# peabody124/PosePipeline

Hardware: AMD Instinct MI355X
Metric: frames/sec (whole node), detect->2D->3D cascade on 1080p; MPJPE vs reference (higher is better)
Workload: dtype f32; eligible float32 convolutions are evaluated as 2-term float16 splits (22 significand bits under per-channel / per-sample power-of-two scales, 3 products per term) on the 16-bit matrix cores with float32 accumulation (float32-accurate at any input magnitude, not bit-identical: tests/test_gpu_spl

## Files before the change

### include/posepipe_hip.h

```cpp
#ifndef POSEPIPE_HIP_H
#define POSEPIPE_HIP_H

#include <stddef.h>
#include <stdint.h>

#ifdef __cplusplus
extern "C" {
#endif

#define PP_ABI_VERSION 10

typedef enum {
    PP_OK = 0,
    PP_ERR_ARG = -1,
    PP_ERR_HIP = -2,
    PP_ERR_STATE = -3,
    PP_ERR_UNSUPPORTED = -4
} pp_status;

typedef enum { PP_MEM_HOST = 0, PP_MEM_DEVICE = 1 } pp_mem_kind;

typedef struct pp_ctx pp_ctx;
typedef struct pp_net pp_net;
typedef struct pp_tracker pp_tracker;
typedef struct pp_topdown pp_topdown;

int pp_abi_version(void);
const char* pp_last_error(void);
int pp_device_count(void);
int pp_ctx_create(int device, pp_ctx** out);
void pp_ctx_destroy(pp_ctx* ctx);
int pp_ctx_set_stream(pp_ctx* ctx, void* hip_stream);
int pp_ctx_synchronize(pp_ctx* ctx);
int pp_timer_start(pp_ctx* ctx);
int pp_timer_stop(pp_ctx* ctx, float* elapsed_ms);
int pp_debug_knob(const char* name, int value);
int pp_malloc(pp_ctx* ctx, size_t bytes, void** dptr);
int pp_free(pp_ctx* ctx, void* dptr);
int pp_memcpy_h2d(pp_ctx* ctx, void* dst, const void* src, size_t bytes);
int pp_memcpy_d2h(pp_ctx* ctx, void* dst, const void* src, size_t bytes);
int pp_memcpy_d2d(pp_ctx* ctx, void* dst, const void* src, size_t bytes);
int pp_host_alloc(pp_ctx* ctx, size_t bytes, void** host_ptr);
int pp_host_free(pp_ctx* ctx, void* host_ptr);
int pp_upload_begin(pp_ctx* ctx, void* dst_device, const void* src_host, size_t bytes);
int pp_upload_begin_nv12(pp_ctx* ctx, void* dst_bgr_device, void* tmp_nv12_device, const void* src_nv12_host, int frames,
                         int height, int width);
int pp_nv12_to_bgr(pp_ctx* ctx, const uint8_t* nv12_device, int frames, int height, int width, uint8_t* bgr_device);
int pp_upload_wait(pp_ctx* ctx, int host_sync);
int pp_upload_release(pp_ctx* ctx);

typedef enum {
    PP_OP_CONV = 1,
    PP_OP_MAXPOOL = 2,
    PP_OP_ROIALIGN = 3,
    PP_OP_COPY = 4,
    PP_OP_VIT_ENCODER = 5,
    PP_OP_DEPTH_TO_SPACE = 6,
    PP_OP_DECONV_BF16 = 8,
    PP_OP_AVGPOOL = 9,
    PP_OP_UPSAMPLE_ADD = 7,
    PP_OP_BILINEAR_ADD = 10,
    PP_OP_DWCONV3X3 = 11,
    PP_OP_LAYERNORM = 12,
    PP_OP_WINDOW_ATTN = 13,
    PP_OP_GELU_ADD = 14,
    PP_OP_ATTENTION = 15
} pp_op_type;

#define PP_RELU_NONE 0
#define PP_RELU_LAST 1
#define PP_RELU_FIRST 2
#define PP_ACT_LEAKY 3
#define PP_ACT_MISH 4
#define PP_ACT_ELU 5
#define PP_ACT_SWISH 6
#define PP_ACT_GELU 7
#define PP_DW_GELU_IN 1

typedef struct pp_op {
    int32_t type;
    int32_t in, out;
    int32_t res1, res2;
    int32_t cin, cout;
    int32_t kh, kw, stride, pad_h, pad_w, dil_h, dil_w;
    int32_t relu;
    int32_t up_log2;
    int32_t out_nchw;
    int32_t res1_shift;
    int32_t res1_off_w;
    int32_t out_c_off;
    int32_t in_c_off;
    int32_t pad_end;
    int64_t w_off, b_off;
    int32_t in2, in3;
    int32_t up2_log2, up3_log2;
} pp_op;

typedef struct pp_buf {
    int32_t h, w, c;
    int32_t pad;
} pp_buf;

int pp_net_create(pp_ctx* ctx, const pp_op* ops, int n_ops, const pp_buf* bufs, int n_bufs,
                  const float* weights, size_t n_weights, int max_batch, pp_net** out);
int pp_net_create_mem(pp_ctx* ctx, const pp_op* ops, int n_ops, const pp_buf* bufs, int n_bufs,
                      const float* weights, size_t n_weights, int weights_mem, int max_batch, pp_net** out);
#define PP_NET_NUMERICS_DEFAULT 0
#define PP_NET_NUMERICS_EXACT 1
#define PP_NET_NUMERICS_SPLIT 2
#define PP_NET_NUMERICS_SPLIT_BF16 3
#define PP_NET_NUMERICS_SPLIT_F16 4
int pp_net_create_ex(pp_ctx* ctx, const pp_op* ops, int n_ops, const pp_buf* bufs, int n_bufs,
                     const float* weights, size_t n_weights, int weights_mem, int max_batch, int numerics, pp_net** out);
int pp_net_numerics(pp_net* net);
int pp_net_split_kind(pp_net* net);
void pp_net_destroy(pp_net* net);
int pp_net_buffer(pp_net* net, int buf, void** dptr, size_t* bytes_per_sample);
int pp_net_input_amax(pp_net* net, int buf, void** dptr);
int pp_net_run(pp_net* net, int batch, int first_op, int last_op);
int pp_net_forward(pp_net* net, int batch, int in_buf, const float* in, int out_buf, float* out,
                   int mem);
int pp_net_set_lanes(pp_net* net, int enable);
int pp_net_set_lane_count(pp_net* net, int n_lanes);
int pp_net_capture(pp_net* net, int batch);
int pp_net_profile(pp_net* net, int batch, float* ms_per_op);
int pp_net_conv_kinds(pp_net* net, int* kinds);
int pp_net_folded_into(pp_net* net, int* into);

int pp_conv_force(int ct, int pt);
int pp_conv_variant(int variant);
int pp_conv_exact(int exact);
int pp_conv_split_kind(int f16);

int pp_conv2d(pp_ctx* ctx, const pp_op* op, int n, int hin, int win, const float* x,
              const float* w, const float* bias, const float* res1, const float* res2, float* y,
              int res1_h, int res1_w, int mem);

int pp_crop_resize_bilinear(pp_ctx* ctx, const float* src_nhwc4, int n_src, int src_h, int src_w, const int32_t* rects5, int n,
                            int out_h, int out_w, float* out_nhwc4);

int pp_net_vit_timing(pp_net* net, int enable, float* ms3, int* n_gemm);
int pp_f32_to_bf16(pp_ctx* ctx, const float* x, uint16_t* y, size_t n);
int pp_gemm_bf16(pp_ctx* ctx, const uint16_t* a, const uint16_t* w, const float* bias, const float* res, int res_mod,
                 void* c, int m, int n, int k, int act, int out_bf16);
int pp_layernorm(pp_ctx* ctx, const float* x, const float* gamma, const float* beta, int rows, int dim, float eps,
                 void* y, int out_bf16);
int pp_attention_bf16(pp_ctx* ctx, const uint16_t* qkv, int batch, int tokens, int heads, int head_dim, uint16_t* out);

int pp_crop_affine_normalize(pp_ctx* ctx, const uint8_t* frames, int n_frames, int h, int w,
                             const int32_t* frame_idx, const double* bbox_tlwh, int n_person,
                             int out_w, int out_h, const float* lut, const int32_t* chan_map,
                             int flip, float* out, float* center_scale, uint8_t* crop_u8,
                             int32_t* valid, int mem);

int pp_flip_merge_decode(pp_ctx* ctx, const float* hm, const float* hm_flip, int n, int k, int h,
                         int w, const int32_t* flip_perm, int shift_heatmap, int post,
                         int blur_kernel, const float* center_scale, float* kpts, float* merged,
                         int mem);

int pp_topdown_create(pp_net* net, int in_buf, int out_buf, int num_joints, const int32_t* flip_perm,
                      int shift_heatmap, int post, int blur_kernel, const float* lut,
                      const int32_t* chan_map, pp_topdown** out);
void pp_topdown_destroy(pp_topdown* t);
int pp_topdown_run(pp_topdown* t, const uint8_t* frames, int n_frames, int h, int w, int frames_mem,
                   const int32_t* frame_idx, const double* bbox_tlwh, int n_person, float* kpts,
                   int kpts_mem, int32_t* valid);
int pp_topdown_run_precropped(pp_topdown* t, const float* x_nhwc4, int x_mem, const float* center_scale,
                              int n_person, float* kpts, int kpts_mem);

int pp_topdown_timing(pp_topdown* t, float* ms3);

int pp_nms(pp_ctx* ctx, const void* boxes, const void* scores, int n, double iou_thr, int convention,
           int32_t* keep, int32_t* n_keep, int mem);

int pp_tracker_create(int mode, int feat_dim, double max_iou_distance, double max_cosine_distance,
                      int max_age, int n_init, pp_tracker** out);
void pp_tracker_destroy(pp_tracker* t);
int pp_tracker_step(pp_tracker* t, const double* dets_tlwh, const double* conf, const double* feats,
                    int n_det, int cap, int64_t* track_id, double* tlwh, int32_t* info, int32_t* n_out);
int pp_tracker_dump(pp_tracker* t, int cap, int64_t* ids, int32_t* state4, double* mean8,
                    double* cov64, int32_t* n_out);
int pp_kalman_initiate(const double* z4, double* mean8, double* cov64);
int pp_kalman_predict(double* mean8, double* cov64);
int pp_kalman_update(double* mean8, double* cov64, const double* z4);
int pp_kalman_gating_distance(const double* mean8, const double* cov64, const double* z4, int n,
                              double* out);
int pp_linear_sum_assignment(const double* cost, int n_rows, int n_cols, int32_t* rows,
                             int32_t* cols, int32_t* n_pairs);

typedef struct pp_detector pp_detector;
int pp_detector_input_size(int src_h, int src_w, int32_t* nh, int32_t* nw, int32_t* hp, int32_t* wp);
int pp_rescale_size(int src_h, int src_w, int max_long, int max_short, int divisor, int32_t* nh, int32_t* nw,
                    int32_t* hp, int32_t* wp);
int pp_resize_pad_normalize(pp_ctx* ctx, const uint8_t* frames, int n, int src_h, int src_w, int frames_mem, int nh,
                            int nw, int hp, int wp, const float* lut, float pad_val, float* out_device);
int pp_detector_constants(double* out, int cap);
int pp_detector_create(pp_net* net_a, pp_net* net_b, const int32_t* bufs_a, const int32_t* bufs_b, int src_h,
                       int src_w, const float* lut, const float* base_anchors, pp_detector** out);
void pp_detector_destroy(pp_detector* d);
int pp_detector_run(pp_detector* d, const uint8_t* frames, int n_frames, int frames_mem, float* dets,
                    int32_t* n_dets, float* proposals, int32_t* n_proposals);
int pp_detector_timing(pp_detector* d, float* ms6);
int pp_detector_enqueue(pp_detector* d, const uint8_t* frames, int n_frames, int frames_mem, int want_proposals);
int pp_detector_collect(pp_detector* d, float* dets, int32_t* n_dets, float* proposals, int32_t* n_proposals);
#define PP_DET_N_MARGINS 8
#define PP_DET_MARGIN_RPN_CUT 0
#define PP_DET_MARGIN_RPN_NMS 1
#define PP_DET_MARGIN_RPN_TOP 2
#define PP_DET_MARGIN_ROI_LEVEL 3
#define PP_DET_MARGIN_SCORE_THR 4
#define PP_DET_MARGIN_DET_NMS 5
#define PP_DET_MARGIN_DET_TOP 6
#define PP_DET_MARGIN_DET_ORDER 7
int pp_detector_enable_margins(pp_detector* d, int enable, float score_weight);
int pp_detector_margins(pp_detector* d, int n_frames, float* margins);

int pp_detector_regress(pp_detector* d, int frame, const float* boxes_src_px, int n, float* out_boxes, float* out_scores);

enum { PP_ECC_OK = 0, PP_ECC_NAN = 1 , PP_ECC_DIVERGED = 2  };
int pp_gray_from_nhwc4(pp_ctx* ctx, const float* x_nhwc4, int n, int h, int w, int r, int g, int b, float* gray);
int pp_ecc_euclidean(pp_ctx* ctx, const float* gray, int n_images, int h, int w, const int32_t* pairs, int n_pairs, int num_iters,
                     double stop_eps, double* warp, double* rho, int32_t* iters, int32_t* status);

int pp_letterbox_bicubic(pp_ctx* ctx, const uint8_t* frames, int n, int src_h, int src_w, int frames_mem,
                         const int32_t* xtab, int nw, int kx, const int32_t* ytab, int nh, int ky, int size_h,
                         int size_w, float* out_device);
int pp_yolo_decode(pp_ctx* ctx, const float* feats, int n, int gh, int gw, int num_classes, int cls,
                   const float* anchors3x2, int input_h, int input_w, int image_h, int image_w, float* boxes,
                   float* scores, int out_mem);
int pp_reid_patches(pp_ctx* ctx, const uint8_t* frames, int n_frames, int src_h, int src_w, int frames_mem,
                    const int32_t* rects, int n, int ph, int pw, float* out_device);

int pp_videopose3d_lift_many(pp_net* net, int in_buf, int out_buf, const float* kpts2d_norm,
                             const int32_t* seg_frames, int n_segs, int in_features, int out_features,
                             int pad, float* out, int mem);
int pp_videopose3d_lift(pp_net* net, int in_buf, int out_buf, const float* kpts2d_norm, int n_frames,
                        int in_features, int out_features, int pad, float* out);

int pp_warp_affine_normalize(pp_ctx* ctx, const uint8_t* frames, int n_frames, int h, int w, const double* center,
                             const double* scale, int out_w, int out_h, const float* lut, const int32_t* chan_map,
                             int flip, float* out, uint8_t* warp_u8, int mem);
int pp_bottomup_aggregate(pp_ctx* ctx, const float* s0, const float* s1, int n_frames, int k, int h0, int w0, int h1,
                          int w1, const int32_t* flip_perm, int hr, int wr, int align_corners, float* hm);
int pp_bottomup_candidates(pp_ctx* ctx, const float* hm, const float* s0, int n_frames, int k, int h0, int w0,
                           const int32_t* flip_perm, int hr, int wr, int align_corners, int max_people, float* cand);
int pp_bottomup_refine(pp_ctx* ctx, const float* hm, const float* s0, int n_frames, int k, int h0, int w0,
                       const int32_t* flip_perm, int hr, int wr, int align_corners, int n_person,
                       const int32_t* person_frame, const float* mean_tag, const int32_t* need, float* out);

int pp_attention_f32(pp_ctx* ctx, const float* qkv, int batch, int tokens, int heads, int c_real, int c_buf, float* out);
int pp_poseformer_spatial_param_floats(void);
int pp_poseformer_head_param_floats(void);
int pp_poseformer_spatial(pp_ctx* ctx, const float* params, const float* kpts2d_norm, int n_frames, int kpts_mem, float* features);
int pp_poseformer_lift(pp_net* net, int in_buf, int out_buf, long long spatial_off, long long pos_off, long long head_off,
                       const float* kpts2d_norm, int n_frames, float* out, int mem, float* stage_ms);

#define PP_OP_DCN3X3 16
#define PP_OP_DWDECONV 17
int pp_fairmot_input_size(int src_h, int src_w, int32_t* hp, int32_t* wp, int32_t* nh, int32_t* nw, int32_t* top, int32_t* left);
int pp_fairmot_preprocess(pp_ctx* ctx, const uint8_t* frames, int n, int src_h, int src_w, int frames_mem, int hp, int wp, int nh,
                          int nw, int top, int left, float* out_device);
int pp_fairmot_decode(pp_ctx* ctx, const float* hm, const float* wh, const float* reg, const float* id, int n, int h, int w, int K,
                      int id_dim, float* dets, float* feats, int32_t* inds, int mem);

typedef struct pp_smpl_model pp_smpl_model;
int pp_warp_affine_normalize_each(pp_ctx* ctx, const uint8_t* frames, int n_frames, int h, int w, const int32_t* frame_idx,
                                  const double* matrices, int n, int out_w, int out_h, const float* lut, const int32_t* chan_map,
                                  float* out, uint8_t* crop_u8, int mem);
long long pp_gru_param_floats(int in, int hidden, int layers);
int pp_gru_forward(pp_ctx* ctx, const float* x, int B, int T, int in, int hidden, int layers, const float* params, float* y, int mem);
int pp_smpl_model_create(pp_ctx* ctx, const float* v_template, const float* shapedirs, const float* posedirs, const float* j_regressor,
                         const float* weights, const float* j_regressor_extra, int n_verts, const int32_t* vertex_ids,
                         const int32_t* joint_map, pp_smpl_model** out);
void pp_smpl_model_destroy(pp_smpl_model* model);
int pp_smpl_forward(pp_ctx* ctx, pp_smpl_model* model, const float* betas, const float* rotmat, const float* cam, int F, float* verts,
                    float* joints3d, float* kp2d, float* pose_aa, int mem);
int pp_vibe_head_unpack(pp_ctx* ctx, const float* pose6d, const float* shape, int shape_stride, const float* cam_in, int cam_stride,
                        int F, float* rotmat, float* betas, float* cam);

#define PP_OP_SUB_CAT 18
// ... 16 lines not shown
```

### posepipeline_amd/_lib.py

```python
from __future__ import annotations

import ctypes as C
import os

import numpy as np

_HERE = os.path.dirname(os.path.abspath(__file__))
LIB_PATH = os.environ.get("POSEPIPE_LIB", os.path.join(_HERE, "libposepipe_hip.so"))

PP_MEM_HOST, PP_MEM_DEVICE = 0, 1
PP_OP_CONV, PP_OP_MAXPOOL, PP_OP_ROIALIGN, PP_OP_COPY, PP_OP_VIT_ENCODER, PP_OP_DEPTH_TO_SPACE, PP_OP_UPSAMPLE_ADD = 1, 2, 3, 4, 5, 6, 7
PP_OP_DECONV_BF16 = 8
PP_OP_AVGPOOL = 9
PP_OP_BILINEAR_ADD = 10
PP_OP_DWCONV3X3, PP_OP_LAYERNORM, PP_OP_WINDOW_ATTN, PP_OP_GELU_ADD = 11, 12, 13, 14
PP_OP_ATTENTION = 15
PP_OP_DCN3X3, PP_OP_DWDECONV = 16, 17
PP_OP_SUB_CAT, PP_OP_BCAST_MUL, PP_OP_BLEND2 = 18, 19, 20
PP_OP_GRAPH_MIX, PP_OP_JOINT_ATTN = 21, 22
PP_RELU_NONE, PP_RELU_LAST, PP_RELU_FIRST = 0, 1, 2
PP_ACT_LEAKY, PP_ACT_MISH, PP_ACT_ELU, PP_ACT_SWISH = 3, 4, 5, 6
PP_ACT_GELU = 7
PP_DW_GELU_IN = 1
PP_NET_NUMERICS_DEFAULT, PP_NET_NUMERICS_EXACT, PP_NET_NUMERICS_SPLIT = 0, 1, 2
PP_NET_NUMERICS_SPLIT_BF16, PP_NET_NUMERICS_SPLIT_F16 = 3, 4
PP_ECC_OK, PP_ECC_NAN, PP_ECC_DIVERGED = 0, 1, 2
NUMERICS = {None: 0, "default": 0, "exact": 1, "split": 2, "split_bf16": 3, "split_f16": 4}


class PosePipeHipError(RuntimeError):
    pass


class pp_op(C.Structure):
    _fields_ = [
        ("type", C.c_int32),
        ("in_", C.c_int32),
        ("out", C.c_int32),
        ("res1", C.c_int32),
        ("res2", C.c_int32),
        ("cin", C.c_int32),
        ("cout", C.c_int32),
        ("kh", C.c_int32),
        ("kw", C.c_int32),
        ("stride", C.c_int32),
        ("pad_h", C.c_int32),
        ("pad_w", C.c_int32),
        ("dil_h", C.c_int32),
        ("dil_w", C.c_int32),
        ("relu", C.c_int32),
        ("up_log2", C.c_int32),
        ("out_nchw", C.c_int32),
        ("res1_shift", C.c_int32),
        ("res1_off_w", C.c_int32),
        ("out_c_off", C.c_int32),
        ("in_c_off", C.c_int32),
        ("pad_end", C.c_int32),
        ("w_off", C.c_int64),
        ("b_off", C.c_int64),
        ("in2", C.c_int32),
        ("in3", C.c_int32),
        ("up2_log2", C.c_int32),
        ("up3_log2", C.c_int32),
    ]

    def __init__(self, *args, **kw):
        kw.setdefault("in2", -1)
        kw.setdefault("in3", -1)
        super().__init__(*args, **kw)


class pp_buf(C.Structure):
    _fields_ = [("h", C.c_int32), ("w", C.c_int32), ("c", C.c_int32), ("pad", C.c_int32)]


_vp = C.c_void_p
_i = C.c_int
_sz = C.c_size_t

SIGNATURES = {
    "pp_abi_version": (_i, []),
    "pp_last_error": (C.c_char_p, []),
    "pp_device_count": (_i, []),
    "pp_ctx_create": (_i, [_i, C.POINTER(_vp)]),
    "pp_ctx_destroy": (None, [_vp]),
    "pp_ctx_set_stream": (_i, [_vp, _vp]),
    "pp_ctx_synchronize": (_i, [_vp]),
    "pp_timer_start": (_i, [_vp]),
    "pp_timer_stop": (_i, [_vp, C.POINTER(C.c_float)]),
    "pp_malloc": (_i, [_vp, _sz, C.POINTER(_vp)]),
    "pp_free": (_i, [_vp, _vp]),
    "pp_memcpy_h2d": (_i, [_vp, _vp, _vp, _sz]),
    "pp_memcpy_d2h": (_i, [_vp, _vp, _vp, _sz]),
    "pp_memcpy_d2d": (_i, [_vp, _vp, _vp, _sz]),
    "pp_host_alloc": (_i, [_vp, _sz, C.POINTER(_vp)]),
    "pp_host_free": (_i, [_vp, _vp]),
    "pp_upload_begin": (_i, [_vp, _vp, _vp, _sz]),
    "pp_upload_begin_nv12": (_i, [_vp, _vp, _vp, _vp, _i, _i, _i]),
    "pp_nv12_to_bgr": (_i, [_vp, _vp, _i, _i, _i, _vp]),
    "pp_upload_wait": (_i, [_vp, _i]),
    "pp_upload_release": (_i, [_vp]),
    "pp_net_create": (_i, [_vp, C.POINTER(pp_op), _i, C.POINTER(pp_buf), _i, _vp, _sz, _i, C.POINTER(_vp)]),
    "pp_net_create_mem": (_i, [_vp, C.POINTER(pp_op), _i, C.POINTER(pp_buf), _i, _vp, _sz, _i, _i, C.POINTER(_vp)]),
    "pp_net_create_ex": (_i, [_vp, C.POINTER(pp_op), _i, C.POINTER(pp_buf), _i, _vp, _sz, _i, _i, _i, C.POINTER(_vp)]),
    "pp_net_numerics": (_i, [_vp]),
    "pp_net_split_kind": (_i, [_vp]),
    "pp_conv_split_kind": (_i, [_i]),
    "pp_net_destroy": (None, [_vp]),
    "pp_net_buffer": (_i, [_vp, _i, C.POINTER(_vp), C.POINTER(_sz)]),
    "pp_net_run": (_i, [_vp, _i, _i, _i]),
    "pp_net_forward": (_i, [_vp, _i, _i, _vp, _i, _vp, _i]),
    "pp_net_capture": (_i, [_vp, _i]),
    "pp_net_set_lanes": (_i, [_vp, _i]),
    "pp_net_set_lane_count": (_i, [_vp, _i]),
    "pp_net_conv_kinds": (_i, [_vp, _vp]),
    "pp_net_folded_into": (_i, [_vp, _vp]),
    "pp_net_profile": (_i, [_vp, _i, _vp]),
    "pp_crop_resize_bilinear": (_i, [_vp, _vp, _i, _i, _i, _vp, _i, _i, _i, _vp]),
    "pp_conv_force": (_i, [_i, _i]),
    "pp_conv_variant": (_i, [_i]),
    "pp_conv_exact": (_i, [_i]),
    "pp_conv2d": (_i, [_vp, C.POINTER(pp_op), _i, _i, _i, _vp, _vp, _vp, _vp, _vp, _vp, _i, _i, _i]),
    "pp_crop_affine_normalize": (_i, [_vp, _vp, _i, _i, _i, _vp, _vp, _i, _i, _i, _vp, _vp, _i, _vp, _vp, _vp, _vp, _i]),
    "pp_topdown_create": (_i, [_vp, _i, _i, _i, _vp, _i, _i, _i, _vp, _vp, C.POINTER(_vp)]),
    "pp_topdown_destroy": (None, [_vp]),
    "pp_topdown_run": (_i, [_vp, _vp, _i, _i, _i, _i, _vp, _vp, _i, _vp, _i, _vp]),
    "pp_topdown_run_precropped": (_i, [_vp, _vp, _i, _vp, _i, _vp, _i]),
    "pp_topdown_timing": (_i, [_vp, _vp]),
    "pp_detector_input_size": (_i, [_i, _i] + [C.POINTER(C.c_int32)] * 4),
    "pp_detector_constants": (_i, [C.POINTER(C.c_double), _i]),
    "pp_debug_knob": (_i, [C.c_char_p, _i]),
    "pp_net_input_amax": (_i, [_vp, _i, C.POINTER(_vp)]),
    "pp_rescale_size": (_i, [_i, _i, _i, _i, _i] + [C.POINTER(C.c_int32)] * 4),
    "pp_resize_pad_normalize": (_i, [_vp, _vp, _i, _i, _i, _i, _i, _i, _i, _i, _vp, C.c_float, _vp]),
    "pp_detector_create": (_i, [_vp, _vp, _vp, _vp, _i, _i, _vp, _vp, C.POINTER(_vp)]),
    "pp_detector_destroy": (None, [_vp]),
    "pp_detector_run": (_i, [_vp, _vp, _i, _i, _vp, _vp, _vp, _vp]),
    "pp_detector_timing": (_i, [_vp, _vp]),
    "pp_detector_enqueue": (_i, [_vp, _vp, _i, _i, _i]),
    "pp_detector_collect": (_i, [_vp, _vp, _vp, _vp, _vp]),
    "pp_detector_enable_margins": (_i, [_vp, _i, C.c_float]),
    "pp_detector_margins": (_i, [_vp, _i, _vp]),
    "pp_detector_regress": (_i, [_vp, _i, _vp, _i, _vp, _vp]),
    "pp_gray_from_nhwc4": (_i, [_vp, _vp, _i, _i, _i, _i, _i, _i, _vp]),
    "pp_ecc_euclidean": (_i, [_vp, _vp, _i, _i, _i, _vp, _i, _i, C.c_double, _vp, _vp, _vp, _vp]),
    "pp_nms": (_i, [_vp, _vp, _vp, _i, C.c_double, _i, _vp, C.POINTER(C.c_int32), _i]),
    "pp_videopose3d_lift": (_i, [_vp, _i, _i, _vp, _i, _i, _i, _i, _vp]),
    "pp_videopose3d_lift_many": (_i, [_vp, _i, _i, _vp, _vp, _i, _i, _i, _i, _vp, _i]),
    "pp_letterbox_bicubic": (_i, [_vp, _vp, _i, _i, _i, _i, _vp, _i, _i, _vp, _i, _i, _i, _i, _vp]),
    "pp_yolo_decode": (_i, [_vp, _vp, _i, _i, _i, _i, _i, _vp, _i, _i, _i, _i, _vp, _vp, _i]),
    "pp_reid_patches": (_i, [_vp, _vp, _i, _i, _i, _i, _vp, _i, _i, _i, _vp]),
    "pp_tracker_create": (_i, [_i, _i, C.c_double, C.c_double, _i, _i, C.POINTER(_vp)]),
    "pp_tracker_destroy": (None, [_vp]),
    "pp_tracker_step": (_i, [_vp, _vp, _vp, _vp, _i, _i, _vp, _vp, _vp, C.POINTER(C.c_int32)]),
    "pp_tracker_dump": (_i, [_vp, _i, _vp, _vp, _vp, _vp, C.POINTER(C.c_int32)]),
    "pp_kalman_initiate": (_i, [_vp, _vp, _vp]),
    "pp_kalman_predict": (_i, [_vp, _vp]),
    "pp_kalman_update": (_i, [_vp, _vp, _vp]),
    "pp_kalman_gating_distance": (_i, [_vp, _vp, _vp, _i, _vp]),
    "pp_linear_sum_assignment": (_i, [_vp, _i, _i, _vp, _vp, C.POINTER(C.c_int32)]),
    "pp_flip_merge_decode": (_i, [_vp, _vp, _vp, _i, _i, _i, _i, _vp, _i, _i, _i, _vp, _vp, _vp, _i]),
    "pp_net_vit_timing": (_i, [_vp, _i, _vp, _vp]),
    "pp_f32_to_bf16": (_i, [_vp, _vp, _vp, _sz]),
    "pp_gemm_bf16": (_i, [_vp, _vp, _vp, _vp, _vp, _i, _vp, _i, _i, _i, _i, _i]),
    "pp_layernorm": (_i, [_vp, _vp, _vp, _vp, _i, _i, C.c_float, _vp, _i]),
    "pp_attention_bf16": (_i, [_vp, _vp, _i, _i, _i, _i, _vp]),
    "pp_warp_affine_normalize": (_i, [_vp, _vp, _i, _i, _i, _vp, _vp, _i, _i, _vp, _vp, _i, _vp, _vp, _i]),
    "pp_bottomup_aggregate": (_i, [_vp, _vp, _vp, _i, _i, _i, _i, _i, _i, _vp, _i, _i, _i, _vp]),
    "pp_bottomup_candidates": (_i, [_vp, _vp, _vp, _i, _i, _i, _i, _vp, _i, _i, _i, _i, _vp]),
    "pp_bottomup_refine": (_i, [_vp, _vp, _vp, _i, _i, _i, _i, _vp, _i, _i, _i, _i, _vp, _vp, _vp, _vp]),
    "pp_attention_f32": (_i, [_vp, _vp, _i, _i, _i, _i, _i, _vp]),
    "pp_poseformer_spatial_param_floats": (_i, []),
    "pp_poseformer_head_param_floats": (_i, []),
    "pp_poseformer_spatial": (_i, [_vp, _vp, _vp, _i, _i, _vp]),
    "pp_poseformer_lift": (_i, [_vp, _i, _i, C.c_longlong, C.c_longlong, C.c_longlong, _vp, _i, _vp, _i, _vp]),
    "pp_fairmot_input_size": (_i, [_i, _i] + [C.POINTER(C.c_int32)] * 6),
    "pp_fairmot_preprocess": (_i, [_vp, _vp, _i, _i, _i, _i, _i, _i, _i, _i, _i, _i, _vp]),
    "pp_fairmot_decode": (_i, [_vp, _vp, _vp, _vp, _vp, _i, _i, _i, _i, _i, _vp, _vp, _vp, _i]),
    "pp_trades_cva": (_i, [_vp, _vp, _vp, _i, _i, _i, _i, _vp, _vp, _vp, _i]),
    "pp_trades_render_prehm": (_i, [_vp, _vp, _i, _i, _i, _vp, _i]),
    "pp_trades_decode": (_i, [_vp, _vp, _vp, _vp, _vp, _i, _i, _i, _i, _vp, _vp, _i]),
    "pp_warp_affine_normalize_each": (_i, [_vp, _vp, _i, _i, _i, _vp, _vp, _i, _i, _i, _vp, _vp, _vp, _vp, _i]),
    "pp_gru_param_floats": (C.c_longlong, [_i, _i, _i]),
    "pp_gru_forward": (_i, [_vp, _vp, _i, _i, _i, _i, _i, _vp, _vp, _i]),
    "pp_smpl_model_create": (_i, [_vp, _vp, _vp, _vp, _vp, _vp, _vp, _i, _vp, _vp, C.POINTER(_vp)]),
    "pp_smpl_model_destroy": (None, [_vp]),
    "pp_smpl_forward": (_i, [_vp, _vp, _vp, _vp, _vp, _i, _vp, _vp, _vp, _vp, _i]),
    "pp_vibe_head_unpack": (_i, [_vp, _vp, _vp, _i, _vp, _i, _i, _vp, _vp, _vp]),
}

_lib = None


def load_library() -> C.CDLL:
    global _lib
    if _lib is not None:
        return _lib
    if not os.path.exists(LIB_PATH):
        raise PosePipeHipError(
            f"{LIB_PATH} not found: build it with `python -c 'import __graft_entry__ as g; g.build()'` "
            "or `make -C posepipeline_amd/csrc` (there is no CPU fallback)"
        )
    lib = C.CDLL(LIB_PATH)
    for name, (res, args) in SIGNATURES.items():
        fn = getattr(lib, name)
        fn.restype = res
        fn.argtypes = args
    _lib = lib
    return lib


import contextlib


@contextlib.contextmanager
def default_numerics(mode):
    lib = load_library()
    prev = _DEFAULT_NUMERICS[0]

    def apply(m):
        check(lib.pp_conv_exact({None: -1, "default": -1, "exact": 1, "split": 0, "split_bf16": 0, "split_f16": 0}[m]), "pp_conv_exact")
        check(lib.pp_conv_split_kind({"split_bf16": 0, "split_f16": 1}.get(m, -1)), "pp_conv_split_kind")
    apply(mode)
    _DEFAULT_NUMERICS[0] = mode
    try:
        yield
    finally:
        apply(prev)
        _DEFAULT_NUMERICS[0] = prev


_DEFAULT_NUMERICS = [None]


def last_error() -> str:
    return load_library().pp_last_error().decode("utf-8", "replace")


def check(rc: int, what: str = "") -> None:
    if rc != 0:
        raise PosePipeHipError(f"{what or 'libposepipe_hip'} failed (status {rc}): {last_error()}")


def ptr(a):
    if a is None:
        return None
    if isinstance(a, int):
        return C.c_void_p(a)
    if isinstance(a, np.ndarray):
        assert a.flags["C_CONTIGUOUS"], "array must be C-contiguous"
        return C.c_void_p(a.ctypes.data)
    if hasattr(a, "data_ptr"):
        assert a.is_contiguous(), "tensor must be contiguous"
        return C.c_void_p(a.data_ptr())
    raise TypeError(type(a))


def mem_kind(a) -> int:
    if isinstance(a, np.ndarray):
        return PP_MEM_HOST
    if hasattr(a, "is_cuda"):
        return PP_MEM_DEVICE if a.is_cuda else PP_MEM_HOST
    raise TypeError(type(a))


class Context:

    def __init__(self, device: int = 0):
# ... 47 lines not shown
```

### posepipeline_amd/csrc/api_core.hip

```cpp
#include <dlfcn.h>

#include <algorithm>
#include <memory>

#include "pp_internal.h"

#include <atomic>
extern std::atomic<int> g_decode_generic, g_split_gemm_epi;

static thread_local std::string g_last_error;

void pp_set_error(const char* fmt, ...) {
    char buf[1024];
    va_list ap;
    va_start(ap, fmt);
    vsnprintf(buf, sizeof(buf), fmt, ap);
    va_end(ap);
    g_last_error = buf;
}

namespace {
struct Roctx {
    int (*push)(const char*) = nullptr;
    int (*pop)() = nullptr;
    Roctx() {
        for (const char* lib : {"librocprofiler-sdk-roctx.so", "librocprofiler-sdk-roctx.so.1", "libroctx64.so", "libroctx64.so.4"}) {
            void* h = dlopen(lib, RTLD_LAZY | RTLD_LOCAL);
            if (!h) continue;
            push = reinterpret_cast<int (*)(const char*)>(dlsym(h, "roctxRangePushA"));
            pop = reinterpret_cast<int (*)()>(dlsym(h, "roctxRangePop"));
            if (push && pop) return;
            push = nullptr; pop = nullptr;
        }
    }
};
const Roctx& roctx() {
    static const Roctx r;
    return r;
}
}

void pp_range_push(const char* name) {
    if (roctx().push) (void)roctx().push(name);
}
void pp_range_pop() {
    if (roctx().pop) (void)roctx().pop();
}

int pp_ctx::ensure_scratch(size_t bytes) {
    if (bytes <= scratch_bytes) return PP_OK;
    if (scratch) {
        PP_HIP_CHECK(hipStreamSynchronize(stream));
        PP_HIP_CHECK(hipFree(scratch));
        scratch = nullptr;
        scratch_bytes = 0;
    }
    size_t want = std::max(bytes, size_t(1) << 20);
    PP_HIP_CHECK(hipMalloc(&scratch, want));
    scratch_bytes = want;
    return PP_OK;
}

extern "C" {

int pp_abi_version(void) { return PP_ABI_VERSION; }

int pp_debug_knob(const char* name, int value) {
    PP_REQUIRE(name && value >= -1 && value <= 1, "pp_debug_knob: name and a value in {-1, 0, 1}");
    if (!strcmp(name, "decode_generic")) g_decode_generic.store(value, std::memory_order_relaxed);
    else if (!strcmp(name, "split_gemm_epilogue")) g_split_gemm_epi.store(value, std::memory_order_relaxed);
    else {
        pp_set_error("pp_debug_knob: unknown knob '%s' (decode_generic, split_gemm_epilogue)", name);
        return PP_ERR_ARG;
    }
    return PP_OK;
}

const char* pp_last_error(void) { return g_last_error.c_str(); }

int pp_device_count(void) {
    int n = 0;
    if (hipGetDeviceCount(&n) != hipSuccess) {
        (void)hipGetLastError();
        return 0;
    }
    return n;
}

int pp_ctx_create(int device, pp_ctx** out) {
    PP_REQUIRE(out != nullptr, "pp_ctx_create: out is NULL");
    *out = nullptr;
    int n = 0;
    hipError_t e = hipGetDeviceCount(&n);
    if (e != hipSuccess || n <= 0) {
        (void)hipGetLastError();
        pp_set_error("pp_ctx_create: no HIP device visible (%s) -- this library has no CPU fallback",
                     e == hipSuccess ? "device count 0" : hipGetErrorString(e));
        return PP_ERR_HIP;
    }
    PP_REQUIRE(device >= 0 && device < n, "pp_ctx_create: device %d out of range [0,%d)", device, n);
    PP_HIP_CHECK(hipSetDevice(device));
    std::unique_ptr<pp_ctx> c(new pp_ctx());
    c->device = device;
    PP_HIP_CHECK(hipStreamCreateWithFlags(&c->stream, hipStreamNonBlocking));
    PP_HIP_CHECK(hipEventCreate(&c->ev_start));
    PP_HIP_CHECK(hipEventCreate(&c->ev_stop));
    PP_HIP_CHECK(hipStreamCreateWithFlags(&c->copy_stream, hipStreamNonBlocking));
    PP_HIP_CHECK(hipEventCreateWithFlags(&c->ev_upload, hipEventDisableTiming));
    PP_HIP_CHECK(hipEventCreateWithFlags(&c->ev_consumed, hipEventDisableTiming));
    *out = c.release();
    return PP_OK;
}

void pp_ctx_destroy(pp_ctx* ctx) {
    if (!ctx) return;
    (void)hipSetDevice(ctx->device);
    if (ctx->stream) (void)hipStreamSynchronize(ctx->stream);
    if (ctx->scratch) (void)hipFree(ctx->scratch);
    if (ctx->ev_start) (void)hipEventDestroy(ctx->ev_start);
    if (ctx->ev_stop) (void)hipEventDestroy(ctx->ev_stop);
    if (ctx->copy_stream) {
        (void)hipStreamSynchronize(ctx->copy_stream);
        (void)hipStreamDestroy(ctx->copy_stream);
    }
    if (ctx->ev_upload) (void)hipEventDestroy(ctx->ev_upload);
    if (ctx->ev_consumed) (void)hipEventDestroy(ctx->ev_consumed);
    if (ctx->own_stream && ctx->stream) (void)hipStreamDestroy(ctx->stream);
    delete ctx;
}

int pp_ctx_set_stream(pp_ctx* ctx, void* hip_stream) {
    PP_REQUIRE(ctx, "pp_ctx_set_stream: ctx is NULL");
    PP_HIP_CHECK(hipStreamSynchronize(ctx->stream));
    if (ctx->own_stream && ctx->stream) PP_HIP_CHECK(hipStreamDestroy(ctx->stream));
    ctx->stream = static_cast<hipStream_t>(hip_stream);
    ctx->own_stream = false;
    return PP_OK;
}

int pp_ctx_synchronize(pp_ctx* ctx) {
    PP_REQUIRE(ctx, "pp_ctx_synchronize: ctx is NULL");
    PP_HIP_CHECK(hipStreamSynchronize(ctx->stream));
    return PP_OK;
}

int pp_timer_start(pp_ctx* ctx) {
    PP_REQUIRE(ctx, "pp_timer_start: ctx is NULL");
    PP_HIP_CHECK(hipEventRecord(ctx->ev_start, ctx->stream));
    return PP_OK;
}

int pp_timer_stop(pp_ctx* ctx, float* elapsed_ms) {
    PP_REQUIRE(ctx && elapsed_ms, "pp_timer_stop: NULL argument");
    PP_HIP_CHECK(hipEventRecord(ctx->ev_stop, ctx->stream));
    PP_HIP_CHECK(hipEventSynchronize(ctx->ev_stop));
    PP_HIP_CHECK(hipEventElapsedTime(elapsed_ms, ctx->ev_start, ctx->ev_stop));
    return PP_OK;
}

int pp_malloc(pp_ctx* ctx, size_t bytes, void** dptr) {
    PP_REQUIRE(ctx && dptr, "pp_malloc: NULL argument");
    PP_HIP_CHECK(hipSetDevice(ctx->device));
    PP_HIP_CHECK(hipMalloc(dptr, bytes ? bytes : 1));
    return PP_OK;
}

int pp_free(pp_ctx* ctx, void* dptr) {
    PP_REQUIRE(ctx, "pp_free: ctx is NULL");
    if (!dptr) return PP_OK;
    PP_HIP_CHECK(hipStreamSynchronize(ctx->stream));
    PP_HIP_CHECK(hipFree(dptr));
    return PP_OK;
}

int pp_memcpy_h2d(pp_ctx* ctx, void* dst, const void* src, size_t bytes) {
    PP_REQUIRE(ctx && (bytes == 0 || (dst && src)), "pp_memcpy_h2d: NULL argument");
    PP_HIP_CHECK(hipMemcpyAsync(dst, src, bytes, hipMemcpyHostToDevice, ctx->stream));
    PP_HIP_CHECK(hipStreamSynchronize(ctx->stream));
    return PP_OK;
}

int pp_host_alloc(pp_ctx* ctx, size_t bytes, void** out) {
    PP_REQUIRE(ctx && out, "pp_host_alloc: NULL argument");
    *out = nullptr;
    PP_HIP_CHECK(hipSetDevice(ctx->device));
    PP_HIP_CHECK(hipHostMalloc(out, bytes ? bytes : 1, hipHostMallocDefault));
    return PP_OK;
}

int pp_host_free(pp_ctx* ctx, void* p) {
    PP_REQUIRE(ctx != nullptr, "pp_host_free: ctx is NULL");
    if (p) PP_HIP_CHECK(hipHostFree(p));
    return PP_OK;
}

int pp_upload_begin(pp_ctx* ctx, void* dst, const void* src, size_t bytes) {
    PP_REQUIRE(ctx && (bytes == 0 || (dst && src)), "pp_upload_begin: NULL argument");
    PP_HIP_CHECK(hipStreamWaitEvent(ctx->copy_stream, ctx->ev_consumed, 0));
    PP_HIP_CHECK(hipMemcpyAsync(dst, src, bytes, hipMemcpyHostToDevice, ctx->copy_stream));
    PP_HIP_CHECK(hipEventRecord(ctx->ev_upload, ctx->copy_stream));
    return PP_OK;
}

int pp_upload_begin_nv12(pp_ctx* ctx, void* dst_bgr, void* tmp_nv12, const void* src_host, int frames, int height, int width) {
    PP_REQUIRE(ctx && (frames == 0 || (dst_bgr && tmp_nv12 && src_host)), "pp_upload_begin_nv12: NULL argument");
    PP_REQUIRE(frames >= 0 && height > 0 && width > 0, "pp_upload_begin_nv12: bad shape");
    PP_HIP_CHECK(hipStreamWaitEvent(ctx->copy_stream, ctx->ev_consumed, 0));
    const size_t bytes = (size_t)frames * height * width * 3 / 2;
    if (bytes) PP_HIP_CHECK(hipMemcpyAsync(tmp_nv12, src_host, bytes, hipMemcpyHostToDevice, ctx->copy_stream));
    const int r = pp_launch_nv12_to_bgr((const unsigned char*)tmp_nv12, (unsigned char*)dst_bgr, frames, height, width, ctx->copy_stream);
    if (r != PP_OK) return r;
    PP_HIP_CHECK(hipEventRecord(ctx->ev_upload, ctx->copy_stream));
    return PP_OK;
}

int pp_nv12_to_bgr(pp_ctx* ctx, const uint8_t* nv12, int frames, int height, int width, uint8_t* bgr) {
    PP_REQUIRE(ctx && (frames == 0 || (nv12 && bgr)), "pp_nv12_to_bgr: NULL argument");
    return pp_launch_nv12_to_bgr(nv12, bgr, frames, height, width, ctx->stream);
}

int pp_upload_wait(pp_ctx* ctx, int host_sync) {
    PP_REQUIRE(ctx != nullptr, "pp_upload_wait: ctx is NULL");
    PP_HIP_CHECK(hipStreamWaitEvent(ctx->stream, ctx->ev_upload, 0));
    if (host_sync) PP_HIP_CHECK(hipEventSynchronize(ctx->ev_upload));
    return PP_OK;
// ... 81 lines not shown
```

### posepipeline_amd/csrc/conv_split.hip

```cpp
#include <algorithm>
#include <atomic>
#include <map>
#include <mutex>
#include <type_traits>
#include <vector>
#include <cstring>
#include <cstdio>

#include "pp_internal.h"
#include "pp_amax.h"

#ifndef PP_SPLIT_ABLATE
#define PP_SPLIT_ABLATE 0
#endif

typedef __attribute__((ext_vector_type(8))) __bf16 bf16x8;
typedef __attribute__((ext_vector_type(8))) _Float16 f16x8;
typedef __attribute__((ext_vector_type(16))) float f32x16;

std::atomic<int> g_split_gemm_epi{-1};

namespace {


struct SplitArgs {
    const float* x;
    const uint4* w;
    const float* bias;
    const float* res1;
    const float* res2;
    float* y;
    int N, H, W, Cin, Cout, ncb;
    int xp_h, xp_w;
    int y_pad, r1_pad, r2_pad, relu;
    int nchunks;
    int tiles_x, tiles_y, TH, TW, bw_log2, gx_log2;
    int PWp;
    int NP, NPp;
    int mode, stride;
    int r1_shift, r1_H, r1_W;
    int ktaps, KW, pad, Hin, Win;
    long long S;
    unsigned x_bytes;
    int xcd_remap;
    int SP;
    int gx, gy;
    int col_major;
    int epi_lds;
    unsigned dv_per[2], dv_row[2];
    unsigned dv_tx[2], dv_ty[2], dv_pw[2];
    unsigned dv_ncol[2], dv_run0[2], dv_run1[2];
    unsigned dv_ktaps[2], dv_kw[2];
    const float* wscale;
    const unsigned* x_amax;
    unsigned* y_amax;
    const float* x2;
    const unsigned* x2_amax;
    int Cin2, stride2, xp2_h, xp2_w, seg1;
#ifdef PP_SPLIT_TIMELINE
    unsigned long long* dbg;
#endif
};

#ifdef PP_SPLIT_TIMELINE
#define PP_TL_DECL unsigned long long tl_t[10] = {0, 0, 0, 0, 0, 0, 0, 0, 0, 0}
#define PP_TL_MARK(i) do { if (a.dbg) tl_t[i] = __builtin_amdgcn_s_memtime(); } while (0)
#define PP_TL_FLUSH()                                                                                                    \
    do {                                                                                                                 \
        if (a.dbg && threadIdx.x == 0) {                                                                                 \
            unsigned hw, xcc;                                                                                            \
            asm volatile("s_getreg_b32 %0, hwreg(HW_REG_HW_ID)" : "=s"(hw));                                            \
            asm volatile("s_getreg_b32 %0, hwreg(HW_REG_XCC_ID)" : "=s"(xcc));                                          \
            unsigned long long* r = a.dbg + (size_t)blockIdx.x * 16;                                                     \
            r[0] = blockIdx.x; r[1] = ((unsigned long long)xcc << 32) | hw;                                              \
            r[2] = tl_t[0]; r[3] = tl_t[1]; r[4] = tl_t[2]; r[5] = tl_t[3]; r[6] = L; r[7] = col;                       \
            for (int i_ = 4; i_ < 10; ++i_) r[4 + i_] = tl_t[i_];                                                        \
        }                                                                                                                \
    } while (0)
#else
#define PP_TL_DECL
#define PP_TL_MARK(i)
#define PP_TL_FLUSH()
#endif

__device__ __forceinline__ unsigned pp_udiv(unsigned n, const unsigned (&dv)[2]) {
    const unsigned t = __umulhi(n, dv[0]);
    const unsigned q = (t + ((n - t) >> 1)) >> (dv[1] & 31u);
    return dv[1] >= 32u ? n : q;
}

__device__ __forceinline__ bool xcd_tile_column(unsigned L, const SplitArgs& a, unsigned& tile, unsigned& col) {
    const unsigned ntiles = (unsigned)a.gx, ncol = (unsigned)a.gy;
    const unsigned xcd = L & 7u, j = L >> 3;
    const unsigned q = ntiles >> 3, r = ntiles & 7u;
    const unsigned run = xcd < r ? q + 1 : q;
    unsigned tj;
    if (a.col_major) {
        if (run == 0) return false;
        col = xcd < r ? pp_udiv(j, a.dv_run1) : pp_udiv(j, a.dv_run0);
        tj = j - col * run;
        if (col >= ncol) return false;
    } else {
        tj = pp_udiv(j, a.dv_ncol);
        col = j - tj * ncol;
        if (tj >= run) return false;
    }
    tile = (xcd < r ? xcd * (q + 1) : r * (q + 1) + (xcd - r) * q) + tj;
    return true;
}

typedef __attribute__((ext_vector_type(2))) __bf16 bf16x2_t;
typedef __attribute__((ext_vector_type(2))) float f32x2_t;
__device__ __forceinline__ void split4(const float4 v, uint2& p0, uint2& p1, uint2& p2) {
    const f32x2_t a = {v.x, v.y}, b = {v.z, v.w};
    const bf16x2_t a0 = __builtin_convertvector(a, bf16x2_t), b0 = __builtin_convertvector(b, bf16x2_t);
    const f32x2_t ra = a - __builtin_convertvector(a0, f32x2_t), rb = b - __builtin_convertvector(b0, f32x2_t);
    const bf16x2_t a1 = __builtin_convertvector(ra, bf16x2_t), b1 = __builtin_convertvector(rb, bf16x2_t);
    const f32x2_t sa = ra - __builtin_convertvector(a1, f32x2_t), sb = rb - __builtin_convertvector(b1, f32x2_t);
    const bf16x2_t a2 = __builtin_convertvector(sa, bf16x2_t), b2 = __builtin_convertvector(sb, bf16x2_t);
    p0 = make_uint2(__builtin_bit_cast(unsigned, a0), __builtin_bit_cast(unsigned, b0));
    p1 = make_uint2(__builtin_bit_cast(unsigned, a1), __builtin_bit_cast(unsigned, b1));
    p2 = make_uint2(__builtin_bit_cast(unsigned, a2), __builtin_bit_cast(unsigned, b2));
}

typedef __attribute__((ext_vector_type(2))) _Float16 f16x2_t;
__device__ __forceinline__ void split2h(const float x0, const float x1, const float s, unsigned& h0, unsigned& h1) {
    unsigned d, e;
    asm("v_fma_mixlo_f16 %0, %1, %2, 0" : "=v"(d) : "v"(x0), "v"(s));
    asm("v_fma_mixhi_f16 %0, %1, %2, 0" : "+v"(d) : "v"(x1), "v"(s));
    asm("v_fma_mixlo_f16 %0, %1, %2, -%3 op_sel_hi:[0,0,1]" : "=v"(e) : "v"(x0), "v"(s), "v"(d));
    asm("v_fma_mixhi_f16 %0, %1, %2, -%3 op_sel:[0,0,1] op_sel_hi:[0,0,1]" : "+v"(e) : "v"(x1), "v"(s), "v"(d));
    h0 = d;
    h1 = e;
}
__device__ __forceinline__ void split4h(const float4 v, const float s, uint2& p0, uint2& p1) {
    split2h(v.x, v.y, s, p0.x, p1.x);
    split2h(v.z, v.w, s, p0.y, p1.y);
}

__device__ __forceinline__ float split_activate(float x, int act) {
    if (act == PP_ACT_LEAKY) return x >= 0.f ? x : 0.1f * x;
    if (act == PP_ACT_MISH) {
        if (x > 20.f) return x;
        const double n = exp((double)x);
        const double t = n * (n + 2.0);
        return x * (float)(t / (t + 2.0));
    }
    if (act == PP_ACT_ELU) return x > 0.f ? x : (float)expm1((double)x);
    if (act == PP_ACT_SWISH) return x * (float)(1.0 / (1.0 + exp(-(double)x)));
    return x;
}

__device__ __forceinline__ int lane_q(int r) {
    const int g1 = ((r >= 4 && r < 12) || (r >= 16 && r < 20) || r >= 28) ? 1 : 0;
    int idx;
    if (!g1) idx = r < 4 ? r : r < 16 ? r - 8 : r - 12;
    else idx = r < 12 ? r - 4 : r < 20 ? r - 8 : r - 16;
    return g1 * 16 + idx;
}
__device__ __forceinline__ void block_pixel(int r, int bw_log2, int& iy, int& ix) {
    if (bw_log2 == 0) {
        iy = 0;
        ix = r;
        return;
    }
    const int q = lane_q(r);
    if (bw_log2 == 1) {
        iy = q >> 4;
        ix = q & 15;
    } else {
        iy = ((q >> 3) & 1) * 2 + (q >> 4);
        ix = q & 7;
    }
}

enum { MODE_TILE = 0, MODE_STREAM = 1, MODE_GEMM = 2 };

template <int T, int NSLOT, int COB, int PXB = 2, int NW = 4, bool RING4 = false, bool H = false, bool S2 = false>
__global__ __launch_bounds__(64 * NW, NW == 4 ? 2 : 1) void conv_split_kernel(SplitArgs a) {
    static_assert(!S2 || (T == 9 && RING4 && H && PXB == 1), "S2 is the 4-wave fp16 ring form with one pixel block per wave");
    constexpr int NT = 64 * NW;
    constexpr int XP = H ? 2 : 3;
    constexpr int WPL = H ? 2 : 3;
    constexpr bool WLDS = NW == 8 || RING4;
    static_assert(!RING4 || (NW == 4 && T == 9), "RING4 is the 4-wave 3x3 form");
    extern __shared__ __attribute__((aligned(16))) unsigned char smem[];
    const int tid = threadIdx.x;
    const int lane = tid & 63;
    const int wave = tid >> 6;
    unsigned L = blockIdx.x, col = blockIdx.y;
    PP_TL_DECL;
    PP_TL_MARK(0);
    if (a.xcd_remap) {
        if (!xcd_tile_column(blockIdx.x, a, L, col)) return;
    }
    const int cb0 = (int)col * COB;
    const int plane_bytes = 2 * a.NPp * 16;
    const int buf_bytes = XP * plane_bytes;

    int n = 0, x0 = 0, y0 = 0;
    unsigned s0 = 0;
    if (a.mode == MODE_TILE) {
        const unsigned L2 = pp_udiv(L, a.dv_tx);
        const int tx = (int)(L - L2 * (unsigned)a.tiles_x);
        n = (int)pp_udiv(L2, a.dv_ty);
        const int ty = (int)(L2 - (unsigned)n * (unsigned)a.tiles_y);
        x0 = tx * a.TW;
        y0 = ty * a.TH;
    } else {
        s0 = L * (unsigned)(32 * PXB * NW);
    }

    unsigned goff[NSLOT];
    unsigned vmask[T == 1 ? NSLOT : 1];
    int simg[H ? NSLOT : 1];
    const int woff0 = ((((tid & 3) >> 1) * a.NPp + (tid >> 2)) * 16 + (tid & 1) * 8);
    if (a.mode == MODE_STREAM) {
        const int pos0 = (int)s0 - a.PWp - 1 + (tid >> 2);
        const unsigned cin4 = (unsigned)a.Cin * 4u;
        const unsigned base = (unsigned)pos0 * cin4 + (unsigned)(tid & 3) * 16u;
#pragma unroll
        for (int j = 0; j < NSLOT; ++j) goff[j] = pos0 + (NT / 4) * j < 0 ? 0xffffffffu : base + (unsigned)((NT / 4) * j) * cin4;
        if constexpr (T == 1) {
#pragma unroll
            for (int j = 0; j < NSLOT; ++j) vmask[j] = 0;
        }
        if constexpr (H) {
#pragma unroll
            for (int j = 0; j < NSLOT; ++j) {
                const int pj = pos0 + (NT / 4) * j;
                simg[j] = (int)pp_udiv((unsigned)min(max(pj, 0), (int)a.S - 1), a.dv_per);
            }
        }
    } else {
#pragma unroll
    for (int j = 0; j < NSLOT; ++j) {
        const int u = tid + NT * j;
        const int p = u >> 2, quad = u & 3;
        const bool in_patch = p < a.NP;
        unsigned off = 0xffffffffu;
        if constexpr (H) simg[j] = n;
        if constexpr (S2) {
            const int ph = (int)pp_udiv((unsigned)p, a.dv_row), r = p - ph * a.SP;
            const int qr = (int)pp_udiv((unsigned)r, a.dv_pw), qc = r - qr * a.PWp;
            const int pr = 2 * qr + (ph >> 1), pc = 2 * qc + (ph & 1);
            const int iy = 2 * y0 - 1 + pr, ix = 2 * x0 - 1 + pc;
            if (in_patch && pc <= 2 * a.TW && (unsigned)iy < (unsigned)a.Hin && (unsigned)ix < (unsigned)a.Win)
                off = (unsigned)(((n * a.xp_h + iy) * a.xp_w + ix) * a.Cin) * 4u;
        } else if (a.mode == MODE_TILE) {
            const int pr = (int)pp_udiv((unsigned)p, a.dv_pw), pc = p - pr * a.PWp;
            const int iy = y0 - 1 + pr, ix = x0 - 1 + pc;
            if (in_patch && pc < a.TW + 2 && (unsigned)iy < (unsigned)a.H && (unsigned)ix < (unsigned)a.W)
                off = (unsigned)(((n * a.xp_h + iy) * a.xp_w + ix) * a.Cin) * 4u;
        } else {
            const unsigned m = s0 + (unsigned)p;
            if constexpr (T == 1) vmask[j] = 0;
            if (in_patch && m < (unsigned)a.S) {
                const int img = (int)pp_udiv(m, a.dv_per), rem = (int)(m - (unsigned)img * (unsigned)(a.H * a.W));
                const int ho = (int)pp_udiv((unsigned)rem, a.dv_row), wo = rem - ho * a.W;
                if constexpr (H) simg[j] = img;
                if (T == 1 && a.ktaps > 1) {
                    const int iy0 = ho * a.stride - a.pad, ix0 = wo * a.stride - a.pad;
                    off = (unsigned)(((img * a.xp_h + iy0) * a.xp_w + ix0) * a.Cin) * 4u;
                    unsigned vm = 0;
                    for (int t = 0, dy = 0, dx = 0; t < a.ktaps; ++t) {
                        if ((unsigned)(iy0 + dy) < (unsigned)a.Hin && (unsigned)(ix0 + dx) < (unsigned)a.Win) vm |= 1u << t;
                        if (++dx == a.KW) { dx = 0; ++dy; }
                    }
                    if constexpr (T == 1) vmask[j] = vm;
                    if (off == 0xffffffffu) off = 0xfffffffeu;
                } else {
                    off = (unsigned)(((img * a.xp_h + ho * a.stride) * a.xp_w + wo * a.stride) * a.Cin) * 4u;
                }
            }
        }
        goff[j] = off == 0xffffffffu ? off : off + (unsigned)quad * 16u;
    }
    }
    const __amdgpu_buffer_rsrc_t xrsrc = __builtin_amdgcn_make_buffer_rsrc((void*)a.x, 0, (int)a.x_bytes, 0x00020000);
    float4 xr[NSLOT];
    auto load_patch = [&](int c) {
        unsigned add = (unsigned)c * 64u;
        int tbit = -1;
        if (T == 1 && a.ktaps > 1) {
            const int cc = (int)pp_udiv((unsigned)c, a.dv_ktaps), t = c - cc * a.ktaps;
            const int dy = (int)pp_udiv((unsigned)t, a.dv_kw), dx = t - dy * a.KW;
            add = (unsigned)(((dy * a.xp_w + dx) * a.Cin + 16 * cc) * 4);
            tbit = t;
        }
#pragma unroll
        for (int j = 0; j < NSLOT; ++j) {
            bool ok = goff[j] != 0xffffffffu;
            if constexpr (T == 1) {
                if (tbit >= 0) ok = ((vmask[j] >> tbit) & 1u) != 0;
            }
            const unsigned off = ok ? goff[j] + add : 0xffffffffu;
            xr[j] = __builtin_bit_cast(float4, __builtin_amdgcn_raw_buffer_load_b128(xrsrc, (int)off, 0, 0));
        }
    };
    const bool last_ok = (tid >> 2) + (NT / 4) * (NSLOT - 1) < a.NP;
    unsigned sxe[H ? (NSLOT + 3) / 4 : 1];
    auto store_patch = [&](int buf, int j0, int j1) {
#pragma unroll
        for (int j = 0; j < NSLOT; ++j) {
            if (j < j0 || j >= j1) continue;
            uint2 p0, p1, p2;
            if constexpr (H) split4h(xr[j], __uint_as_float((268u - ((sxe[j >> 2] >> (8 * (j & 3))) & 0xffu)) << 23), p0, p1);
            else split4(xr[j], p0, p1, p2);
            if (j == NSLOT - 1 && !last_ok) continue;
            unsigned char* d = smem + buf * buf_bytes + woff0 + (NT / 4) * 16 * j;
            *reinterpret_cast<uint2*>(d) = p0;
            *reinterpret_cast<uint2*>(d + plane_bytes) = p1;
            if constexpr (!H) *reinterpret_cast<uint2*>(d + 2 * plane_bytes) = p2;
        }
    };
    PP_TL_MARK(4);
    constexpr int WSLOT = COB * WPL * 1024;
    constexpr int NDMA = (COB * WPL + NW - 1) / NW;
    const unsigned wring = (unsigned)((RING4 ? 1 : 2) * buf_bytes);
    const unsigned lds_base = (unsigned)(size_t)(__attribute__((address_space(3))) unsigned char*)smem;
    const int nsteps = a.nchunks * T;
    const size_t wstep = (size_t)a.ncb * WPL * 64;
    auto issue_w = [&](int step) {
        if (step >= nsteps) return;
#pragma unroll
        for (int i = 0; i < NDMA; ++i) {
            const int myslab = (wave + NW * i) % (COB * WPL);
            const unsigned dst = __builtin_amdgcn_readfirstlane(lds_base + wring + (unsigned)((step & 3) * WSLOT + myslab * 1024));
            const uint4* g = a.w + (size_t)cb0 * (WPL * 64) + myslab * 64 + lane + (size_t)step * wstep;
            asm volatile("s_mov_b32 m0, %1\n\ts_nop 0\n\tglobal_load_lds_dwordx4 %0, off" ::"v"(g), "s"(dst) : "memory", "m0");
        }
    };
    const uint4* wlane = a.w + (size_t)cb0 * WPL * 64 + lane;
    constexpr int WSETS = COB >= 4 ? 1 : 2;
    uint4 wf[WSETS][COB][WPL];
    uint4 xf[PXB][XP];
    const uint4* wp = wlane;
    auto load_w = [&](uint4 (&dst)[COB][WPL]) {
#pragma unroll
        for (int cb = 0; cb < COB; ++cb)
#pragma unroll
            for (int pl = 0; pl < WPL; ++pl) dst[cb][pl] = wp[(cb * WPL + pl) * 64];
        wp += wstep;
    };
    if constexpr (WLDS) {
        issue_w(0);
        issue_w(1);
        issue_w(2);
        load_patch(0);
    } else {
        load_patch(0);
        load_w(wf[0]);
    }
    unsigned xam[H ? NSLOT : 1];
    if constexpr (H) {
#pragma unroll
        for (int j = 0; j < NSLOT; ++j) xam[j] = a.x_amax[simg[j]];
    }
    __builtin_amdgcn_sched_barrier(0);

    auto pixel_coords = [&](int lane_, int wave_, int pb, int& aofs_, int& on_, int& oy_, int& ox_, bool& ok_) {
        if (a.mode == MODE_TILE) {
            const int BW = 32 >> a.bw_log2, BH = 1 << a.bw_log2;
            int by, bx;
            block_pixel(lane_ & 31, a.bw_log2, by, bx);
            const int b = wave_ * PXB + pb;
            const int gy = b >> a.gx_log2, gx = b & ((1 << a.gx_log2) - 1);
            const int ry = gy * BH + by, rx = gx * BW + bx;
            aofs_ = (((lane_ >> 5) * a.NPp) + ry * a.PWp + rx) * 16;
            on_ = n;
            oy_ = y0 + ry;
            ox_ = x0 + rx;
            ok_ = oy_ < a.H && ox_ < a.W;
        } else {
            const unsigned per = a.mode == MODE_STREAM ? (unsigned)(a.xp_h * a.PWp) : (unsigned)(a.H * a.W);
            const unsigned row = a.mode == MODE_STREAM ? (unsigned)a.PWp : (unsigned)a.W;
            const int pl = (wave_ * PXB + pb) * 32 + (lane_ & 31);
            aofs_ = (((lane_ >> 5) * a.NPp) + pl) * 16;
            const unsigned sp = s0 + (unsigned)pl;
            const bool in = sp < (unsigned)a.S;
            const unsigned sc = in ? sp : 0u;
            const unsigned img = pp_udiv(sc, a.dv_per);
            const unsigned rem = sc - img * per;
            const unsigned yy = pp_udiv(rem, a.dv_row);
            on_ = (int)img;
            oy_ = (int)yy;
            ox_ = (int)(rem - yy * row);
            ok_ = in && oy_ < a.H && ox_ < a.W;
        }
    };
    int aofs[PXB];
#pragma unroll
    for (int pb = 0; pb < PXB; ++pb) {
        int on_, oy_, ox_;
        bool ok_;
        pixel_coords(lane, wave, pb, aofs[pb], on_, oy_, ox_, ok_);
    }

    f32x16 acc[COB][PXB];
#pragma unroll
    for (int cb = 0; cb < COB; ++cb)
#pragma unroll
        for (int pb = 0; pb < PXB; ++pb)
#pragma unroll
            for (int i = 0; i < 16; ++i) acc[cb][pb][i] = 0.f;
    if constexpr (H) {
#pragma unroll
        for (int q = 0; q < (NSLOT + 3) / 4; ++q) sxe[q] = 0;
#pragma unroll
        for (int j = 0; j < NSLOT; ++j) sxe[j >> 2] |= pp_amax_exp(xam[j]) << (8 * (j & 3));
    }

    auto load_x = [&](const unsigned char* pbuf, int t, int pb) {
        const int dy = t / 3, dx = t % 3;
        const int toff = S2 ? ((((dy & 1) * 2 + (dx & 1)) * a.SP) + (dy >> 1) * a.PWp + (dx >> 1)) * 16 : T == 9 ? (dy * a.PWp + dx) * 16 : 0;
#pragma unroll
        for (int pl = 0; pl < XP; ++pl) xf[pb][pl] = *reinterpret_cast<const uint4*>(pbuf + pl * plane_bytes + aofs[pb] + toff);
    };

    if constexpr (!WLDS) {
        store_patch(0, 0, NSLOT);
        PP_TL_MARK(5);
        if (a.nchunks > 1) load_patch(1);
        __syncthreads();
#pragma unroll
        for (int pb = 0; pb < PXB; ++pb) load_x(smem, 0, pb);
    }

    auto mma = [&](const uint4 (&wc)[COB][WPL], int pb) {
        if constexpr (H) {
            constexpr int WI[3] = {1, 0, 0}, XI[3] = {0, 1, 0};
#pragma unroll
            for (int p = 0; p < 3; ++p)
#pragma unroll
                for (int cb = 0; cb < COB; ++cb)
                    acc[cb][pb] = __builtin_amdgcn_mfma_f32_32x32x16_f16(__builtin_bit_cast(f16x8, wc[cb][WI[p]]),
                                                                         __builtin_bit_cast(f16x8, xf[pb][XI[p]]), acc[cb][pb], 0, 0, 0);
        } else {
        constexpr int WI[6] = {2, 1, 0, 1, 0, 0}, XI[6] = {0, 1, 2, 0, 1, 0};
#pragma unroll
        for (int p = 0; p < 6; ++p)
#pragma unroll
            for (int cb = 0; cb < COB; ++cb)
                acc[cb][pb] = __builtin_amdgcn_mfma_f32_32x32x16_bf16(__builtin_bit_cast(bf16x8, wc[cb][WI[p]]),
                                                                      __builtin_bit_cast(bf16x8, xf[pb][XI[p]]), acc[cb][pb], 0, 0, 0);
        }
    };

    if constexpr (WLDS) {
        auto read_w = [&](int step, uint4 (&dst)[COB][WPL]) {
            const unsigned char* base = smem + wring + (step & 3) * WSLOT + lane * 16;
#pragma unroll
            for (int cb = 0; cb < COB; ++cb)
#pragma unroll
                for (int pl = 0; pl < WPL; ++pl) dst[cb][pl] = *reinterpret_cast<const uint4*>(base + (cb * WPL + pl) * 1024);
        };
        auto wait_all_but = [&](int n) {
            if (n == NSLOT + NDMA) asm volatile("s_waitcnt vmcnt(%0)" ::"n"(NSLOT + NDMA) : "memory");
            else if (n == NSLOT) asm volatile("s_waitcnt vmcnt(%0)" ::"n"(NSLOT) : "memory");
            else if (n == NDMA) asm volatile("s_waitcnt vmcnt(%0)" ::"n"(NDMA) : "memory");
            else asm volatile("s_waitcnt vmcnt(0)" ::: "memory");
        };
        store_patch(0, 0, NSLOT);
        PP_TL_MARK(5);
        if (a.nchunks > 1) load_patch(1);
        asm volatile("s_waitcnt lgkmcnt(0)" ::: "memory");
        __builtin_amdgcn_s_barrier();
        read_w(0, wf[0]);
#pragma unroll
        for (int pb = 0; pb < PXB; ++pb) load_x(smem, 0, pb);

        auto chunk8 = [&](auto par, int c) {
            constexpr int PAR = decltype(par)::value;
            const unsigned char* pbuf = smem + (c & 1) * buf_bytes;
            const int st0 = c * T;
            const bool more_patch = c + 1 < a.nchunks;
#pragma unroll
            for (int t = 0; t < T; ++t) {
                const int cur = (PAR + t) & 1;
                const int st = st0 + t;
#pragma unroll
                for (int pb = 0; pb < PXB; ++pb) {
                    if (pb == PXB - 1 && t == T / 2) {
                        if (more_patch) store_patch((c + 1) & 1, 0, NSLOT);
                        issue_w(st + 3);
                    }
                    mma(wf[cur % WSETS], pb);
                    __builtin_amdgcn_sched_barrier(0);
                    if (pb == 0) {
                        if (st + 1 < nsteps) read_w(st + 1, wf[(cur ^ 1) % WSETS]);
                        if (t != T / 2) issue_w(st + 3);
                    }
                    if (t + 1 < T) load_x(pbuf, t + 1, pb);
                    __builtin_amdgcn_sched_barrier(0);
                }
                {
                    const int younger = (st + 3 < nsteps ? NDMA : 0) + ((t == 0 && c + 1 < a.nchunks) ? NSLOT : 0);
                    wait_all_but(younger);
                    __builtin_amdgcn_s_barrier();
                }
            }
            if (c + 1 < a.nchunks) {
#pragma unroll
                for (int pb = 0; pb < PXB; ++pb) load_x(smem + ((c + 1) & 1) * buf_bytes, 0, pb);
            }
            if (c + 2 < a.nchunks) load_patch(c + 2);
        };
        auto chunk4 = [&](auto par, int c) {
            constexpr int PAR = decltype(par)::value;
            const int st0 = c * T;
            const bool more_patch = c + 1 < a.nchunks;
#pragma unroll
            for (int t = 0; t < T; ++t) {
                const int cur = (PAR + t) & 1;
                const int st = st0 + t;
#pragma unroll
                for (int pb = 0; pb < PXB; ++pb) {
                    if (pb == 0 && t == T - 1) {
                        if (more_patch) store_patch(0, 0, NSLOT);
                        issue_w(st + 3);
                        if (c + 2 < a.nchunks) load_patch(c + 2);
                    }
                    mma(wf[cur % WSETS], pb);
                    __builtin_amdgcn_sched_barrier(0);
                    if (pb == 0) {
                        if (WSETS == 2 && st + 1 < nsteps) read_w(st + 1, wf[(cur ^ 1) % WSETS]);
// ... 45 lines not shown
            __builtin_amdgcn_sched_barrier(0);
#pragma unroll
            for (int pb = 0; pb < PXB; ++pb) {
#if !(PP_SPLIT_ABLATE & 2)
                if (pb == PXB - 1 && t == T / 2 && c + 1 < a.nchunks) store_patch((c + 1) & 1, 0, NSLOT);
#endif
#if !(PP_SPLIT_ABLATE & 16)
                mma(wf[(PP_SPLIT_ABLATE & 1) ? 0 : cur % WSETS], pb);
#endif
                __builtin_amdgcn_sched_barrier(0);
#if !(PP_SPLIT_ABLATE & 8)
                if (t + 1 < T) load_x(pbuf, t + 1, pb);
#endif
                __builtin_amdgcn_sched_barrier(0);
            }
        }
#if !(PP_SPLIT_ABLATE & 4)
        __syncthreads();
#endif
#if !(PP_SPLIT_ABLATE & 8)
        if (c + 1 < a.nchunks) {
#pragma unroll
            for (int pb = 0; pb < PXB; ++pb) load_x(smem + ((c + 1) & 1) * buf_bytes, 0, pb);
        }
#endif
#if !(PP_SPLIT_ABLATE & 2)
        if (c + 2 < a.nchunks) load_patch(c + 2);
#endif
    };
    PP_TL_MARK(1);
    int c = 0;
    for (; c + 1 < a.nchunks; c += 2) {
        chunk(std::integral_constant<int, 0>{}, c);
        chunk(std::integral_constant<int, 1>{}, c + 1);
    }
    if (c < a.nchunks) chunk(std::integral_constant<int, 0>{}, c);
    }
    PP_TL_MARK(2);

    int on[PXB], oy[PXB], ox[PXB];
    bool ook[PXB];
    unsigned oam[H ? PXB : 1];
    {
        int tid_e = tid;
        asm volatile("" : "+v"(tid_e));
#pragma unroll
        for (int pb = 0; pb < PXB; ++pb) {
            int aofs_;
            pixel_coords(tid_e & 63, tid_e >> 6, pb, aofs_, on[pb], oy[pb], ox[pb], ook[pb]);
        }
        if constexpr (H) {
#pragma unroll
            for (int pb = 0; pb < PXB; ++pb) oam[pb] = a.x_amax[on[pb]];
        }
    }
#if (PP_SPLIT_ABLATE & 32)
    if (a.relu != 77) {
        if (ook[0]) a.y[(((size_t)on[0] * (a.H + a.y_pad) + oy[0]) * (a.W + a.y_pad) + ox[0]) * a.Cout + (lane >> 5)] = acc[0][0][0] + acc[COB - 1][PXB - 1][15];
        return;
    }
#endif
    constexpr int CBB = COB >= 3 ? 1 : COB;
    size_t ypix[PXB], r1pix[PXB], r2pix[PXB];
    float xinv[H ? PXB : 1];
#pragma unroll
    for (int pb = 0; pb < PXB; ++pb) {
        if constexpr (H) xinv[pb] = pp_act_unscale(oam[pb]);
        const int n_ = ook[pb] ? on[pb] : 0, y_ = ook[pb] ? oy[pb] : 0, x_ = ook[pb] ? ox[pb] : 0;
        ypix[pb] = ((size_t)n_ * (a.H + a.y_pad) + y_) * (a.W + a.y_pad) + x_;
        r1pix[pb] = ((size_t)n_ * (a.r1_H + a.r1_pad) + (y_ >> a.r1_shift)) * (a.r1_W + a.r1_pad) + (x_ >> a.r1_shift);
        r2pix[pb] = ((size_t)n_ * (a.H + a.r2_pad) + y_) * (a.W + a.r2_pad) + x_;
    }
    float ymax[PXB];
#pragma unroll
    for (int pb = 0; pb < PXB; ++pb) ymax[pb] = 0.f;
#pragma unroll
    for (int cq = 0; cq < COB; cq += CBB) {
    bool cok[CBB][4];
    int cos[CBB][4];
    float4 b4[CBB][4];
    float4 sc4[H ? CBB : 1][H ? 4 : 1];
#pragma unroll
    for (int cb = 0; cb < CBB; ++cb)
#pragma unroll
        for (int g = 0; g < 4; ++g) {
            const int co = (cb0 + cq + cb) * 32 + 8 * g + 4 * (lane >> 5);
            cok[cb][g] = co < a.Cout;
            cos[cb][g] = cok[cb][g] ? co : 0;
            b4[cb][g] = *reinterpret_cast<const float4*>(a.bias + cos[cb][g]);
            if constexpr (H) sc4[cb][g] = *reinterpret_cast<const float4*>(a.wscale + cos[cb][g]);
        }
    float4 rv[PXB][CBB][4];
    if (a.res1) {
#pragma unroll
        for (int pb = 0; pb < PXB; ++pb)
#pragma unroll
            for (int cb = 0; cb < CBB; ++cb)
#pragma unroll
                for (int g = 0; g < 4; ++g) rv[pb][cb][g] = *reinterpret_cast<const float4*>(a.res1 + r1pix[pb] * a.Cout + cos[cb][g]);
    }
#pragma unroll
    for (int pb = 0; pb < PXB; ++pb)
#pragma unroll
        for (int cb = 0; cb < CBB; ++cb)
#pragma unroll
            for (int g = 0; g < 4; ++g) {
                const f32x16 cc = acc[cq + cb][pb];
                const float4 b = b4[cb][g];
                float4 v;
                if constexpr (H) {
                    const float xi = xinv[pb];
                    const float4 sc = make_float4(sc4[cb][g].x * xi, sc4[cb][g].y * xi, sc4[cb][g].z * xi, sc4[cb][g].w * xi);
                    v = make_float4(__builtin_fmaf(cc[4 * g + 0], sc.x, b.x), __builtin_fmaf(cc[4 * g + 1], sc.y, b.y),
                                    __builtin_fmaf(cc[4 * g + 2], sc.z, b.z), __builtin_fmaf(cc[4 * g + 3], sc.w, b.w));
                } else {
                    v = make_float4(cc[4 * g + 0] + b.x, cc[4 * g + 1] + b.y, cc[4 * g + 2] + b.z, cc[4 * g + 3] + b.w);
                }
                if (a.relu == PP_RELU_FIRST) { v.x = fmaxf(v.x, 0.f); v.y = fmaxf(v.y, 0.f); v.z = fmaxf(v.z, 0.f); v.w = fmaxf(v.w, 0.f); }
                else if (a.relu >= PP_ACT_LEAKY) { v.x = split_activate(v.x, a.relu); v.y = split_activate(v.y, a.relu); v.z = split_activate(v.z, a.relu); v.w = split_activate(v.w, a.relu); }
                if (a.res1) { v.x += rv[pb][cb][g].x; v.y += rv[pb][cb][g].y; v.z += rv[pb][cb][g].z; v.w += rv[pb][cb][g].w; }
                rv[pb][cb][g] = v;
            }
    PP_TL_MARK(6);
    if (a.res2) {
#pragma unroll
        for (int pb = 0; pb < PXB; ++pb)
#pragma unroll
            for (int cb = 0; cb < CBB; ++cb)
#pragma unroll
                for (int g = 0; g < 4; ++g) {
                    const float4 r = *reinterpret_cast<const float4*>(a.res2 + r2pix[pb] * a.Cout + cos[cb][g]);
                    rv[pb][cb][g].x += r.x; rv[pb][cb][g].y += r.y; rv[pb][cb][g].z += r.z; rv[pb][cb][g].w += r.w;
                }
    }
#pragma unroll
    for (int pb = 0; pb < PXB; ++pb) {
#pragma unroll
        for (int cb = 0; cb < CBB; ++cb)
#pragma unroll
            for (int g = 0; g < 4; ++g) {
                float4 v = rv[pb][cb][g];
                if (a.relu == PP_RELU_LAST) { v.x = fmaxf(v.x, 0.f); v.y = fmaxf(v.y, 0.f); v.z = fmaxf(v.z, 0.f); v.w = fmaxf(v.w, 0.f); }
                if (ook[pb] && cok[cb][g]) {
                    *reinterpret_cast<float4*>(a.y + ypix[pb] * a.Cout + cos[cb][g]) = v;
                    ymax[pb] = fmaxf(ymax[pb], pp_abs4max(v));
                }
            }
    }
    }
    if (a.y_amax) {
        int wg_first = n, wg_last = n;
        if (a.mode != MODE_TILE) {
            const unsigned last = (unsigned)min((long long)s0 + 32 * PXB * NW - 1, a.S - 1);
            wg_first = (int)pp_udiv(min(s0, last), a.dv_per);
            wg_last = (int)pp_udiv(last, a.dv_per);
        }
        pp_amax_commit_wg<NW, PXB>(a.y_amax, on, ymax, wg_first, wg_last, reinterpret_cast<float*>(smem));
    }
    PP_TL_MARK(3);
#ifdef PP_SPLIT_TIMELINE
    asm volatile("s_waitcnt vmcnt(0)" ::: "memory");
    PP_TL_MARK(7);
#endif
    PP_TL_FLUSH();
}

typedef __attribute__((ext_vector_type(4))) float f32x4;

template <int NSLOT, bool H = false, bool WRING = false>
__global__ __launch_bounds__(256, 2) void conv_split48_kernel(SplitArgs a) {
    constexpr int NT = 256, NPAIR = 5, CB = 3, SB = 4;
    constexpr int XP = H ? 2 : 3;
    constexpr int WPL = H ? 2 : 3;
    extern __shared__ __attribute__((aligned(16))) unsigned char smem[];
    const int tid = threadIdx.x;
    const int lane = tid & 63;
    const int wave = tid >> 6;
    unsigned L = blockIdx.x, col = blockIdx.y;
    PP_TL_DECL;
    PP_TL_MARK(0);
    if (a.xcd_remap) {
        if (!xcd_tile_column(blockIdx.x, a, L, col)) return;
    }
    const int cbase = (int)col * CB;
    const int plane_bytes = 2 * a.NPp * 16;
    const int buf_bytes = XP * plane_bytes;
    int n = 0, x0 = 0, y0 = 0;
    unsigned s0 = 0;
    if (a.mode == MODE_TILE) {
        const unsigned L2 = pp_udiv(L, a.dv_tx);
        const int tx = (int)(L - L2 * (unsigned)a.tiles_x);
        n = (int)pp_udiv(L2, a.dv_ty);
        const int ty = (int)(L2 - (unsigned)n * (unsigned)a.tiles_y);
        x0 = tx * a.TW;
        y0 = ty * a.TH;
    } else {
        s0 = L * 256u;
    }
    unsigned goff[NSLOT];
    int simg[H ? NSLOT : 1];
    const int woff0 = ((((tid & 3) >> 1) * a.NPp + (tid >> 2)) * 16 + (tid & 1) * 8);
    if (a.mode == MODE_STREAM) {
        const int pos0 = (int)s0 - a.PWp - 1 + (tid >> 2);
        const unsigned cin4 = (unsigned)a.Cin * 4u;
        const unsigned base = (unsigned)pos0 * cin4 + (unsigned)(tid & 3) * 16u;
#pragma unroll
        for (int j = 0; j < NSLOT; ++j) goff[j] = pos0 + (NT / 4) * j < 0 ? 0xffffffffu : base + (unsigned)((NT / 4) * j) * cin4;
        if constexpr (H) {
#pragma unroll
            for (int j = 0; j < NSLOT; ++j) {
                const int pj = pos0 + (NT / 4) * j;
                simg[j] = (int)pp_udiv((unsigned)min(max(pj, 0), (int)a.S - 1), a.dv_per);
            }
        }
    } else {
#pragma unroll
        for (int j = 0; j < NSLOT; ++j) {
            const int u = tid + NT * j;
            const int p = u >> 2, quad = u & 3;
            const bool in_patch = p < a.NP;
            unsigned off = 0xffffffffu;
            if constexpr (H) simg[j] = n;
            const int pr = (int)pp_udiv((unsigned)p, a.dv_pw), pc = p - pr * a.PWp;
            const int iy = y0 - 1 + pr, ix = x0 - 1 + pc;
            if (in_patch && pc < a.TW + 2 && (unsigned)iy < (unsigned)a.H && (unsigned)ix < (unsigned)a.W)
                off = (unsigned)(((n * a.xp_h + iy) * a.xp_w + ix) * a.Cin) * 4u;
            goff[j] = off == 0xffffffffu ? off : off + (unsigned)quad * 16u;
        }
    }
    const __amdgpu_buffer_rsrc_t xrsrc = __builtin_amdgcn_make_buffer_rsrc((void*)a.x, 0, (int)a.x_bytes, 0x00020000);
    float4 xr[NSLOT];
    auto load_patch = [&](int c) {
#pragma unroll
        for (int j = 0; j < NSLOT; ++j) {
            const unsigned off = goff[j] == 0xffffffffu ? 0xffffffffu : goff[j] + (unsigned)c * 64u;
            xr[j] = __builtin_bit_cast(float4, __builtin_amdgcn_raw_buffer_load_b128(xrsrc, (int)off, 0, 0));
        }
    };
    const bool last_ok = (tid >> 2) + (NT / 4) * (NSLOT - 1) < a.NP;
    float sx[H ? NSLOT : 1];
    auto store_patch = [&](int buf) {
#pragma unroll
        for (int j = 0; j < NSLOT; ++j) {
            uint2 p0, p1, p2;
            if constexpr (H) split4h(xr[j], sx[j], p0, p1);
            else split4(xr[j], p0, p1, p2);
            if (j == NSLOT - 1 && !last_ok) continue;
            unsigned char* d = smem + buf * buf_bytes + woff0 + (NT / 4) * 16 * j;
            *reinterpret_cast<uint2*>(d) = p0;
            *reinterpret_cast<uint2*>(d + plane_bytes) = p1;
            if constexpr (!H) *reinterpret_cast<uint2*>(d + 2 * plane_bytes) = p2;
        }
    };
    const uint4* wp = a.w + (size_t)cbase * WPL * 64 + lane;
    const size_t wstep = (size_t)a.ncb * WPL * 64;
    uint4 wf[2][CB][WPL];
    auto load_w = [&](uint4 (&dst)[CB][WPL]) {
#pragma unroll
        for (int cb = 0; cb < CB; ++cb)
#pragma unroll
            for (int pl = 0; pl < WPL; ++pl) dst[cb][pl] = wp[(cb * WPL + pl) * 64];
        wp += wstep;
    };
    constexpr int WSLOT = CB * WPL * 1024, NDMA = (CB * WPL + 3) / 4;
    const int nsteps = a.nchunks * NPAIR;
    const unsigned lds_base = (unsigned)(size_t)(__attribute__((address_space(3))) unsigned char*)smem;
    const unsigned wring = (unsigned)(2 * buf_bytes);
    auto issue_w = [&](int step) {
        if (step >= nsteps) return;
#pragma unroll
        for (int i = 0; i < NDMA; ++i) {
            const int myslab = (wave + 4 * i) % (CB * WPL);
            const unsigned dst = __builtin_amdgcn_readfirstlane(lds_base + wring + (unsigned)((step & 3) * WSLOT + myslab * 1024));
            const uint4* g = a.w + (size_t)cbase * WPL * 64 + myslab * 64 + lane + (size_t)step * wstep;
            asm volatile("s_mov_b32 m0, %1\n\ts_nop 0\n\tglobal_load_lds_dwordx4 %0, off" ::"v"(g), "s"(dst) : "memory", "m0");
        }
    };
    auto read_w = [&](int step, uint4 (&dst)[CB][WPL]) {
        const unsigned char* base = smem + wring + (step & 3) * WSLOT + lane * 16;
#pragma unroll
        for (int cb = 0; cb < CB; ++cb)
#pragma unroll
            for (int pl = 0; pl < WPL; ++pl) dst[cb][pl] = *reinterpret_cast<const uint4*>(base + (cb * WPL + pl) * 1024);
    };
    auto wait_all_but = [&](int n) {
        if (n == NSLOT + NDMA) asm volatile("s_waitcnt vmcnt(%0) lgkmcnt(0)" ::"n"(NSLOT + NDMA) : "memory");
        else if (n == NSLOT) asm volatile("s_waitcnt vmcnt(%0) lgkmcnt(0)" ::"n"(NSLOT) : "memory");
        else if (n == NDMA) asm volatile("s_waitcnt vmcnt(%0) lgkmcnt(0)" ::"n"(NDMA) : "memory");
        else asm volatile("s_waitcnt vmcnt(0) lgkmcnt(0)" ::: "memory");
    };
    PP_TL_MARK(4);
    if constexpr (WRING) {
        issue_w(0);
        issue_w(1);
        issue_w(2);
        load_patch(0);
    } else {
        load_patch(0);
        load_w(wf[0]);
    }
    unsigned xam[H ? NSLOT : 1];
    if constexpr (H) {
#pragma unroll
        for (int j = 0; j < NSLOT; ++j) xam[j] = a.x_amax[simg[j]];
    }
    __builtin_amdgcn_sched_barrier(0);
    const int khalf = (lane >> 4) & 1;
    auto sub_block = [&](int sb, int& aof, int& on_, int& oy_, int& ox_, bool& ok) {
        const int b = wave * 2 + (sb >> 1), r = (sb & 1) * 16 + (lane & 15);
        if (a.mode == MODE_TILE) {
            const int BW = 32 >> a.bw_log2, BH = 1 << a.bw_log2;
            int by, bx;
            block_pixel(r, a.bw_log2, by, bx);
            const int gy = b >> a.gx_log2, gx = b & ((1 << a.gx_log2) - 1);
            const int ry = gy * BH + by, rx = gx * BW + bx;
            aof = ((khalf * a.NPp) + ry * a.PWp + rx) * 16;
            on_ = n;
            oy_ = y0 + ry;
            ox_ = x0 + rx;
            ok = oy_ < a.H && ox_ < a.W;
        } else {
            const int pl = b * 32 + r;
            aof = ((khalf * a.NPp) + pl) * 16;
            const unsigned sp = s0 + (unsigned)pl;
            const bool in = sp < (unsigned)a.S;
            const unsigned sc = in ? sp : 0u;
            const unsigned img = pp_udiv(sc, a.dv_per);
            const unsigned rem = sc - img * (unsigned)(a.xp_h * a.PWp);
            const unsigned yy = pp_udiv(rem, a.dv_row);
            on_ = (int)img;
            oy_ = (int)yy;
            ox_ = (int)(rem - yy * (unsigned)a.PWp);
            ok = in && oy_ < a.H && ox_ < a.W;
        }
    };
    int aofs[SB];
    unsigned oam[H ? SB : 1];
#pragma unroll
    for (int sb = 0; sb < SB; ++sb) {
        int t0, t1, t2;
        bool t3;
        sub_block(sb, aofs[sb], t0, t1, t2, t3);
        if constexpr (H) oam[sb] = a.x_amax[t0];
    }
    int tofs[NPAIR];
#pragma unroll
    for (int q = 0; q < NPAIR; ++q) {
        const int t = min(2 * q + (lane >> 5), 8);
        tofs[q] = ((t / 3) * a.PWp + (t % 3)) * 16;
    }
    f32x4 acc[CB][SB];
#pragma unroll
    for (int cb = 0; cb < CB; ++cb)
#pragma unroll
        for (int sb = 0; sb < SB; ++sb) acc[cb][sb] = f32x4{0.f, 0.f, 0.f, 0.f};
    uint4 xf[2][XP];
    auto load_x = [&](const unsigned char* pbuf, int q, int sb) {
#pragma unroll
        for (int pl = 0; pl < XP; ++pl) xf[sb & 1][pl] = *reinterpret_cast<const uint4*>(pbuf + pl * plane_bytes + aofs[sb] + tofs[q]);
    };
    auto mma = [&](const uint4 (&wc)[CB][WPL], int sb) {
        if constexpr (H) {
            constexpr int WI[3] = {1, 0, 0}, XI[3] = {0, 1, 0};
#pragma unroll
            for (int p = 0; p < 3; ++p)
#pragma unroll
                for (int cb = 0; cb < CB; ++cb)
                    acc[cb][sb] = __builtin_amdgcn_mfma_f32_16x16x32_f16(__builtin_bit_cast(f16x8, wc[cb][WI[p]]),
                                                                         __builtin_bit_cast(f16x8, xf[sb & 1][XI[p]]), acc[cb][sb], 0, 0, 0);
        } else {
        constexpr int WI[6] = {2, 1, 0, 1, 0, 0}, XI[6] = {0, 1, 2, 0, 1, 0};
#pragma unroll
        for (int p = 0; p < 6; ++p)
#pragma unroll
            for (int cb = 0; cb < CB; ++cb)
                acc[cb][sb] = __builtin_amdgcn_mfma_f32_16x16x32_bf16(__builtin_bit_cast(bf16x8, wc[cb][WI[p]]),
                                                                      __builtin_bit_cast(bf16x8, xf[sb & 1][XI[p]]), acc[cb][sb], 0, 0, 0);
        }
    };
    if constexpr (H) {
#pragma unroll
        for (int j = 0; j < NSLOT; ++j) sx[j] = pp_act_scale(xam[j]);
    }
    store_patch(0);
    PP_TL_MARK(5);
    if (a.nchunks > 1) load_patch(1);
    if constexpr (WRING) {
        asm volatile("s_waitcnt lgkmcnt(0)" ::: "memory");
        __builtin_amdgcn_s_barrier();
        read_w(0, wf[0]);
    } else {
        __syncthreads();
    }
    load_x(smem, 0, 0);
    auto chunk = [&](auto par, int c) {
        constexpr int PAR = decltype(par)::value;
        const unsigned char* pbuf = smem + (c & 1) * buf_bytes;
#pragma unroll
        for (int q = 0; q < NPAIR; ++q) {
            const int cur = (PAR + q) & 1;
            load_w(wf[cur ^ 1]);
            __builtin_amdgcn_sched_barrier(0);
#pragma unroll
            for (int sb = 0; sb < SB; ++sb) {
                if (sb == SB - 1 && q == NPAIR / 2 && c + 1 < a.nchunks) store_patch((c + 1) & 1);
                if (sb + 1 < SB) load_x(pbuf, q, sb + 1);
                else if (q + 1 < NPAIR) load_x(pbuf, q + 1, 0);
                __builtin_amdgcn_sched_barrier(0);
                mma(wf[cur], sb);
                __builtin_amdgcn_sched_barrier(0);
            }
        }
        __syncthreads();
        if (c + 1 < a.nchunks) load_x(smem + ((c + 1) & 1) * buf_bytes, 0, 0);
        if (c + 2 < a.nchunks) load_patch(c + 2);
    };
    auto chunk_ring = [&](auto par, int c) {
        constexpr int PAR = decltype(par)::value;
        const unsigned char* pbuf = smem + (c & 1) * buf_bytes;
#pragma unroll
        for (int q = 0; q < NPAIR; ++q) {
            const int cur = (PAR + q) & 1;
            const int st = c * NPAIR + q;
#pragma unroll
            for (int sb = 0; sb < SB; ++sb) {
                if (sb == SB - 1 && q == NPAIR / 2) {
                    if (c + 1 < a.nchunks) store_patch((c + 1) & 1);
                    issue_w(st + 3);
                    if (c + 2 < a.nchunks) load_patch(c + 2);
                }
                if (sb + 1 < SB) load_x(pbuf, q, sb + 1);
                else if (q + 1 < NPAIR) load_x(pbuf, q + 1, 0);
                __builtin_amdgcn_sched_barrier(0);
                mma(wf[cur], sb);
                __builtin_amdgcn_sched_barrier(0);
                if (sb == 0) {
                    if (st + 1 < nsteps) read_w(st + 1, wf[cur ^ 1]);
                    if (q != NPAIR / 2) issue_w(st + 3);
                }
            }
            const int younger = (st + 3 < nsteps ? NDMA : 0) + (((q == NPAIR / 2 || q == NPAIR / 2 + 1) && c + 2 < a.nchunks) ? NSLOT : 0);
            wait_all_but(younger);
            __builtin_amdgcn_s_barrier();
        }
        if (c + 1 < a.nchunks) load_x(smem + ((c + 1) & 1) * buf_bytes, 0, 0);
    };
    PP_TL_MARK(1);
    int c = 0;
    for (; c + 1 < a.nchunks; c += 2) {
        if constexpr (WRING) {
            chunk_ring(std::integral_constant<int, 0>{}, c);
            chunk_ring(std::integral_constant<int, 1>{}, c + 1);
        } else {
            chunk(std::integral_constant<int, 0>{}, c);
            chunk(std::integral_constant<int, 1>{}, c + 1);
        }
    }
    if (c < a.nchunks) {
        if constexpr (WRING) chunk_ring(std::integral_constant<int, 0>{}, c);
        else chunk(std::integral_constant<int, 0>{}, c);
    }
    PP_TL_MARK(2);
    bool cok[CB];
    int cos[CB];
    float4 b4[CB];
    float4 sc4[H ? CB : 1];
#pragma unroll
    for (int cb = 0; cb < CB; ++cb) {
        const int co = (cbase + cb) * 16 + 4 * (lane >> 4);
        cok[cb] = co < a.Cout;
        cos[cb] = cok[cb] ? co : 0;
        b4[cb] = *reinterpret_cast<const float4*>(a.bias + cos[cb]);
        if constexpr (H) sc4[cb] = *reinterpret_cast<const float4*>(a.wscale + cos[cb]);
    }
    size_t ypix[SB], r1pix[SB], r2pix[SB];
    bool ook[SB];
    int onn[SB];
    float xinv[H ? SB : 1];
#pragma unroll
    for (int sb = 0; sb < SB; ++sb) {
        int aof_, on_, oy_, ox_;
        sub_block(sb, aof_, on_, oy_, ox_, ook[sb]);
        onn[sb] = on_;
        if constexpr (H) xinv[sb] = pp_act_unscale(oam[sb]);
        const int n_ = ook[sb] ? on_ : 0, y_ = ook[sb] ? oy_ : 0, x_ = ook[sb] ? ox_ : 0;
        ypix[sb] = ((size_t)n_ * (a.H + a.y_pad) + y_) * (a.W + a.y_pad) + x_;
        r1pix[sb] = ((size_t)n_ * (a.r1_H + a.r1_pad) + (y_ >> a.r1_shift)) * (a.r1_W + a.r1_pad) + (x_ >> a.r1_shift);
        r2pix[sb] = ((size_t)n_ * (a.H + a.r2_pad) + y_) * (a.W + a.r2_pad) + x_;
    }
    float4 rv[SB][CB];
    if (a.res1) {
#pragma unroll
        for (int sb = 0; sb < SB; ++sb)
#pragma unroll
            for (int cb = 0; cb < CB; ++cb) rv[sb][cb] = *reinterpret_cast<const float4*>(a.res1 + r1pix[sb] * a.Cout + cos[cb]);
    }
#pragma unroll
    for (int sb = 0; sb < SB; ++sb)
#pragma unroll
        for (int cb = 0; cb < CB; ++cb) {
            const f32x4 cc = acc[cb][sb];
            const float4 b = b4[cb];
            float4 v;
            if constexpr (H) v = make_float4(__builtin_fmaf(cc[0], sc4[cb].x * xinv[sb], b.x), __builtin_fmaf(cc[1], sc4[cb].y * xinv[sb], b.y),
                                             __builtin_fmaf(cc[2], sc4[cb].z * xinv[sb], b.z), __builtin_fmaf(cc[3], sc4[cb].w * xinv[sb], b.w));
            else v = make_float4(cc[0] + b.x, cc[1] + b.y, cc[2] + b.z, cc[3] + b.w);
            if (a.relu == PP_RELU_FIRST) { v.x = fmaxf(v.x, 0.f); v.y = fmaxf(v.y, 0.f); v.z = fmaxf(v.z, 0.f); v.w = fmaxf(v.w, 0.f); }
            else if (a.relu >= PP_ACT_LEAKY) { v.x = split_activate(v.x, a.relu); v.y = split_activate(v.y, a.relu); v.z = split_activate(v.z, a.relu); v.w = split_activate(v.w, a.relu); }
            if (a.res1) { v.x += rv[sb][cb].x; v.y += rv[sb][cb].y; v.z += rv[sb][cb].z; v.w += rv[sb][cb].w; }
            rv[sb][cb] = v;
        }
    PP_TL_MARK(6);
    if (a.res2) {
#pragma unroll
        for (int sb = 0; sb < SB; ++sb)
#pragma unroll
            for (int cb = 0; cb < CB; ++cb) {
                const float4 r = *reinterpret_cast<const float4*>(a.res2 + r2pix[sb] * a.Cout + cos[cb]);
                rv[sb][cb].x += r.x; rv[sb][cb].y += r.y; rv[sb][cb].z += r.z; rv[sb][cb].w += r.w;
            }
    }
    float ymax[SB];
#pragma unroll
    for (int sb = 0; sb < SB; ++sb) {
        ymax[sb] = 0.f;
#pragma unroll
        for (int cb = 0; cb < CB; ++cb) {
            float4 v = rv[sb][cb];
            if (a.relu == PP_RELU_LAST) { v.x = fmaxf(v.x, 0.f); v.y = fmaxf(v.y, 0.f); v.z = fmaxf(v.z, 0.f); v.w = fmaxf(v.w, 0.f); }
            if (ook[sb] && cok[cb]) {
                *reinterpret_cast<float4*>(a.y + ypix[sb] * a.Cout + cos[cb]) = v;
                ymax[sb] = fmaxf(ymax[sb], pp_abs4max(v));
            }
        }
    }
    if (a.y_amax) {
        int wg_first = n, wg_last = n;
        if (a.mode != MODE_TILE) {
            const unsigned last = (unsigned)min((long long)s0 + 255, a.S - 1);
            wg_first = (int)pp_udiv(min(s0, last), a.dv_per);
            wg_last = (int)pp_udiv(last, a.dv_per);
        }
        pp_amax_commit_wg<4, SB>(a.y_amax, onn, ymax, wg_first, wg_last, reinterpret_cast<float*>(smem));
    }
    PP_TL_MARK(3);
#ifdef PP_SPLIT_TIMELINE
    asm volatile("s_waitcnt vmcnt(0)" ::: "memory");
    PP_TL_MARK(7);
#endif
    PP_TL_FLUSH();
}

__device__ __forceinline__ float channel_scale(float cmax) {
    if (!(cmax > 0.f) || !(cmax < 3.0e38f)) return 1.f;
    int e;
    (void)frexpf(cmax, &e);
    return ldexpf(1.f, 15 - e);
}
__device__ __forceinline__ void split_weight_h(float v, float c, unsigned short& q0, unsigned short& q1, unsigned short& q2) {
    const float vs = v * c;
    const _Float16 g0 = (_Float16)vs;
    const float r = vs - (float)g0;
    const _Float16 g1 = (_Float16)r;
    q0 = __builtin_bit_cast(unsigned short, g0);
    q1 = __builtin_bit_cast(unsigned short, g1);
    q2 = 0;
}
__global__ __launch_bounds__(64) void weight_channel_max_kernel(const float* w, int kchunks, int CoutPad, int nout, float* cmax, float* inv_scale) {
    const int cout = blockIdx.x, lane = threadIdx.x;
    float m = 0.f;
    if (cout < CoutPad)
        for (int c = lane >> 5; c < kchunks; c += 2) m = fmaxf(m, fabsf(w[((size_t)c * CoutPad + cout) * 32 + (lane & 31)]));
#pragma unroll
    for (int o = 32; o > 0; o >>= 1) m = fmaxf(m, __shfl_xor(m, o));
    if (lane == 0 && cout < nout) {
        cmax[cout] = m;
        inv_scale[cout] = 1.f / channel_scale(m);
    }
}

template <bool H>
__global__ __launch_bounds__(256) void split_weights48_kernel(const float* w, uint4* out, int Cin, int CoutPad, int ncb16, size_t total, const float* cmax) {
    const size_t i = blockIdx.x * (size_t)256 + threadIdx.x;
    if (i >= total) return;
    const int lane = (int)(i & 63);
    size_t r = i >> 6;
    const int cb = (int)(r % ncb16);
    r /= ncb16;
    const int pair = (int)(r % 5);
    const int c = (int)(r / 5);
    const int g = lane >> 4;
    const int t = 2 * pair + (g >> 1);
    const int cout = cb * 16 + (lane & 15);
    unsigned short h[3][8];
#pragma unroll
    for (int j = 0; j < 8; ++j) {
        const int cin = c * 16 + (g & 1) * 8 + j;
        const int k = t * Cin + cin;
        float v = 0.f;
        if (t < 9 && cout < CoutPad) v = w[((size_t)(k >> 5) * CoutPad + cout) * 32 + 8 * (k & 3) + ((k & 31) >> 2)];
        if constexpr (H) {
            split_weight_h(v, channel_scale(cmax[cout]), h[0][j], h[1][j], h[2][j]);
            continue;
        }
        const __bf16 q0 = (__bf16)v;
        const float r1 = v - (float)q0;
        const __bf16 q1 = (__bf16)r1;
        const float r2 = r1 - (float)q1;
        const __bf16 q2 = (__bf16)r2;
        h[0][j] = __builtin_bit_cast(unsigned short, q0);
        h[1][j] = __builtin_bit_cast(unsigned short, q1);
        h[2][j] = __builtin_bit_cast(unsigned short, q2);
    }
    constexpr int WPL = H ? 2 : 3;
    const size_t frag = (i >> 6) * WPL;
#pragma unroll
    for (int pl = 0; pl < WPL; ++pl) {
        uint4 o;
        o.x = h[pl][0] | ((unsigned)h[pl][1] << 16);
        o.y = h[pl][2] | ((unsigned)h[pl][3] << 16);
        o.z = h[pl][4] | ((unsigned)h[pl][5] << 16);
        o.w = h[pl][6] | ((unsigned)h[pl][7] << 16);
        out[(frag + pl) * 64 + lane] = o;
    }
}

template <int WM, int WN, bool H = false, bool SEG2 = false>
__global__ __launch_bounds__(64 * WM * WN, 512 / (64 * WM * WN)) void conv_split_gemm_kernel(SplitArgs a) {
    static_assert(H || !SEG2, "the second K segment exists in the fp16 form only");
    constexpr int XP = H ? 2 : 3;
    constexpr int WPL = H ? 2 : 3;
    constexpr int NT = 64 * WM * WN, NWAVE = WM * WN;
    constexpr int BM = 128 * WM, BN = 64 * WN;
    constexpr int XS = BM * 4 / NT;
    constexpr int WU = BN * 2 * WPL;
    constexpr int NPp = BM + 4;
    constexpr int XPLANE = 2 * NPp * 16;
    constexpr int XBYTES = XP * XPLANE, STAGE = XBYTES + WU * 16;
    extern __shared__ __attribute__((aligned(16))) unsigned char smem[];
    const int tid = threadIdx.x;
    const int lane = tid & 63;
    const int wave = tid >> 6;
    const int wm = wave / WN, wn = wave % WN;
    unsigned bx = blockIdx.x, by = blockIdx.y;
    PP_TL_DECL;
    PP_TL_MARK(0);
    if (a.xcd_remap) {
        if (!xcd_tile_column(blockIdx.x, a, bx, by)) return;
    }
    const unsigned L = bx, col = by;
    (void)L; (void)col;
    const long long m0 = (long long)bx * BM;
    const int cbB = by * (BN / 32);
    const int cb0 = cbB + wn * 2;

    const unsigned mfirst = (unsigned)min(m0 + wm * 128, a.S - 1), mlast = (unsigned)min(m0 + wm * 128 + 127, a.S - 1);
    const int img_first = __builtin_amdgcn_readfirstlane((int)pp_udiv(mfirst, a.dv_per)), img_last = __builtin_amdgcn_readfirstlane((int)pp_udiv(mlast, a.dv_per));
    unsigned oam_first = 0;
    if constexpr (H) oam_first = a.x_amax[img_first];
    if constexpr (SEG2) oam_first = max(oam_first, a.x2_amax[img_first]);
    const unsigned lds_base0 = (unsigned)(size_t)(__attribute__((address_space(3))) unsigned char*)smem;
    const size_t wstep0 = (size_t)a.ncb * (WPL * 64);
    f32x16 acc[2][4];
    if constexpr (H) {
    constexpr int XR = 3, XSTG = BM * 64, WR = 3, WBYTES = WU * 16;
    constexpr int NXD = BM / 16 / NWAVE;
    constexpr int NWD = WU / 64 / NWAVE;
    static_assert(BM / 16 % NWAVE == 0 && WU / 64 % NWAVE == 0, "every wave issues the same number of DMAs (vmcnt arithmetic)");
    unsigned gx[NXD];
#pragma unroll
    for (int i = 0; i < NXD; ++i) {
        const int pl = (wave + NWAVE * i) * 16 + (lane >> 2);
        const unsigned m = (unsigned)min(m0 + pl, a.S - 1);
        const int img = (int)pp_udiv(m, a.dv_per), rem = (int)(m - (unsigned)img * (unsigned)(a.H * a.W));
        const int ho = (int)pp_udiv((unsigned)rem, a.dv_row), wo = rem - ho * a.W;
        gx[i] = (unsigned)(((img * a.xp_h + ho * a.stride) * a.xp_w + wo * a.stride) * a.Cin) * 4u + (unsigned)(((lane & 3) ^ ((pl >> 1) & 3)) * 16);
    }
    unsigned gx2[SEG2 ? NXD : 1];
    if constexpr (SEG2) {
#pragma unroll
        for (int i = 0; i < NXD; ++i) {
            const int pl = (wave + NWAVE * i) * 16 + (lane >> 2);
            const unsigned m = (unsigned)min(m0 + pl, a.S - 1);
            const int img = (int)pp_udiv(m, a.dv_per), rem = (int)(m - (unsigned)img * (unsigned)(a.H * a.W));
            const int ho = (int)pp_udiv((unsigned)rem, a.dv_row), wo = rem - ho * a.W;
            gx2[i] = (unsigned)(((img * a.xp2_h + ho * a.stride2) * a.xp2_w + wo * a.stride2) * a.Cin2) * 4u + (unsigned)(((lane & 3) ^ ((pl >> 1) & 3)) * 16);
        }
    }
    float xsc[4];
#pragma unroll
    for (int pb = 0; pb < 4; ++pb) xsc[pb] = pp_act_scale(oam_first);
    if (img_first != img_last) {
#pragma unroll
        for (int pb = 0; pb < 4; ++pb) {
// ... 561 lines not shown
#pragma unroll
        for (int j = 0; j < STEM_SLOTS; ++j) {
            const int p = tid + 512 * j;
            uint2 p0, p1;
            split4h(xr[j], sx, p0, p1);
            if (p >= STEM_PH * STEM_PW) continue;
            unsigned char* d = pbase + buf * STEM_BUF + p * 8;
            *reinterpret_cast<uint2*>(d) = p0;
            *reinterpret_cast<uint2*>(d + STEM_PLANE) = p1;
        }
    };

    const int xofs = ((4 * wave) * STEM_PW + 2 * px + 2 * hk) * 8;
    const unsigned char* const wlane = wl + lane * 16;
    const int rdrow = lane >> 3, rdc = lane & 7;
    float bias_l[2][4], wsc_l[2][4];
#pragma unroll
    for (int cb = 0; cb < 2; ++cb) {
        const float4 b = *reinterpret_cast<const float4*>(a.bias + cb * 32 + 4 * rdc);
        const float4 c = *reinterpret_cast<const float4*>(a.wscale + cb * 32 + 4 * rdc);
        bias_l[cb][0] = b.x; bias_l[cb][1] = b.y; bias_l[cb][2] = b.z; bias_l[cb][3] = b.w;
        wsc_l[cb][0] = c.x; wsc_l[cb][1] = c.y; wsc_l[cb][2] = c.z; wsc_l[cb][3] = c.w;
    }

    int t = blockIdx.x;
    if (t >= a.ntiles) return;
    load_patch(t);
    {
        const float sx = pp_act_scale(a.x_amax[tn]);
        store_patch(0, sx);
    }
    __syncthreads();
    int it = 0;
    for (; t < a.ntiles; t += gridDim.x, ++it) {
        const int buf = it & 1;
        int n, y0, x0;
        locate(t, n, y0, x0);
        const unsigned am = a.x_amax[n];
        const int tnext = t + (int)gridDim.x;
        const bool more = tnext < a.ntiles;
        unsigned am_next = 0;
        if (more) {
            load_patch(tnext);
            am_next = a.x_amax[tn];
        }
        f32x16 acc[2][2];
#pragma unroll
        for (int cb = 0; cb < 2; ++cb)
#pragma unroll
            for (int pb = 0; pb < 2; ++pb)
#pragma unroll
                for (int i = 0; i < 16; ++i) acc[cb][pb][i] = 0.f;
        const unsigned char* const pl = pbase + buf * STEM_BUF + xofs;
        uint4 wf[2][2][2], xf[2][2][2];
        auto load_frags = [&](int s, int set) {
#pragma unroll
            for (int cb = 0; cb < 2; ++cb)
#pragma unroll
                for (int pn = 0; pn < 2; ++pn) wf[set][cb][pn] = *reinterpret_cast<const uint4*>(wlane + ((s * 2 + cb) * 2 + pn) * 1024);
#pragma unroll
            for (int pb = 0; pb < 2; ++pb)
#pragma unroll
                for (int pn = 0; pn < 2; ++pn)
                    xf[set][pb][pn] = *reinterpret_cast<const uint4*>(pl + pn * STEM_PLANE + ((2 * pb + (s >> 1)) * STEM_PW + (s & 1) * 4) * 8);
        };
        load_frags(0, 0);
#pragma unroll
        for (int s = 0; s < STEM_STEPS; ++s) {
            if (s == STEM_STEPS / 2 && more) store_patch(buf ^ 1, pp_act_scale(am_next));
            if (s + 1 < STEM_STEPS) load_frags(s + 1, (s + 1) & 1);
            __builtin_amdgcn_sched_barrier(0);
            constexpr int WI[3] = {1, 0, 0}, XI[3] = {0, 1, 0};
#pragma unroll
            for (int p = 0; p < 3; ++p)
#pragma unroll
                for (int pb = 0; pb < 2; ++pb)
#pragma unroll
                    for (int cb = 0; cb < 2; ++cb)
                        acc[cb][pb] = __builtin_amdgcn_mfma_f32_32x32x16_f16(__builtin_bit_cast(f16x8, wf[s & 1][cb][WI[p]]),
                                                                             __builtin_bit_cast(f16x8, xf[s & 1][pb][XI[p]]), acc[cb][pb], 0, 0, 0);
            __builtin_amdgcn_sched_barrier(0);
        }
        __syncthreads();

        const float xinv = pp_act_unscale(am);
        unsigned char* const stg = pbase + buf * STEM_BUF + wave * 4096;
        float ymax = 0.f;
#pragma unroll
        for (int pb = 0; pb < 2; ++pb) {
            const int oy = y0 + 2 * wave + pb;
#pragma unroll
            for (int cb = 0; cb < 2; ++cb) {
#pragma unroll
                for (int g = 0; g < 4; ++g) {
                    const float4 v = make_float4(acc[cb][pb][4 * g], acc[cb][pb][4 * g + 1], acc[cb][pb][4 * g + 2], acc[cb][pb][4 * g + 3]);
                    *reinterpret_cast<float4*>(stg + px * 128 + (((2 * g + hk) ^ (px & 7)) << 4)) = v;
                }
                asm volatile("s_waitcnt lgkmcnt(0)" ::: "memory");
#pragma unroll
                for (int r4 = 0; r4 < 4; ++r4) {
                    const int r = r4 * 8 + rdrow, ox = x0 + r;
                    const float4 c = *reinterpret_cast<const float4*>(stg + r * 128 + ((rdc ^ (r & 7)) << 4));
                    float4 v = make_float4(__builtin_fmaf(c.x, wsc_l[cb][0] * xinv, bias_l[cb][0]), __builtin_fmaf(c.y, wsc_l[cb][1] * xinv, bias_l[cb][1]),
                                           __builtin_fmaf(c.z, wsc_l[cb][2] * xinv, bias_l[cb][2]), __builtin_fmaf(c.w, wsc_l[cb][3] * xinv, bias_l[cb][3]));
                    if (a.relu != PP_RELU_NONE) { v.x = fmaxf(v.x, 0.f); v.y = fmaxf(v.y, 0.f); v.z = fmaxf(v.z, 0.f); v.w = fmaxf(v.w, 0.f); }
                    if (oy < a.Hout && ox < a.Wout) {
                        *reinterpret_cast<float4*>(a.y + (((size_t)n * (a.Hout + a.y_pad) + oy) * (a.Wout + a.y_pad) + ox) * 64 + cb * 32 + 4 * rdc) = v;
                        ymax = fmaxf(ymax, pp_abs4max(v));
                    }
                }
                asm volatile("s_waitcnt lgkmcnt(0)" ::: "memory");
            }
        }
        if (a.y_amax) {
            const int img[1] = {n};
            const float m[1] = {ymax};
            pp_amax_commit_wg<8, 1>(a.y_amax, img, m, n, n, red);
        }
        __syncthreads();
    }
}

__global__ __launch_bounds__(256) void split_weights_stem7_kernel(const float* w, uint4* out, int CoutPad, const float* cmax) {
    const int i = blockIdx.x * 256 + threadIdx.x;
    if (i >= STEM_STEPS * 2 * 64) return;
    const int lane = i & 63, cb = (i >> 6) & 1, s = i >> 7;
    const int cout = cb * 32 + (lane & 31);
    unsigned short h[2][8];
#pragma unroll
    for (int j = 0; j < 8; ++j) {
        const int dy = s >> 1, dx = 4 * (s & 1) + 2 * (lane >> 5) + (j >> 2), c = j & 3;
        float v = 0.f;
        if (dx < 7) {
            const int k = (dy * 7 + dx) * 4 + c;
            v = w[((size_t)(k >> 5) * CoutPad + cout) * 32 + 8 * (k & 3) + ((k & 31) >> 2)];
        }
        unsigned short q2;
        split_weight_h(v, channel_scale(cmax[cout]), h[0][j], h[1][j], q2);
    }
#pragma unroll
    for (int pn = 0; pn < 2; ++pn) {
        uint4 o;
        o.x = h[pn][0] | ((unsigned)h[pn][1] << 16);
        o.y = h[pn][2] | ((unsigned)h[pn][3] << 16);
        o.z = h[pn][4] | ((unsigned)h[pn][5] << 16);
        o.w = h[pn][6] | ((unsigned)h[pn][7] << 16);
        out[(size_t)(((s * 2 + cb) * 2 + pn) * 64 + lane)] = o;
    }
}

}


static TileGeom tap_tiling(const ConvArgs& a, int nw, int stream_env) {
    const int max_np = nw == 8 ? 768 : 512, xp_h = a.Hin + a.x_pad, xp_w = a.Win + a.x_pad;
    TileGeom g = pick_tile(a.Hout, a.Wout, max_np, nw / 2);
    g.mode = MODE_TILE;
    const int snp = 64 * nw + 2 + 2 * xp_w;
    const double stream_eff = (double)a.Hout * a.Wout / ((double)xp_h * xp_w);
    bool use_stream = a.x_pad >= 1 && snp <= max_np && (g.eff < 0 || stream_eff > g.eff + 0.02);
    if (stream_env == 0 && g.eff >= 0) use_stream = false;
    if (stream_env == 1 && a.x_pad >= 1 && snp <= max_np) use_stream = true;
    if (use_stream) {
        g.mode = MODE_STREAM;
        g.PWp = xp_w;
        g.NP = g.NPp = snp;
        while (g.NPp % 8 != 4) ++g.NPp;
    }
    return g;
}

SplitPlan pp_conv_split_plan(const ConvArgs& a) {
    static const int stem7_on = env_int("POSEPIPE_SPLIT_STEM7", 1);
    static const int s2_on = env_int("POSEPIPE_SPLIT_S2", 1), s2p_on = env_int("POSEPIPE_SPLIT_S2P", 1);
    static const int gemm8_on = env_int("POSEPIPE_SPLIT_GEMM8", 1), gemm4_min_c = env_int("POSEPIPE_SPLIT_GEMM4_MIN_C", 64);
    static const int gemm_min_cin = env_int("POSEPIPE_SPLIT_GEMM_MIN_CIN", 1024);
    static const int c48_on = env_int("POSEPIPE_SPLIT_C48", 1), c48_mult = env_int("POSEPIPE_SPLIT_C48_MULT", 0);
    static const int stream_env = env_int("POSEPIPE_SPLIT_STREAM", -1);
    const char* s2_env = getenv("POSEPIPE_SPLIT_S2_MIN_CIN");
    SplitPlan p;
    p.f16 = a.split_f16 != 0;
    const size_t wpl = p.f16 ? 2 : 3;
    p.ncb = (a.Cout + 31) / 32;
    p.nout = p.ncb * 32;
    if (stem7_on && p.f16 && a.KH == 7 && a.KW == 7 && a.stride == 2 && a.pad_h == 3 && a.pad_w == 3 && a.dil_h == 1 && a.dil_w == 1 &&
        a.Cin == 4 && a.Cout == 64 && a.CoutPad >= 64 && a.up_log2 == 0 && !a.out_nchw && !a.res1 && !a.res2 &&
        (a.relu == PP_RELU_NONE || a.relu == PP_RELU_FIRST || a.relu == PP_RELU_LAST) && (a.y_stride == 0 || a.y_stride == a.Cout) &&
        a.y_coff == 0 && a.Hout == (a.Hin - 1) / 2 + 1 && a.Wout == (a.Win - 1) / 2 + 1) {
        p.kernel = SPLIT_STEM7;
        p.cin = a.Cin;
        p.frag_bytes = STEM_WBYTES;
        p.bytes = p.frag_bytes + (size_t)2 * p.nout * sizeof(float);
        return p;
    }
    const bool k3 = a.KH == 3 && a.KW == 3 && a.stride == 1 && a.pad_h == 1 && a.pad_w == 1 && a.dil_h == 1 && a.dil_w == 1 &&
                    a.Hout == a.Hin && a.Wout == a.Win;
    const bool k1 = a.KH == 1 && a.KW == 1 && a.pad_h == 0 && a.pad_w == 0;
    const bool full = a.KH == a.Hin && a.KW == a.Win && a.pad_h == 0 && a.pad_w == 0 && a.dil_h == 1 && a.dil_w == 1 &&
                      a.x_pad == 0 && a.Hout == 1 && a.Wout == 1 && !k1;
    const bool s2_pick = s2_env ? a.Cin >= atoi(s2_env) : p.f16 ? (a.Cin >= 96 || (a.Cin >= 48 && p.ncb >= 6)) : (a.Cin >= 128 && (p.ncb & 1) == 0);
    const bool s2_shape = a.KH == 3 && a.KW == 3 && a.stride == 2 && a.pad_h == 1 && a.pad_w == 1 && a.dil_h == 1 && a.dil_w == 1 && !full;
    const bool s2p_map = a.Hout * a.Wout >= 1500 || (a.Hout * a.Wout >= 400 && a.Cout >= 96);
    const bool s2p = s2p_on && p.f16 && s2_shape && s2p_map;
    const bool k3s2 = s2_on && s2_shape && (s2_pick || s2p);
    if (!(k3 || k1 || full || k3s2)) return p;
    p.taps = (k3 || k3s2) ? 9 : 1;
    p.cin = full ? a.K : a.Cin;
    const bool product = gemm8_on && p.taps == 1 && p.cin >= gemm4_min_c && a.Cout % 128 == 0;
    const bool one_column = p.f16 && p.cin >= 256 && a.Cout > 32 && a.Cout <= 64 && a.HWout >= 4096;
    if (p.taps == 1 && p.cin < gemm_min_cin && !one_column && !product) return p;
    const bool res1_plain = !a.res1 || (a.res1_off_w == 0 && a.res1_shift >= 0 && a.res1_shift <= 4 &&
                                        ((a.Hout - 1) >> a.res1_shift) < a.res1_H && ((a.Wout - 1) >> a.res1_shift) < a.res1_W &&
                                        (a.res1_shift > 0 || (a.res1_H == a.Hout && a.res1_W == a.Wout)));
    if (!(p.cin % 16 == 0 && a.Cout % 4 == 0 && a.up_log2 == 0 && !a.out_nchw && res1_plain && a.relu <= PP_ACT_SWISH &&
          (a.y_stride == 0 || a.y_stride == a.Cout) && a.y_coff == 0))
        return p;
    const bool c48 = c48_on && k3 && ((a.Cout > 32 && a.Cout <= 48) || (c48_mult == 1 && a.Cout % 48 == 0) || (c48_mult == 2 && a.Cout == 192));
    if (a.Cin2 > 0) {
        if (!(product && p.f16 && k1 && a.stride == 1 && !a.res1 && a.Cin2 % 16 == 0 && a.stride2 >= 1 && a.x_pad == 0 && a.x2_pad == 0 &&
              (a.Hout - 1) * a.stride2 < a.Hin2 && (a.Wout - 1) * a.stride2 < a.Win2))
            return SplitPlan();
        p.cin2 = a.Cin2;
    }
    size_t steps = (size_t)((p.cin + p.cin2) / 16) * p.taps;
    if (product) {
        p.kernel = SPLIT_PRODUCT;
    } else if (!k3 && !s2p) {
        p.kernel = p.taps > 1 ? SPLIT_TAP_GATHER : SPLIT_ONE_TAP;
        p.tile[0].mode = MODE_GEMM;
        p.tile[0].NP = 256;
        p.tile[0].NPp = 260;
    } else if (s2p) {
        p.kernel = SPLIT_S2P;
        p.tile[0] = pick_tile_s2(a.Hout, a.Wout, 13 * 64);
        p.tile[0].mode = MODE_TILE;
    } else if (c48) {
        p.kernel = SPLIT_C48;
        p.ncb = (a.Cout + 47) / 48 * 3;
        p.nout = p.ncb * 16;
        steps = (size_t)(p.cin / 16) * 5;
        p.tile[0] = tap_tiling(a, 4, stream_env);
    } else {
        p.kernel = SPLIT_TAP3;
        p.tile[0] = tap_tiling(a, 4, stream_env);
        p.tile[1] = tap_tiling(a, 8, stream_env);
    }
    p.frag_bytes = (steps + 1) * p.ncb * wpl * 64 * sizeof(uint4);
    p.bytes = p.frag_bytes + (p.f16 ? (size_t)2 * p.nout * sizeof(float) : 0);
    if (p.cin2 > 0) {
        p.bias_off = (p.bytes + 15) / 16 * 16;
        p.bytes = p.bias_off + (size_t)a.CoutPad * sizeof(float);
    }
    return p;
}

static int split_weights_folded(const SplitPlan& p, const ConvArgs& a, void* out, hipStream_t stream) {
    const int kcat = p.cin + p.cin2, kpad = (kcat + 31) / 32 * 32;
    const size_t total = (size_t)kpad * a.CoutPad;
    float* cat = nullptr;
    PP_HIP_CHECK(hipMalloc((void**)&cat, total * sizeof(float)));
    hipLaunchKernelGGL(concat_weights_kernel, dim3((unsigned)((total + 255) / 256)), dim3(256), 0, stream, a.w, a.w2, cat, p.cin, p.cin2, a.CoutPad, total);
    SplitPlan q = p;
    q.cin = kcat;
    q.cin2 = 0;
    ConvArgs b = a;
    b.w = cat;
    b.Cin = kcat; b.K = kcat; b.Kpad = kpad;
    int rc = pp_conv_split_weights(q, b, out, stream);
    std::vector<float> b0(a.CoutPad), b1(a.CoutPad);
    hipError_t e = hipStreamSynchronize(stream);
    if (e == hipSuccess) e = hipMemcpy(b0.data(), a.bias, b0.size() * sizeof(float), hipMemcpyDeviceToHost);
    if (e == hipSuccess) e = hipMemcpy(b1.data(), a.bias2, b1.size() * sizeof(float), hipMemcpyDeviceToHost);
    for (size_t i = 0; i < b0.size(); ++i) b0[i] += b1[i];
    if (e == hipSuccess) e = hipMemcpy(static_cast<unsigned char*>(out) + p.bias_off, b0.data(), b0.size() * sizeof(float), hipMemcpyHostToDevice);
    (void)hipFree(cat);
    if (rc == PP_OK && e != hipSuccess) {
        pp_set_error("split_weights (folded shortcut) failed: %s", hipGetErrorString(e));
        rc = PP_ERR_HIP;
    }
    return rc;
}

int pp_conv_split_weights(const SplitPlan& p, const ConvArgs& a, void* out, hipStream_t stream) {
    if (p.cin2 > 0) return split_weights_folded(p, a, out, stream);
    float* cmax = nullptr;
    if (p.f16) {
        float* inv_scale = reinterpret_cast<float*>(static_cast<unsigned char*>(out) + p.frag_bytes);
        cmax = inv_scale + p.nout;
        hipLaunchKernelGGL(weight_channel_max_kernel, dim3((unsigned)p.nout), dim3(64), 0, stream, a.w, a.Kpad / 32, a.CoutPad, p.nout, cmax, inv_scale);
    }
    const char* what = "split_weights";
    if (p.kernel == SPLIT_STEM7) {
        what = "split_weights_stem7";
        hipLaunchKernelGGL(split_weights_stem7_kernel, dim3((STEM_STEPS * 2 * 64 + 255) / 256), dim3(256), 0, stream, a.w, (uint4*)out, a.CoutPad, cmax);
    } else if (p.kernel == SPLIT_C48) {
        what = "split_weights48";
        const size_t total = (size_t)(p.cin / 16) * 5 * p.ncb * 64;
        const dim3 grid((unsigned)((total + 255) / 256));
        if (p.f16) hipLaunchKernelGGL(split_weights48_kernel<true>, grid, dim3(256), 0, stream, a.w, (uint4*)out, p.cin, a.CoutPad, p.ncb, total, cmax);
        else hipLaunchKernelGGL(split_weights48_kernel<false>, grid, dim3(256), 0, stream, a.w, (uint4*)out, p.cin, a.CoutPad, p.ncb, total, cmax);
    } else {
        const size_t total = (size_t)(p.cin / 16) * p.taps * p.ncb * 64;
        const dim3 grid((unsigned)((total + 255) / 256));
        if (p.f16) hipLaunchKernelGGL(split_weights_kernel<true>, grid, dim3(256), 0, stream, a.w, (uint4*)out, p.cin, p.taps, a.CoutPad, p.ncb, total, cmax);
        else hipLaunchKernelGGL(split_weights_kernel<false>, grid, dim3(256), 0, stream, a.w, (uint4*)out, p.cin, p.taps, a.CoutPad, p.ncb, total, cmax);
    }
    hipError_t e = hipGetLastError();
    if (e != hipSuccess) {
        pp_set_error("%s launch failed: %s", what, hipGetErrorString(e));
        return PP_ERR_HIP;
    }
    return PP_OK;
}

__global__ __launch_bounds__(256) void amax_kernel(const float4* x, size_t quads, unsigned per, unsigned* amax) {
    const unsigned n = blockIdx.x / per, part = blockIdx.x - n * per;
    const float4* xs = x + (size_t)n * quads;
    float m = 0.f;
    for (size_t i = (size_t)part * 256 + threadIdx.x; i < quads; i += (size_t)per * 256) m = fmaxf(m, pp_abs4max(xs[i]));
    __shared__ float red[16];
    const int im[1] = {(int)n};
    const float mm[1] = {m};
    pp_amax_commit_wg<4, 1>(amax, im, mm, (int)n, (int)n, red);
}

int pp_launch_amax(const float* x, int n, size_t elems, unsigned* amax, hipStream_t stream) {
    if (n <= 0 || elems == 0) return PP_OK;
    if (elems % 4 != 0) {
        pp_set_error("amax: %zu floats per sample (a multiple of 4 is required)", elems);
        return PP_ERR_ARG;
    }
    const size_t quads = elems / 4;
    const unsigned per = (unsigned)std::min<size_t>(std::max<size_t>((quads + 1023) / 1024, 1), std::max<size_t>(2048 / (size_t)n, 1));
    hipLaunchKernelGGL(amax_kernel, dim3(per * (unsigned)n), dim3(256), 0, stream, (const float4*)x, quads, per, amax);
    hipError_t e = hipGetLastError();
    if (e != hipSuccess) {
        pp_set_error("amax launch failed: %s", hipGetErrorString(e));
        return PP_ERR_HIP;
    }
    return PP_OK;
}

#ifdef PP_SPLIT_TIMELINE
static unsigned long long* tl_buf = nullptr;
static const size_t TL_MAX_WG = 1 << 19;
static unsigned long long* tl_begin(const ConvArgs& a, hipStream_t stream) {
    static const char* path = getenv("POSEPIPE_SPLIT_TIMELINE");
    static const int only_cin = env_int("POSEPIPE_SPLIT_TIMELINE_CIN", 0);
    static const int max_launches = env_int("POSEPIPE_SPLIT_TIMELINE_MAX", 300);
    static int recorded = 0;
    if (!path || (only_cin && a.Cin != only_cin) || recorded >= max_launches) return nullptr;
    ++recorded;
    if (!tl_buf && hipMalloc(&tl_buf, TL_MAX_WG * 128) != hipSuccess) return nullptr;
    (void)hipMemsetAsync(tl_buf, 0, TL_MAX_WG * 128, stream);
    return tl_buf;
}
static void tl_end(const ConvArgs& a, const SplitArgs& s, const char* kernel, unsigned nwg, hipStream_t stream) {
    if (!s.dbg) return;
    (void)hipStreamSynchronize(stream);
    nwg = std::min<unsigned>(nwg, TL_MAX_WG);
    std::vector<unsigned long long> h((size_t)nwg * 16);
    (void)hipMemcpy(h.data(), tl_buf, h.size() * 8, hipMemcpyDeviceToHost);
    static int launch = 0;
    FILE* f = fopen(getenv("POSEPIPE_SPLIT_TIMELINE"), "ab");
    if (!f) return;
    long long hdr[16] = {0x54494d454c494e45ll, launch++, (long long)nwg, a.N, a.Hout, a.Wout, a.Cin, a.Cout, s.mode, s.nchunks, s.gx, s.gy,
                         a.res1 != nullptr, a.res2 != nullptr, 0, 0};
    memcpy(&hdr[14], kernel, std::min<size_t>(strlen(kernel), 15));
    fwrite(hdr, 8, 16, f);
    fwrite(h.data(), 8, h.size(), f);
    fclose(f);
}
#define PP_TL_BEGIN() s.dbg = tl_begin(a, stream)
#define PP_TL_END(name, nwg) tl_end(a, s, name, nwg, stream)
#else
#define PP_TL_BEGIN()
#define PP_TL_END(name, nwg)
#endif

static void fill_divisors(SplitArgs& s) {
    const bool stream_mode = s.mode == MODE_STREAM;
    make_magic(stream_mode ? (unsigned)(s.xp_h * s.PWp) : (unsigned)(s.H * s.W), s.dv_per);
    make_magic(stream_mode ? (unsigned)s.PWp : (unsigned)s.W, s.dv_row);
    make_magic((unsigned)std::max(s.tiles_x, 1), s.dv_tx);
    make_magic((unsigned)std::max(s.tiles_y, 1), s.dv_ty);
    make_magic((unsigned)std::max(s.PWp, 1), s.dv_pw);
    make_magic((unsigned)std::max(s.gy, 1), s.dv_ncol);
    make_magic((unsigned)std::max(s.gx >> 3, 1), s.dv_run0);
    make_magic((unsigned)((s.gx >> 3) + 1), s.dv_run1);
    make_magic((unsigned)std::max(s.ktaps, 1), s.dv_ktaps);
    make_magic((unsigned)std::max(s.KW, 1), s.dv_kw);
}

template <auto K, int MAX_LDS, class Args>
static void launch_split(dim3 grid, unsigned threads, size_t lds, hipStream_t stream, const Args& s) {
    static PpPerDeviceOnce once;
    once.run([] { (void)hipFuncSetAttribute((const void*)K, hipFuncAttributeMaxDynamicSharedMemorySize, MAX_LDS); });
    hipLaunchKernelGGL(K, grid, dim3(threads), lds, stream, s);
}

template <int NS, int... MORE, class F>
static void with_nslot(int nslot, F&& f) {
    if constexpr (sizeof...(MORE) == 0) f(std::integral_constant<int, NS>());
    else if (nslot <= NS) f(std::integral_constant<int, NS>());
    else with_nslot<MORE...>(nslot, f);
}

template <int T, int NW, bool R4, int NS>
static void launch_tap(int cob, bool f16, dim3 grid, size_t lds, hipStream_t stream, const SplitArgs& s) {
    constexpr int L = (NW == 8 ? 160 : 100) * 1024;
    if constexpr (R4) {
        if (cob == 3) return launch_split<conv_split_kernel<9, NS, 3, 2, 4, true, true>, L>(grid, 256, lds, stream, s);
        if (cob == 4) return launch_split<conv_split_kernel<9, NS, 4, 2, 4, true, true>, L>(grid, 256, lds, stream, s);
    }
    if (f16 && cob == 2) launch_split<conv_split_kernel<T, NS, 2, 2, NW, R4, true>, L>(grid, 64 * NW, lds, stream, s);
    else if (f16) launch_split<conv_split_kernel<T, NS, 1, 2, NW, R4, true>, L>(grid, 64 * NW, lds, stream, s);
    else if (cob == 2) launch_split<conv_split_kernel<T, NS, 2, 2, NW, R4, false>, L>(grid, 64 * NW, lds, stream, s);
    else launch_split<conv_split_kernel<T, NS, 1, 2, NW, R4, false>, L>(grid, 64 * NW, lds, stream, s);
}

static unsigned apply_tiling(SplitArgs& s, const TileGeom& g, const ConvArgs& a, int nw) {
    s.mode = g.mode;
    s.NP = g.NP;
    s.NPp = g.NPp;
    if (g.mode == MODE_GEMM) {
        s.S = (long long)a.M;
        return (unsigned)((a.M + 255) / 256);
    }
    s.PWp = g.PWp;
    if (g.mode == MODE_STREAM) {
        s.S = (long long)a.N * s.xp_h * s.xp_w;
        return (unsigned)((s.S + 64 * nw - 1) / (64 * nw));
    }
    s.tiles_x = g.tiles_x; s.tiles_y = g.tiles_y; s.TH = g.TH; s.TW = g.TW; s.bw_log2 = g.bw_log2; s.gx_log2 = g.gx_log2;
    return (unsigned)(g.tiles_x * g.tiles_y * a.N);
}

static int launch_stem7(const ConvArgs& a, hipStream_t stream) {
    if (!a.x_amax) {
        pp_set_error("conv_split: the fp16 form needs the per-sample maximum of its input (ConvArgs::x_amax)");
        return PP_ERR_STATE;
    }
    StemArgs s{};
    s.x = a.x; s.w = (const uint4*)a.wsplit; s.bias = a.bias; s.y = a.y;
    s.wscale = reinterpret_cast<const float*>(static_cast<const unsigned char*>(a.wsplit) + STEM_WBYTES);
    s.x_amax = a.x_amax; s.y_amax = a.y_amax;
    s.N = a.N; s.Hin = a.Hin; s.Win = a.Win; s.xp_h = a.Hin + a.x_pad; s.xp_w = a.Win + a.x_pad;
    s.Hout = a.Hout; s.Wout = a.Wout; s.y_pad = a.y_pad; s.relu = a.relu;
    s.tiles_x = (a.Wout + STEM_TW - 1) / STEM_TW;
    s.tiles_y = (a.Hout + STEM_TH - 1) / STEM_TH;
    s.ntiles = a.N * s.tiles_x * s.tiles_y;
    s.x_bytes = a.x_bytes;
    make_magic((unsigned)s.tiles_x, s.dv_tx);
    make_magic((unsigned)s.tiles_y, s.dv_ty);
    static const int ncu = [] {
        int dev = 0, n = 256;
        if (hipGetDevice(&dev) == hipSuccess) (void)hipDeviceGetAttribute(&n, hipDeviceAttributeMultiprocessorCount, dev);
        return n > 0 ? n : 256;
    }();
    launch_split<conv_split_stem7_kernel, STEM_LDS>(dim3((unsigned)std::min(s.ntiles, ncu)), 512, STEM_LDS, stream, s);
    hipError_t e = hipGetLastError();
    if (e != hipSuccess) {
        pp_set_error("conv_split_stem7 launch failed: %s", hipGetErrorString(e));
        return PP_ERR_HIP;
    }
    return PP_OK;
}

int pp_launch_conv_split(const SplitPlan& p, const ConvArgs& a, hipStream_t stream) {
    if (a.wsplit && p.kernel == SPLIT_STEM7) return launch_stem7(a, stream);
    if (!a.wsplit || p.kernel == SPLIT_NONE) {
        pp_set_error("conv_split: layer not eligible");
        return PP_ERR_ARG;
    }
    static const int colmaj_mb = env_int("POSEPIPE_SPLIT_COLMAJOR_MB", 256), gemm_remap = env_int("POSEPIPE_SPLIT_GEMM_REMAP", 1);
    static const int epi_env = env_int("POSEPIPE_SPLIT_GEMM_EPI", 1);
    static const int cob2_env = env_int("POSEPIPE_SPLIT_S2_COB", 0), cob_env = env_int("POSEPIPE_SPLIT_COB", 0);
    static const int nw8_f16 = env_int("POSEPIPE_SPLIT_NW8_F16", 0);
    static const int nw8_min_blocks = env_int("POSEPIPE_SPLIT_NW8_MIN_BLOCKS", 512), nw8_min_chunks = env_int("POSEPIPE_SPLIT_NW8_MIN_CHUNKS", 16);
    static const int ring4_env = env_int("POSEPIPE_SPLIT_RING4", 1), ring48_env = env_int("POSEPIPE_SPLIT_RING48", 1);
    const bool full = p.cin != a.Cin;
    SplitArgs s{};
    s.x = a.x; s.w = (const uint4*)a.wsplit; s.bias = a.bias; s.res1 = a.res1; s.res2 = a.res2; s.y = a.y;
    s.N = a.N; s.H = a.Hout; s.W = a.Wout; s.Cin = p.cin; s.Cout = a.Cout;
    s.ncb = p.ncb;
    s.xp_h = full ? 1 : a.Hin + a.x_pad;
    s.xp_w = full ? 1 : a.Win + a.x_pad;
    s.stride = a.stride;
    s.y_pad = a.y_pad; s.r1_pad = a.r1_pad; s.r2_pad = a.r2_pad; s.relu = a.relu;
    s.r1_shift = a.res1 ? a.res1_shift : 0;
    s.r1_H = a.res1 ? a.res1_H : a.Hout;
    s.r1_W = a.res1 ? a.res1_W : a.Wout;
    s.nchunks = (p.cin + p.cin2) / 16;
    s.seg1 = p.cin / 16;
    if (p.cin2 > 0) {
        if (p.cin2 != a.Cin2 || !a.x2 || !a.x2_amax || p.kernel != SPLIT_PRODUCT || !p.f16 || a.res1) {
            pp_set_error("conv_split: the plan has a folded shortcut of %d channels, the launch does not match it", p.cin2);
            return PP_ERR_STATE;
        }
        s.x2 = a.x2; s.x2_amax = a.x2_amax; s.Cin2 = a.Cin2; s.stride2 = a.stride2;
        s.xp2_h = a.Hin2 + a.x2_pad; s.xp2_w = a.Win2 + a.x2_pad;
    }
    s.ktaps = 1; s.KW = a.KW; s.pad = a.pad_h; s.Hin = a.Hin; s.Win = a.Win;
    if (p.kernel == SPLIT_TAP_GATHER) {
        s.ktaps = p.taps;
        s.nchunks = (p.cin / 16) * p.taps;
    }
    s.x_bytes = a.x_bytes;
    s.xcd_remap = a.xcd_remap;
    const bool f16 = p.f16 != 0;
    const int xp = f16 ? 2 : 3;
    const int wpl = f16 ? 2 : 3;
    s.wscale = f16 ? reinterpret_cast<const float*>(static_cast<const unsigned char*>(a.wsplit) + p.frag_bytes) : nullptr;
    s.x_amax = a.x_amax;
    s.y_amax = a.y_amax;
    if (f16 && !a.x_amax) {
        pp_set_error("conv_split: the fp16 form needs the per-sample maximum of its input (ConvArgs::x_amax)");
        return PP_ERR_STATE;
    }
    PP_TL_BEGIN();
    s.col_major = (size_t)a.x_bytes <= (size_t)colmaj_mb << 20;
    const char* tag;
    dim3 grid;
    if (p.kernel == SPLIT_PRODUCT) {
        s.mode = MODE_GEMM;
        s.S = (long long)a.M;
        s.col_major = 0;
        const int BM = 256, BN = 128;
        grid = dim3((unsigned)((a.M + BM - 1) / BM), (unsigned)(a.Cout / BN));
        s.gx = (int)grid.x; s.gy = (int)grid.y;
        s.xcd_remap = gemm_remap && s.gy > 1;
        if (s.xcd_remap) grid = dim3((unsigned)((s.gx + 7) / 8 * 8 * s.gy), 1);
        const int epi_knob = g_split_gemm_epi.load(std::memory_order_relaxed);
        s.epi_lds = epi_knob >= 0 ? epi_knob : epi_env;
        const int nwave = 4;
        fill_divisors(s);
        const size_t lds_loop = f16 ? (size_t)3 * BM * 64 + (size_t)3 * BN * 2 * wpl * 16 : (size_t)2 * (xp * 2 * (BM + 4) * 16 + BN * 2 * wpl * 16);
        const size_t lds = std::max<size_t>(lds_loop, s.epi_lds ? (size_t)nwave * (16384 + 2048) : 0);
        if (p.cin2 > 0) launch_split<conv_split_gemm_kernel<2, 2, true, true>, 80 * 1024>(grid, 256, lds, stream, s);
        else if (f16) launch_split<conv_split_gemm_kernel<2, 2, true>, 80 * 1024>(grid, 256, lds, stream, s);
        else launch_split<conv_split_gemm_kernel<2, 2, false>, 80 * 1024>(grid, 256, lds, stream, s);
        tag = "g256x128";
    } else if (p.kernel == SPLIT_S2P) {
        if (p.tile[0].eff < 0) {
            pp_set_error("conv_split: no strided-patch tile for a %dx%d map", a.Hout, a.Wout);
            return PP_ERR_STATE;
        }
        const unsigned gx = apply_tiling(s, p.tile[0], a, 4);
        s.SP = (s.TH + 1) * s.PWp;
        int cob = 1;
        for (int c : {4, 3, 2})
            if (s.ncb % c == 0 && (size_t)2 * 2 * s.NPp * 16 + (size_t)4 * c * 2 * 1024 <= 80 * 1024 && (cob2_env == 0 || cob2_env == c)) {
                cob = c;
                break;
            }
        grid = dim3(gx, (unsigned)(s.ncb / cob));
        s.gx = (int)grid.x; s.gy = (int)grid.y;
        if (s.xcd_remap) grid = dim3((unsigned)((s.gx + 7) / 8 * 8 * s.gy), 1);
        fill_divisors(s);
        make_magic((unsigned)s.SP, s.dv_row);
        const size_t lds = (size_t)2 * 2 * s.NPp * 16 + (size_t)4 * cob * 2 * 1024;
        with_nslot<10, 11, 13>((s.NP + 63) / 64, [&](auto ns) {
            constexpr int NS = decltype(ns)::value, L = 100 * 1024;
            if (cob == 4) launch_split<conv_split_kernel<9, NS, 4, 1, 4, true, true, true>, L>(grid, 256, lds, stream, s);
            else if (cob == 3) launch_split<conv_split_kernel<9, NS, 3, 1, 4, true, true, true>, L>(grid, 256, lds, stream, s);
            else if (cob == 2) launch_split<conv_split_kernel<9, NS, 2, 1, 4, true, true, true>, L>(grid, 256, lds, stream, s);
            else launch_split<conv_split_kernel<9, NS, 1, 1, 4, true, true, true>, L>(grid, 256, lds, stream, s);
        });
        tag = "s2p";
    } else if (p.kernel == SPLIT_C48) {
        const unsigned gx = apply_tiling(s, p.tile[0], a, 4);
        s.gx = (int)gx;
        s.gy = s.ncb / 3;
        grid = s.xcd_remap ? dim3((unsigned)((s.gx + 7) / 8 * 8 * s.gy), 1) : dim3(gx, (unsigned)s.gy);
        fill_divisors(s);
        const size_t patch48 = (size_t)2 * xp * 2 * s.NPp * 16;
        const bool ring48 = f16 && ring48_env && patch48 + (size_t)4 * 3 * wpl * 1024 <= 80 * 1024;
        const size_t lds = patch48 + (ring48 ? (size_t)4 * 3 * wpl * 1024 : 0);
        with_nslot<5, 6, 7, 8>((s.NP + 63) / 64, [&](auto ns) {
            constexpr int NS = decltype(ns)::value, L = 100 * 1024;
            if (ring48) launch_split<conv_split48_kernel<NS, true, true>, L>(grid, 256, lds, stream, s);
            else if (f16) launch_split<conv_split48_kernel<NS, true, false>, L>(grid, 256, lds, stream, s);
            else launch_split<conv_split48_kernel<NS, false, false>, L>(grid, 256, lds, stream, s);
        });
        tag = "c48";
    } else {
        const bool tap3 = p.kernel == SPLIT_TAP3;
        int cob = (s.ncb & 1) ? 1 : 2;
        if (tap3 && f16 && s.ncb % 3 == 0 && (cob_env == 0 || cob_env == 3)) cob = 3;
        else if (tap3 && f16 && s.ncb % 4 == 0 && (cob_env == 0 || cob_env == 4)) cob = 4;
        int nw = tap3 && (!f16 || nw8_f16) ? 8 : 4;
        unsigned gx = apply_tiling(s, p.tile[nw == 8], a, nw);
        if (nw == 8 && !((long)gx * (s.ncb / cob) >= nw8_min_blocks && s.nchunks >= nw8_min_chunks)) {
            nw = 4;
            gx = apply_tiling(s, p.tile[0], a, nw);
        }
        const int nslot = (s.NP + 16 * nw - 1) / (16 * nw);
        const auto ring_fits = [&](int c) {
            return ring4_env && nw == 4 && s.mode != MODE_GEMM && (size_t)xp * 2 * s.NPp * 16 + (size_t)4 * c * wpl * 1024 <= 80 * 1024;
        };
        if (cob >= 3 && !(ring_fits(cob) && (cob_env >= 3 || (long)gx * (s.ncb / cob) >= 400))) cob = (s.ncb & 1) ? 1 : 2;
        const bool ring = ring_fits(cob);
        grid = dim3(gx, (unsigned)(s.ncb / cob));
        s.gx = (int)grid.x; s.gy = (int)grid.y;
        if (s.xcd_remap) grid = dim3((unsigned)((s.gx + 7) / 8 * 8 * s.gy), 1);
        const size_t lds = (size_t)(ring ? 1 : 2) * xp * 2 * s.NPp * 16 + ((nw == 8 || ring) ? (size_t)4 * cob * wpl * 1024 : 0);
        fill_divisors(s);
        if (s.mode == MODE_GEMM) launch_tap<1, 4, false, 4>(cob, f16, grid, lds, stream, s);
        else if (nw == 8) with_nslot<5, 6>(nslot, [&](auto ns) { launch_tap<9, 8, false, decltype(ns)::value>(cob, f16, grid, lds, stream, s); });
        else if (ring) with_nslot<5, 6, 7, 8>(nslot, [&](auto ns) { launch_tap<9, 4, true, decltype(ns)::value>(cob, f16, grid, lds, stream, s); });
        else with_nslot<5, 6, 7, 8>(nslot, [&](auto ns) { launch_tap<9, 4, false, decltype(ns)::value>(cob, f16, grid, lds, stream, s); });
        tag = s.mode == MODE_GEMM ? "gemm4" : nw == 8 ? "nw8" : ring ? "ring4" : "nw4";
    }
    PP_TL_END(tag, grid.x * grid.y);
    hipError_t e = hipGetLastError();
    if (e != hipSuccess) {
        pp_set_error("conv_split (%s) launch failed: %s", tag, hipGetErrorString(e));
        return PP_ERR_HIP;
    }
    return PP_OK;
}
```

### posepipeline_amd/csrc/net.hip

```cpp
#include <algorithm>
#include <memory>

#include "pp_internal.h"
#include "pp_amax.h"

struct pp_net {
    pp_ctx* ctx = nullptr;
    std::vector<pp_op> ops;
    std::vector<pp_buf> bufs;
    std::vector<size_t> buf_off;
    std::vector<size_t> buf_elems;
    float* weights = nullptr;
    size_t n_weights = 0;
    unsigned char* wsplit = nullptr;
    std::vector<SplitPlan> split_plan;
    int numerics = PP_NET_NUMERICS_EXACT;
    int split_f16 = 0;
    unsigned* amax = nullptr;
    std::vector<int> op_x_slot, op_y_slot, op_post_slot, slot_owner;
    std::vector<int> op_x2_slot;
    std::vector<int> fold_into, fold_src;
    bool folded(int i) const { return !fold_into.empty() && fold_into[i] >= 0; }
    int carries(int i) const { return fold_src.empty() ? -1 : fold_src[i]; }
    void reads(int i, int (&r)[5]) const {
// ... 741 lines not shown
    for (auto& e : net->ext)
        if (e.buf == buf) e.provided = false;
}

unsigned* pp_net_input_amax_slot(pp_net* net, int buf) {
    if (!net || !net->amax) return nullptr;
    for (auto& e : net->ext)
        if (e.buf == buf) return net->amax_slot(e.slot);
    return nullptr;
}

extern "C" {

int pp_net_create(pp_ctx* ctx, const pp_op* ops, int n_ops, const pp_buf* bufs, int n_bufs,
                  const float* weights, size_t n_weights, int max_batch, pp_net** out) {
    return pp_net_create_mem(ctx, ops, n_ops, bufs, n_bufs, weights, n_weights, PP_MEM_HOST, max_batch, out);
}

int pp_net_create_mem(pp_ctx* ctx, const pp_op* ops, int n_ops, const pp_buf* bufs, int n_bufs,
                      const float* weights, size_t n_weights, int weights_mem, int max_batch, pp_net** out) {
    return pp_net_create_ex(ctx, ops, n_ops, bufs, n_bufs, weights, n_weights, weights_mem, max_batch, PP_NET_NUMERICS_DEFAULT, out);
}

int pp_net_numerics(pp_net* net) { return net ? net->numerics : PP_ERR_ARG; }
int pp_net_split_kind(pp_net* net) {
    if (!net) return PP_ERR_ARG;
    return net->numerics != PP_NET_NUMERICS_SPLIT ? PP_NET_NUMERICS_EXACT : net->split_f16 ? PP_NET_NUMERICS_SPLIT_F16 : PP_NET_NUMERICS_SPLIT_BF16;
}

int pp_net_create_ex(pp_ctx* ctx, const pp_op* ops, int n_ops, const pp_buf* bufs, int n_bufs,
                     const float* weights, size_t n_weights, int weights_mem, int max_batch, int numerics, pp_net** out) {
    PP_REQUIRE(ctx && ops && bufs && weights && out, "pp_net_create: NULL argument");
    PP_REQUIRE(numerics >= PP_NET_NUMERICS_DEFAULT && numerics <= PP_NET_NUMERICS_SPLIT_F16, "pp_net_create_ex: bad numerics %d", numerics);
    PP_REQUIRE(weights_mem == PP_MEM_HOST || weights_mem == PP_MEM_DEVICE, "pp_net_create: bad weights_mem %d", weights_mem);
    PP_REQUIRE(n_ops > 0 && n_bufs > 0 && max_batch > 0, "pp_net_create: empty program");
    *out = nullptr;
    std::unique_ptr<pp_net> net(new pp_net());
    net->ctx = ctx;
    net->ops.assign(ops, ops + n_ops);
    net->bufs.assign(bufs, bufs + n_bufs);
    net->max_batch = max_batch;
    net->n_weights = n_weights;
    net->numerics = numerics != PP_NET_NUMERICS_DEFAULT ? numerics : (pp_conv_split_enabled() ? PP_NET_NUMERICS_SPLIT : PP_NET_NUMERICS_EXACT);
    if (net->numerics >= PP_NET_NUMERICS_SPLIT) {
        net->split_f16 = net->numerics == PP_NET_NUMERICS_SPLIT ? pp_conv_split_f16_default() : net->numerics == PP_NET_NUMERICS_SPLIT_F16;
        net->numerics = PP_NET_NUMERICS_SPLIT;
    }
    size_t off = 0;
    for (int b = 0; b < n_bufs; ++b) {
        PP_REQUIRE(bufs[b].h > 0 && bufs[b].w > 0 && bufs[b].c > 0 && bufs[b].pad >= 0 && bufs[b].pad <= 8, "buffer %d has an empty dim / bad halo", b);
        const size_t e = (size_t)(bufs[b].h + bufs[b].pad) * (bufs[b].w + bufs[b].pad) * bufs[b].c;
        net->buf_elems.push_back(e);
        net->buf_off.push_back(off);
        off += (e * max_batch + 63) / 64 * 64;
    }
    net->arena_floats = off;
    for (int i = 0; i < n_ops; ++i) PP_TRY(net_check_op(*net, net->ops[i], i));
    PP_HIP_CHECK(hipSetDevice(ctx->device));
    PP_HIP_CHECK(hipMalloc((void**)&net->weights, n_weights * sizeof(float)));
    PP_HIP_CHECK(hipMemcpyAsync(net->weights, weights, n_weights * sizeof(float),
                                weights_mem == PP_MEM_HOST ? hipMemcpyHostToDevice : hipMemcpyDeviceToDevice, ctx->stream));
    PP_HIP_CHECK(hipMalloc((void**)&net->arena, net->arena_floats * sizeof(float)));
    PP_HIP_CHECK(hipMemsetAsync(net->arena, 0, net->arena_floats * sizeof(float), ctx->stream));
    net->vits.assign(n_ops, nullptr);
    net->deconvs.assign(n_ops, nullptr);
    for (int i = 0; i < n_ops; ++i) {
        const pp_op& op = net->ops[i];
        const pp_buf& bi = net->bufs[op.in];
        if (op.type == PP_OP_DECONV_BF16)
            PP_TRY(pp_deconv_bf16_create(net->weights + op.w_off, net->weights + op.b_off, bi.h, bi.w, op.cin, op.cout, max_batch,
                                         ctx->stream, &net->deconvs[i]));
        if (op.type == PP_OP_VIT_ENCODER)
            PP_TRY(pp_vit_encoder_create(net->weights + op.w_off, bi.h * bi.w, op.cin, op.kh, op.kw, op.cin * op.stride, max_batch,
                                         ctx->stream, &net->vits[i]));
    }
    net->split_plan.assign(n_ops, SplitPlan());
    if (net->numerics == PP_NET_NUMERICS_SPLIT) {
        size_t bytes = 0;
        for (int i = 0; i < n_ops; ++i) {
            if (net->ops[i].type != PP_OP_CONV) continue;
            SplitPlan p = pp_conv_split_plan(net_conv_args(net.get(), i, 1));
            if (p.kernel == SPLIT_NONE) continue;
            net->split_plan[i] = p;
        }
        net_fold_shortcuts(net.get());
        for (int i = 0; i < n_ops; ++i) {
            SplitPlan& p = net->split_plan[i];
            if (p.kernel == SPLIT_NONE) continue;
            p.off = (long long)bytes;
            bytes += (p.bytes + 255) / 256 * 256;
        }
        net_plan_amax(net.get());
        if (!net->slot_owner.empty()) {
            const size_t ab = net->slot_owner.size() * (size_t)max_batch * sizeof(unsigned);
            PP_HIP_CHECK(hipMalloc((void**)&net->amax, ab));
            PP_HIP_CHECK(hipMemsetAsync(net->amax, 0, ab, ctx->stream));
        }
        if (bytes) {
            PP_HIP_CHECK(hipMalloc((void**)&net->wsplit, bytes));
            for (int i = 0; i < n_ops; ++i) {
                const SplitPlan& p = net->split_plan[i];
                if (p.kernel == SPLIT_NONE) continue;
                ConvArgs ca = net_conv_args(net.get(), i, 1);
                ca.bias = net->weights + net->ops[i].b_off;
                PP_TRY(pp_conv_split_weights(p, ca, net->wsplit + p.off, ctx->stream));
            }
        }
    }
    PP_HIP_CHECK(hipStreamSynchronize(ctx->stream));
    for (int i = 0; i < n_ops; ++i)
        if (net->ops[i].type == PP_OP_CONV) PP_TRY(pp_conv_prepare(net_conv_args(net.get(), i, 1)));
    const char* env_lanes = getenv("POSEPIPE_NET_LANES");
    PP_TRY(net_make_lanes(net.get(), env_lanes ? atoi(env_lanes) : 4));
    *out = net.release();
    return PP_OK;
}

static int net_make_lanes(pp_net* net, int n_lanes) {
    net->drop_lanes();
    const int n_ops = (int)net->ops.size();
    if (n_lanes > 1 && n_ops >= 8) {
        net_plan_lanes(net, n_lanes);
        net->lanes.resize(n_lanes);
        for (auto& l : net->lanes) PP_HIP_CHECK(hipStreamCreateWithFlags(&l, hipStreamNonBlocking));
        net->op_done.assign(n_ops, nullptr);
        for (int i = 0; i < n_ops; ++i)
            if (net->op_needs_event[i]) PP_HIP_CHECK(hipEventCreateWithFlags(&net->op_done[i], hipEventDisableTiming));
        PP_HIP_CHECK(hipEventCreateWithFlags(&net->fork_ev, hipEventDisableTiming));
        net->join_ev.resize(n_lanes);
        for (auto& e : net->join_ev) PP_HIP_CHECK(hipEventCreateWithFlags(&e, hipEventDisableTiming));
    }
    return PP_OK;
}

int pp_net_input_amax(pp_net* net, int buf, void** dptr) {
    PP_REQUIRE(net && dptr && buf >= 0 && buf < (int)net->bufs.size(), "pp_net_input_amax: bad argument");
    *dptr = nullptr;
    for (auto& e : net->ext)
        if (e.buf == buf && net->amax) {
            e.provided = true;
            *dptr = net->amax_slot(e.slot);
        }
    return PP_OK;
}

int pp_net_conv_kinds(pp_net* net, int* kinds) {
    PP_REQUIRE(net && kinds, "pp_net_conv_kinds: NULL argument");
    for (size_t i = 0; i < net->ops.size(); ++i) {
        kinds[i] = net->ops[i].type != PP_OP_CONV ? 0 : net->split_plan[i].kernel != SPLIT_NONE || net->folded((int)i) ? 2 : 1;
    }
    return PP_OK;
}

int pp_net_folded_into(pp_net* net, int* into) {
    PP_REQUIRE(net && into, "pp_net_folded_into: NULL argument");
    for (size_t i = 0; i < net->ops.size(); ++i) into[i] = net->folded((int)i) ? net->fold_into[i] : -1;
    return PP_OK;
}

void pp_net_destroy(pp_net* net) { delete net; }

int pp_net_buffer(pp_net* net, int buf, void** dptr, size_t* bytes_per_sample) {
    PP_REQUIRE(net && buf >= 0 && buf < (int)net->bufs.size(), "pp_net_buffer: bad buffer id");
    PP_REQUIRE(net->bufs[buf].pad == 0, "pp_net_buffer: buffer %d has a zero halo (conv-internal layout); expose dense buffers only", buf);
    if (dptr) *dptr = net->buf_ptr(buf);
    if (bytes_per_sample) *bytes_per_sample = net->buf_elems[buf] * sizeof(float);
    return PP_OK;
}

int pp_net_run(pp_net* net, int batch, int first_op, int last_op) {
    PP_REQUIRE(net, "pp_net_run: net is NULL");
    PP_REQUIRE(batch > 0 && batch <= net->max_batch, "pp_net_run: batch %d not in (0,%d]", batch, net->max_batch);
    if (last_op < 0) last_op = (int)net->ops.size();
    PP_REQUIRE(first_op >= 0 && last_op <= (int)net->ops.size() && first_op <= last_op, "pp_net_run: bad op range");
    if (net->graph_exec && batch == net->graph_batch && first_op == 0 && last_op == (int)net->ops.size()) {
        PP_HIP_CHECK(hipGraphLaunch(net->graph_exec, net->ctx->stream));
        return PP_OK;
    }
    hipStream_t main = net->ctx->stream;
    PpRange range("pp_net_run");
    PP_TRY(net_reset_amax(net, first_op, last_op, batch, main));
    if (net->lanes.empty() || !net->use_lanes || last_op - first_op < 8) {
        for (int i = first_op; i < last_op; ++i) PP_TRY(net_launch_op(net, i, batch, main));
        return PP_OK;
    }
    PP_HIP_CHECK(hipEventRecord(net->fork_ev, main));
    for (hipStream_t l : net->lanes) PP_HIP_CHECK(hipStreamWaitEvent(l, net->fork_ev, 0));
    for (int i = first_op; i < last_op; ++i) {
        hipStream_t s = net->lanes[net->op_lane[i]];
        for (int d : net->op_waits[i])
            if (d >= first_op) PP_HIP_CHECK(hipStreamWaitEvent(s, net->op_done[d], 0));
        PP_TRY(net_launch_op(net, i, batch, s));
        if (net->op_needs_event[i]) PP_HIP_CHECK(hipEventRecord(net->op_done[i], s));
    }
    for (size_t l = 0; l < net->lanes.size(); ++l) {
        PP_HIP_CHECK(hipEventRecord(net->join_ev[l], net->lanes[l]));
        PP_HIP_CHECK(hipStreamWaitEvent(main, net->join_ev[l], 0));
    }
    return PP_OK;
}

int pp_net_vit_timing(pp_net* net, int enable, float* ms3, int* n_gemm) {
    PP_REQUIRE(net, "pp_net_vit_timing: net is NULL");
    for (auto* v : net->vits) {
        if (!v) continue;
        if (ms3) {
            PP_HIP_CHECK(hipStreamSynchronize(net->ctx->stream));
            PP_TRY(pp_vit_encoder_get_timing(v, ms3, n_gemm));
        }
        pp_vit_encoder_set_timing(v, enable);
        return PP_OK;
    }
    pp_set_error("pp_net_vit_timing: the program has no PP_OP_VIT_ENCODER");
    return PP_ERR_STATE;
}

int pp_net_set_lane_count(pp_net* net, int n_lanes) {
    PP_REQUIRE(net && n_lanes >= 1 && n_lanes <= 16, "pp_net_set_lane_count: net is NULL or n_lanes not in [1, 16]");
    PP_HIP_CHECK(hipStreamSynchronize(net->ctx->stream));
    for (auto l : net->lanes) PP_HIP_CHECK(hipStreamSynchronize(l));
    if (net->graph_exec) {
        PP_HIP_CHECK(hipGraphExecDestroy(net->graph_exec));
        net->graph_exec = nullptr;
    }
    return net_make_lanes(net, n_lanes);
}

int pp_net_set_lanes(pp_net* net, int enable) {
    PP_REQUIRE(net, "pp_net_set_lanes: net is NULL");
    PP_HIP_CHECK(hipStreamSynchronize(net->ctx->stream));
    net->use_lanes = enable != 0;
    return PP_OK;
}

int pp_net_capture(pp_net* net, int batch) {
    PP_REQUIRE(net, "pp_net_capture: net is NULL");
    PP_REQUIRE(batch > 0 && batch <= net->max_batch, "pp_net_capture: bad batch");
    if (net->graph_exec) {
        PP_HIP_CHECK(hipGraphExecDestroy(net->graph_exec));
        net->graph_exec = nullptr;
    }
    hipStream_t s = net->ctx->stream;
    PP_HIP_CHECK(hipStreamSynchronize(s));
    hipGraph_t graph = nullptr;
    PP_HIP_CHECK(hipStreamBeginCapture(s, hipStreamCaptureModeThreadLocal));
    int rc = net_reset_amax(net, 0, (int)net->ops.size(), batch, s);
    for (int i = 0; i < (int)net->ops.size() && rc == PP_OK; ++i) rc = net_launch_op(net, i, batch, s);
    hipError_t e = hipStreamEndCapture(s, &graph);
    if (rc != PP_OK) {
        if (graph) (void)hipGraphDestroy(graph);
        return rc;
    }
    PP_HIP_CHECK(e);
    PP_HIP_CHECK(hipGraphInstantiate(&net->graph_exec, graph, nullptr, nullptr, 0));
    PP_HIP_CHECK(hipGraphDestroy(graph));
    net->graph_batch = batch;
    return PP_OK;
}

int pp_net_forward(pp_net* net, int batch, int in_buf, const float* in, int out_buf, float* out, int mem) {
    PP_REQUIRE(net && in && out, "pp_net_forward: NULL argument");
    PP_REQUIRE(in_buf >= 0 && in_buf < (int)net->bufs.size() && out_buf >= 0 && out_buf < (int)net->bufs.size(),
               "pp_net_forward: bad buffer id");
    PP_REQUIRE(batch > 0 && batch <= net->max_batch, "pp_net_forward: batch %d not in (0,%d]", batch, net->max_batch);
    PP_REQUIRE(net->bufs[in_buf].pad == 0 && net->bufs[out_buf].pad == 0, "pp_net_forward: input / output buffers must be dense (pad 0)");
    hipStream_t s = net->ctx->stream;
    const hipMemcpyKind kin = mem == PP_MEM_HOST ? hipMemcpyHostToDevice : hipMemcpyDeviceToDevice;
    const hipMemcpyKind kout = mem == PP_MEM_HOST ? hipMemcpyDeviceToHost : hipMemcpyDeviceToDevice;
    PP_HIP_CHECK(hipMemcpyAsync(net->buf_ptr(in_buf), in, (size_t)batch * net->buf_elems[in_buf] * sizeof(float), kin, s));
    pp_net_void_input_amax(net, in_buf);
    PP_TRY(pp_net_run(net, batch, 0, (int)net->ops.size()));
    PP_HIP_CHECK(hipMemcpyAsync(out, net->buf_ptr(out_buf), (size_t)batch * net->buf_elems[out_buf] * sizeof(float), kout, s));
    PP_HIP_CHECK(hipStreamSynchronize(s));
    return PP_OK;
}

int pp_net_profile(pp_net* net, int batch, float* ms_per_op) {
    PP_REQUIRE(net, "pp_net_profile: net is NULL");
    PP_REQUIRE(batch > 0 && batch <= net->max_batch, "pp_net_profile: bad batch");
    hipStream_t s = net->ctx->stream;
    const int n = (int)net->ops.size();
    std::vector<hipEvent_t> ev(n + 1, nullptr);
    auto timed_run = [&]() -> int {
        for (auto& e : ev) PP_HIP_CHECK(hipEventCreate(&e));
        int rc = net_reset_amax(net, 0, n, batch, s);
        PP_HIP_CHECK(hipEventRecord(ev[0], s));
        for (int i = 0; i < n && rc == PP_OK; ++i) {
            rc = net_launch_op(net, i, batch, s);
            if (rc == PP_OK && hipEventRecord(ev[i + 1], s) != hipSuccess) rc = PP_ERR_HIP;
        }
        if (rc == PP_OK && hipStreamSynchronize(s) != hipSuccess) rc = PP_ERR_HIP;
        return rc;
    };
    const int rc = timed_run();
    if (rc == PP_OK && ms_per_op) {
        for (int i = 0; i < n; ++i) {
            float ms = 0.f;
            (void)hipEventElapsedTime(&ms, ev[i], ev[i + 1]);
            ms_per_op[i] = ms;
        }
    }
    for (auto e : ev)
        if (e) (void)hipEventDestroy(e);
    return rc;
}

// ... 2 lines not shown
```

### posepipeline_amd/csrc/pp_internal.h

```cpp
#pragma once
#include <hip/hip_runtime.h>
#include <cstdarg>
#include <cstdio>
#include <cstring>
#include <string>
#include <vector>
#include <mutex>

#include "posepipe_hip.h"

void pp_set_error(const char* fmt, ...);

#define PP_HIP_CHECK(expr)                                                              \
    do {                                                                                \
        hipError_t _e = (expr);                                                         \
        if (_e != hipSuccess) {                                                         \
            pp_set_error("%s failed: %s (%s:%d)", #expr, hipGetErrorString(_e), __FILE__, \
                         __LINE__);                                                     \
            return PP_ERR_HIP;                                                          \
        }                                                                               \
    } while (0)

#define PP_REQUIRE(cond, ...)            \
    do {                                 \
        if (!(cond)) {                   \
            pp_set_error(__VA_ARGS__);   \
            return PP_ERR_ARG;           \
        }                                \
    } while (0)

struct PpPerDeviceOnce {
    std::mutex m;
    unsigned long long done = 0;
    template <class F> void run(F&& f) {
        int dev = 0;
        (void)hipGetDevice(&dev);
        std::lock_guard<std::mutex> g(m);
        if ((done >> (dev & 63)) & 1ull) return;
        f();
        done |= 1ull << (dev & 63);
    }
};

struct pp_ctx {
    int device = 0;
    hipStream_t stream = nullptr;
    bool own_stream = true;
    hipEvent_t ev_start = nullptr, ev_stop = nullptr;
    hipStream_t copy_stream = nullptr;
    hipEvent_t ev_upload = nullptr;
    hipEvent_t ev_consumed = nullptr;
    void* scratch = nullptr;
    size_t scratch_bytes = 0;
    int ensure_scratch(size_t bytes);
};

struct ScratchCursor {
    pp_ctx* ctx;
    size_t off = 0;
    explicit ScratchCursor(pp_ctx* c) : ctx(c) {}
    static size_t align(size_t b) { return (b + 255) & ~size_t(255); }
    template <class T>
    T* take(size_t count) {
        T* p = reinterpret_cast<T*>(static_cast<char*>(ctx->scratch) + off);
        off += align(count * sizeof(T));
        return p;
    }
};

void pp_range_push(const char* name);
void pp_range_pop();
struct PpRange {
    explicit PpRange(const char* name) { pp_range_push(name); }
    ~PpRange() { pp_range_pop(); }
    PpRange(const PpRange&) = delete;
    PpRange& operator=(const PpRange&) = delete;
};
struct PpStages {
    bool open = false;
    void next(const char* name) {
        if (open) pp_range_pop();
        open = name != nullptr;
        if (open) pp_range_push(name);
    }
    ~PpStages() { next(nullptr); }
};

struct ConvArgs {
    const float* x;
    const float* w;
    const float* bias;
    const float* res1;
    const float* res2;
    float* y;
    int N, Hin, Win, Cin, Hout, Wout, Cout, CoutPad;
    int KH, KW, stride, pad_h, pad_w, dil_h, dil_w;
    int K, Kpad, M, HWout;
    unsigned div_hw_m, div_hw_s1, div_hw_s2, div_w_m, div_w_s1, div_w_s2;
    unsigned div_c_m, div_c_s1, div_c_s2, div_kw_m, div_kw_s1, div_kw_s2;
    int xcd_remap;
    unsigned x_bytes;
    int relu, up_log2, out_nchw;
    int res1_shift, res1_off_w, res1_H, res1_W;
    int y_stride, y_coff;
    const uint2* tap_table;
    int x_pad, y_pad, r1_pad, r2_pad;
    int no_bounds;
    const void* wsplit;
    int numerics;
    int split_f16;
    const unsigned* x_amax;
    unsigned* y_amax;
    const float* x2;
    const float* w2;
    const float* bias2;
    const unsigned* x2_amax;
    int Cin2, Hin2, Win2, stride2, x2_pad;
};
struct TileGeom {
    int TH, TW, bw_log2, gx_log2, PWp, NP, NPp, tiles_x, tiles_y;
    double eff;
    int mode;
};
enum SplitKernel {
    SPLIT_NONE = 0,
    SPLIT_STEM7,
    SPLIT_PRODUCT,
    SPLIT_C48,
    SPLIT_TAP3,
    SPLIT_S2P,
    SPLIT_ONE_TAP,
    SPLIT_TAP_GATHER,
};
struct SplitPlan {
    int kernel = SPLIT_NONE;
    int f16 = 0;
    int taps = 1, cin = 0;
    int cin2 = 0;
    size_t bias_off = 0;
    int ncb = 0;
    int nout = 0;
    size_t frag_bytes = 0;
    size_t bytes = 0;
    TileGeom tile[2] = {};
    long long off = -1;
};
SplitPlan pp_conv_split_plan(const ConvArgs& a);
int pp_conv_split_weights(const SplitPlan& p, const ConvArgs& a, void* out, hipStream_t stream);
int pp_launch_conv_split(const SplitPlan& p, const ConvArgs& a, hipStream_t stream);
bool pp_conv_tracks_amax(const ConvArgs& a, bool split);
bool pp_conv_split_enabled();
bool pp_conv_split_f16_default();
int pp_conv_prepare(const ConvArgs& a);
int pp_conv_out_dim(int in, int k, int stride, int pad, int dil);
int pp_launch_conv(const ConvArgs& a, const SplitPlan* plan, hipStream_t stream);
int pp_launch_conv_p3(const ConvArgs& a, int ct, int pt, hipStream_t stream, bool fake_addresses = false);

struct PoolArgs {
    const float* x;
    float* y;
    int N, Hin, Win, C, Hout, Wout, KH, KW, stride, pad_h, pad_w;
    int x_stride, x_coff, y_stride, y_coff;
};
int pp_launch_maxpool(const PoolArgs& a, hipStream_t stream);
int pp_launch_avgpool(const float* x, float* y, int n, int hin, int win, int c, int kh, int kw, int stride, hipStream_t stream);

struct GemmArgs {
    const void* A;
    const void* B;
    const float* bias;
    const float* res;
    void* C;
    int M, N, K;
    int act;
    int out_bf16;
    int res_mod;
    int group_m;
    int qkv_tokens, qkv_hd;
};
int pp_launch_gemm_bf16(const GemmArgs& a, hipStream_t stream);
int pp_gemm_bf16_prepare();
struct pp_deconv_bf16;
int pp_deconv_bf16_create(const float* weights, const float* bias, int h, int w, int cin, int cout, int max_batch,
                          hipStream_t stream, pp_deconv_bf16** out);
void pp_deconv_bf16_destroy(pp_deconv_bf16* d);
int pp_deconv_bf16_run(pp_deconv_bf16* d, const float* x, float* out, int batch, int relu, hipStream_t stream);
int pp_launch_f32_to_bf16(const float* x, void* y, size_t n, hipStream_t stream);
int pp_launch_nv12_to_bgr(const unsigned char* nv12, unsigned char* bgr, int frames, int h, int w, hipStream_t stream);
int pp_launch_layernorm(const float* x, const float* pos, int pos_mod, float* x_out, const float* gamma,
                        const float* beta, int rows, int dim, float eps, void* y, int out_bf16, hipStream_t stream);
int pp_launch_attention(const void* qkv, int batch, int tokens, int heads, int head_dim, void* out, hipStream_t stream,
                        int head_major = 0);
int pp_launch_depth_to_space(const float* x, float* y, int n, int h, int w, int c, hipStream_t stream);
int pp_launch_upsample_add(const float* t, const float* res1, const float* res2, float* y, int n, int H, int W, int c,
                           int up_log2, int relu, hipStream_t stream, const float* t2 = nullptr, int up2 = 0,
                           const float* t3 = nullptr, int up3 = 0, unsigned* y_amax = nullptr);
int pp_launch_bilinear_add(const float* t, const float* res1, float* y, int n, int H, int W, int c, int y_stride, int y_coff,
                           int up_log2, int relu, hipStream_t stream, const float* t2 = nullptr, int up2 = 0,
                           const float* t3 = nullptr, int up3 = 0, unsigned* y_amax = nullptr);
int pp_launch_dwconv3x3(const float* x, const float* w, const float* bias, float* y, int n, int hin, int win, int c, int stride,
                        int act, int gelu_in, hipStream_t stream);
int pp_launch_layernorm_nhwc(const float* x, const float* gamma, const float* beta_eps, float* y, size_t rows, int c_real,
                             int c_buf, hipStream_t stream);
int pp_launch_gelu_add(const float* x, const float* res, float* y, size_t elems, hipStream_t stream);
int pp_launch_window_attn(const float* qkv, const float* table, const float* bias, float* out, int n, int h, int w, int c_real,
                          int c_buf, int heads, hipStream_t stream);
int pp_window_attn_max_head_dim();
int pp_launch_attention_f32(const float* qkv, float* out, int batch, int tokens, int heads, int c_real, int c_buf, hipStream_t stream);
int pp_attention_f32_max_tokens();
int pp_attention_f32_max_head_dim();
int pp_launch_dcn3x3(const float* x, const float* om, const float* wgt, const float* bias, float* y, int n, int h, int w, int cin,
                     int cout, int om_c, int relu, hipStream_t stream);
int pp_dcn3x3_max_cout();
int pp_launch_dwdeconv(const float* x, const float* wgt, const float* res, float* y, int n, int h, int w, int c, int stride,
                       hipStream_t stream);
int pp_launch_sub_cat(const float* a, const float* b, const float* lead, float* y, size_t pixels, int c, int c2, hipStream_t stream);
int pp_launch_bcast_mul(const float* x, const float* g, float* y, size_t pixels, int c, hipStream_t stream);
int pp_launch_blend2(const float* x0, const float* x1, const float* l0, const float* l1, float* y, size_t pixels, int c, hipStream_t stream);
int pp_launch_graph_mix(const float* x, const float* amat, const float* bias_nb, float* y, int n, int h, int w, int g, int c,
                        int y_stride, int y_coff, int relu, hipStream_t stream);
int pp_launch_joint_attn(const float* qkv, float* out, int n, int h, int w, int heads, int c_real, int c_buf, int y_stride, int y_coff,
                         hipStream_t stream);
int pp_joint_attn_max_head_dim();
struct pp_vit_encoder;
size_t pp_vit_param_floats(int tokens, int dim, int depth, int hidden);
int pp_vit_encoder_create(const float* params, int tokens, int dim, int depth, int heads, int hidden, int max_batch,
                          hipStream_t stream, pp_vit_encoder** out);
void pp_vit_encoder_destroy(pp_vit_encoder* e);
int pp_vit_encoder_run(pp_vit_encoder* e, const float* in, float* out, int batch, hipStream_t stream);
void pp_vit_encoder_set_timing(pp_vit_encoder* e, int enable);
int pp_vit_encoder_get_timing(pp_vit_encoder* e, float ms3[3], int* n_gemm);

struct PersonXform {
    double a00, a01, b0, a10, a11, b1;
    int frame;
    int valid;
};
bool pp_person_transform(const double* bbox_tlwh, int out_w, int out_h, float center_scale[4], PersonXform* t, int udp = 0);
int pp_enqueue_crop(hipStream_t s, const uint8_t* frames, int h, int w, const PersonXform* xf, int n_person,
                    int out_w, int out_h, const float* lut, const int32_t chan_map[3], int flip, float* out,
                    uint8_t* crop_u8);
int pp_enqueue_flip_w(hipStream_t s, const float* src, float* dst, int n, int h, int w);

struct DecodeParams {
    int n, k, h, w;
    int shift_heatmap, post, blur_kernel;
};
int pp_enqueue_decode(hipStream_t s, const DecodeParams& p, const float* hm, const float* hm_flip,
                      const int32_t* flip_perm, const float* center_scale, float* kpts, float* merged);
```

### posepipeline_amd/program.py

```python
from __future__ import annotations

import ctypes as C
from dataclasses import dataclass, field

import numpy as np

from . import _lib as L


def fold_bn(weight, conv_bias, gamma, beta, mean, var, eps=1e-5):
    scale = gamma.astype(np.float64) / np.sqrt(var.astype(np.float64) + eps)
    w = weight.astype(np.float64) * scale.reshape((-1,) + (1,) * (weight.ndim - 1))
    b0 = np.zeros_like(scale) if conv_bias is None else conv_bias.astype(np.float64)
    b = beta.astype(np.float64) + (b0 - mean.astype(np.float64)) * scale
    return w.astype(np.float32), b.astype(np.float32)


def pack_conv(weight, bias, cin_pad=None):
    w = np.asarray(weight, dtype=np.float32)
    if w.ndim == 3:
        w = w[:, :, None, :]
    cout, cin, kh, kw = w.shape
    cin_p = cin_pad if cin_pad is not None else (cin + 3) // 4 * 4
    assert cin_p % 4 == 0 and cin_p >= cin
# ... 360 lines not shown
                for k in OPERAND_FIELDS + ("out",):
                    if op[k] >= 0:
                        ok[op[k]] = False
                continue
            o = op["out"]
            if op["out_nchw"] or op["out_c_off"] or self.vbufs[o].c != op["cout"]:
                ok[o] = False
            h, w, _ = self.dims(op["in_"])
            eh, ew = op["pad_end"] & 1, (op["pad_end"] >> 1) & 1
            ho = conv_out_dim(h, op["kh"], op["stride"], op["pad_h"], op["dil_h"], eh) - ((op["pad_end"] >> 2) & 1)
            wo = conv_out_dim(w, op["kw"], op["stride"], op["pad_w"], op["dil_w"], ew) - ((op["pad_end"] >> 3) & 1)
            over = max(op["pad_h"], op["pad_w"], (ho - 1) * op["stride"] - op["pad_h"] + (op["kh"] - 1) * op["dil_h"] - (h - 1),
                       (wo - 1) * op["stride"] - op["pad_w"] + (op["kw"] - 1) * op["dil_w"] - (w - 1))
            if over > 0:
                need[op["in_"]] = max(need[op["in_"]], over)
        return [need[v] if ok[v] and 0 < need[v] <= 2 else 0 for v in range(n_v)]

    def build(self) -> Program:
        n_v = len(self.vbufs)
        last_use = [-1] * n_v
        first_def = [None] * n_v
        for i, op in enumerate(self.vops):
            for key in OPERAND_FIELDS + ("out",):
                if op[key] >= 0:
                    last_use[op[key]] = i
            if first_def[op["out"]] is None:
                first_def[op["out"]] = i
        vpad = self._halo_plan()
        phys_dims: list[tuple] = []
        phys_pad: list[int] = []
        free: dict[tuple, list[int]] = {}
        v2p = [-1] * n_v
        for v, b in enumerate(self.vbufs):
            if b.pinned:
                phys_dims.append((b.h, b.w, b.c))
                phys_pad.append(0)
                v2p[v] = len(phys_dims) - 1
        for i, op in enumerate(self.vops):
            v = op["out"]
            if v2p[v] < 0:
                key = self.dims(v) + (vpad[v],)
                pool = free.get(key, [])
                busy = {v2p[op[k]] for k in OPERAND_FIELDS if op[k] >= 0}
                pick = next((p for p in pool if p not in busy), None)
                if pick is not None:
                    pool.remove(pick)
                    v2p[v] = pick
                else:
                    phys_dims.append(key[:3])
                    phys_pad.append(vpad[v])
                    v2p[v] = len(phys_dims) - 1
            for key in OPERAND_FIELDS + ("out",):
                u = op[key]
                if u >= 0 and last_use[u] == i and not self.vbufs[u].pinned and v2p[u] >= 0:
                    lst = free.setdefault(self.dims(u) + (vpad[u],), [])
                    if v2p[u] not in lst:
                        lst.append(v2p[u])
        ops = []
        for op in self.vops:
            rec = L.pp_op()
            for k, val in op.items():
                if k in ("name", "flops"):
                    continue
                if k == "out" or k in OPERAND_FIELDS:
                    val = v2p[val] if val >= 0 else -1
                setattr(rec, k, int(val))
            ops.append(rec)
        blob = np.concatenate(self.blob_parts) if self.blob_parts else np.zeros(4, np.float32)
        named = {k: v2p[v] for k, v in self.named.items()}
        return Program(ops=ops, bufs=phys_dims, buf_pad=phys_pad, blob=blob, named=named,
                       flops=float(sum(op["flops"] for op in self.vops)),
                       op_flops=[op["flops"] for op in self.vops], op_names=[op["name"] for op in self.vops],
                       param_offsets=dict(self.param_offsets))


class Net:

    def __init__(self, ctx: L.Context, prog: Program, max_batch: int, blob_dev=None, numerics=None):
        self.ctx = ctx
        self.prog = prog
        self.max_batch = int(max_batch)
        lib = ctx.lib
        n_ops = len(prog.ops)
        ops = (L.pp_op * n_ops)(*prog.ops)
        pads = prog.buf_pad or [0] * len(prog.bufs)
        bufs = (L.pp_buf * len(prog.bufs))(*[L.pp_buf(*d, p) for d, p in zip(prog.bufs, pads)])
        h = C.c_void_p()
        if blob_dev is not None:
            dptr, n_floats = blob_dev
            L.check(lib.pp_net_create_ex(ctx.handle, ops, n_ops, bufs, len(prog.bufs), C.c_void_p(int(dptr)), int(n_floats),
                                         L.PP_MEM_DEVICE, self.max_batch, L.NUMERICS[numerics], C.byref(h)), "pp_net_create_ex")
        else:
            blob = np.ascontiguousarray(prog.blob, dtype=np.float32)
            L.check(lib.pp_net_create_ex(ctx.handle, ops, n_ops, bufs, len(prog.bufs), L.ptr(blob), blob.size, L.PP_MEM_HOST,
                                         self.max_batch, L.NUMERICS[numerics], C.byref(h)), "pp_net_create_ex")
        self.handle = h
        self.numerics = "split" if lib.pp_net_numerics(h) == L.PP_NET_NUMERICS_SPLIT else "exact"
        self.split_kind = {L.PP_NET_NUMERICS_SPLIT_BF16: "split_bf16", L.PP_NET_NUMERICS_SPLIT_F16: "split_f16"}.get(lib.pp_net_split_kind(h), "exact")

    def close(self):
        if getattr(self, "handle", None):
            if getattr(self.ctx, "handle", None):
                self.ctx.lib.pp_net_destroy(self.handle)
            self.handle = None

    def __del__(self):
        try:
            self.close()
        except Exception:
            pass

    def buffer(self, name_or_id):
        pid = self.prog.named[name_or_id] if isinstance(name_or_id, str) else int(name_or_id)
        p = C.c_void_p()
        nb = C.c_size_t()
        L.check(self.ctx.lib.pp_net_buffer(self.handle, pid, C.byref(p), C.byref(nb)), "pp_net_buffer")
        return int(p.value), int(nb.value), self.prog.bufs[pid]

    def run(self, batch, first=0, last=None):
        last = len(self.prog.ops) if last is None else last
        L.check(self.ctx.lib.pp_net_run(self.handle, batch, first, last), "pp_net_run")

    def set_lanes(self, enable: bool):
        L.check(self.ctx.lib.pp_net_set_lanes(self.handle, int(bool(enable))), "pp_net_set_lanes")

    def set_lane_count(self, n_lanes: int):
        L.check(self.ctx.lib.pp_net_set_lane_count(self.handle, int(n_lanes)), "pp_net_set_lane_count")

    def capture(self, batch):
        L.check(self.ctx.lib.pp_net_capture(self.handle, batch), "pp_net_capture")

    def forward(self, x: np.ndarray, in_name="input", out_name="output") -> np.ndarray:
        x = np.ascontiguousarray(x, dtype=np.float32)
        n = x.shape[0]
        pin, pout = self.prog.named[in_name], self.prog.named[out_name]
        assert tuple(x.shape[1:]) == tuple(self.prog.bufs[pin]), (x.shape, self.prog.bufs[pin])
        oh, ow, oc = self.prog.bufs[pout]
        out = np.empty((n, oh, ow, oc), dtype=np.float32)
        L.check(self.ctx.lib.pp_net_forward(self.handle, n, pin, L.ptr(x), pout, L.ptr(out), L.PP_MEM_HOST),
                "pp_net_forward")
        return out

    def read(self, name_or_id, batch) -> np.ndarray:
        dptr, nb, (h, w, c) = self.buffer(name_or_id)
        out = np.empty((batch, h, w, c), dtype=np.float32)
        self.ctx.d2h(out, dptr)
        return out

    def conv_kinds(self) -> np.ndarray:
        kinds = np.zeros(len(self.prog.ops), dtype=np.int32)
        L.check(self.ctx.lib.pp_net_conv_kinds(self.handle, L.ptr(kinds)), "pp_net_conv_kinds")
        return kinds

    def folded_into(self) -> np.ndarray:
        into = np.zeros(len(self.prog.ops), dtype=np.int32)
        L.check(self.ctx.lib.pp_net_folded_into(self.handle, L.ptr(into)), "pp_net_folded_into")
        return into

    def profile(self, batch) -> np.ndarray:
        ms = np.zeros(len(self.prog.ops), dtype=np.float32)
        L.check(self.ctx.lib.pp_net_profile(self.handle, batch, L.ptr(ms)), "pp_net_profile")
        return ms
```

Before: 625.0.

## Add compact stream mode skipping padded pixels in split 3x3 conv kernels

Measured after the change: 628.9, median of 6. About the same (+0.6%).

```diff
diff --git a/include/posepipe_hip.h b/include/posepipe_hip.h
--- a/include/posepipe_hip.h
+++ b/include/posepipe_hip.h
@@ -126,6 +126,7 @@
 int pp_net_profile(pp_net* net, int batch, float* ms_per_op);
 int pp_net_conv_kinds(pp_net* net, int* kinds);
 int pp_net_folded_into(pp_net* net, int* into);
+int pp_net_conv_tiles(pp_net* net, int batch, int* tiles);
 
 int pp_conv_force(int ct, int pt);
 int pp_conv_variant(int variant);
diff --git a/posepipeline_amd/_lib.py b/posepipeline_amd/_lib.py
--- a/posepipeline_amd/_lib.py
+++ b/posepipeline_amd/_lib.py
@@ -114,6 +114,7 @@
     "pp_net_set_lanes": (_i, [_vp, _i]),
     "pp_net_set_lane_count": (_i, [_vp, _i]),
     "pp_net_conv_kinds": (_i, [_vp, _vp]),
+    "pp_net_conv_tiles": (_i, [_vp, _i, _vp]),
     "pp_net_folded_into": (_i, [_vp, _vp]),
     "pp_net_profile": (_i, [_vp, _i, _vp]),
     "pp_crop_resize_bilinear": (_i, [_vp, _vp, _i, _i, _i, _vp, _i, _i, _i, _vp]),
diff --git a/posepipeline_amd/csrc/api_core.hip b/posepipeline_amd/csrc/api_core.hip
--- a/posepipeline_amd/csrc/api_core.hip
+++ b/posepipeline_amd/csrc/api_core.hip
@@ -6,7 +6,7 @@
 #include "pp_internal.h"
 
 #include <atomic>
-extern std::atomic<int> g_decode_generic, g_split_gemm_epi;
+extern std::atomic<int> g_decode_generic, g_split_gemm_epi, g_split_stream_compact;
 
 static thread_local std::string g_last_error;
 
@@ -69,8 +69,9 @@
     PP_REQUIRE(name && value >= -1 && value <= 1, "pp_debug_knob: name and a value in {-1, 0, 1}");
     if (!strcmp(name, "decode_generic")) g_decode_generic.store(value, std::memory_order_relaxed);
     else if (!strcmp(name, "split_gemm_epilogue")) g_split_gemm_epi.store(value, std::memory_order_relaxed);
+    else if (!strcmp(name, "split_stream_compact")) g_split_stream_compact.store(value, std::memory_order_relaxed);
     else {
-        pp_set_error("pp_debug_knob: unknown knob '%s' (decode_generic, split_gemm_epilogue)", name);
+        pp_set_error("pp_debug_knob: unknown knob '%s' (decode_generic, split_gemm_epilogue, split_stream_compact)", name);
         return PP_ERR_ARG;
     }
     return PP_OK;
diff --git a/posepipeline_amd/csrc/conv_split.hip b/posepipeline_amd/csrc/conv_split.hip
--- a/posepipeline_amd/csrc/conv_split.hip
+++ b/posepipeline_amd/csrc/conv_split.hip
@@ -19,6 +19,7 @@
 typedef __attribute__((ext_vector_type(16))) float f32x16;
 
 std::atomic<int> g_split_gemm_epi{-1};
+std::atomic<int> g_split_stream_compact{-1};
 
 namespace {
 
@@ -41,6 +42,8 @@
     int r1_shift, r1_H, r1_W;
     int ktaps, KW, pad, Hin, Win;
     long long S;
+    long long Sx;
+    int compact;
     unsigned x_bytes;
     int xcd_remap;
     int SP;
@@ -49,6 +52,7 @@
     int epi_lds;
     unsigned dv_per[2], dv_row[2];
     unsigned dv_tx[2], dv_ty[2], dv_pw[2];
+    unsigned dv_vper[2], dv_vrow[2];
     unsigned dv_ncol[2], dv_run0[2], dv_run1[2];
     unsigned dv_ktaps[2], dv_kw[2];
     const float* wscale;
@@ -109,6 +113,14 @@
     return true;
 }
 
+__device__ __forceinline__ unsigned compact_pos(unsigned v, const SplitArgs& a, unsigned& img, unsigned& yy, unsigned& xx) {
+    img = pp_udiv(v, a.dv_vper);
+    const unsigned rem = v - img * (unsigned)(a.H * a.W);
+    yy = pp_udiv(rem, a.dv_vrow);
+    xx = rem - yy * (unsigned)a.W;
+    return (img * (unsigned)a.xp_h + yy) * (unsigned)a.PWp + xx;
+}
+
 typedef __attribute__((ext_vector_type(2))) __bf16 bf16x2_t;
 typedef __attribute__((ext_vector_type(2))) float f32x2_t;
 __device__ __forceinline__ void split4(const float4 v, uint2& p0, uint2& p1, uint2& p2) {
@@ -210,13 +222,20 @@
     } else {
         s0 = L * (unsigned)(32 * PXB * NW);
     }
+    unsigned sx0 = s0;
+    if constexpr (T == 9 && !S2) {
+        if (a.compact) {
+            unsigned i_, y_, x_;
+            sx0 = compact_pos(s0, a, i_, y_, x_);
+        }
+    }
 
     unsigned goff[NSLOT];
     unsigned vmask[T == 1 ? NSLOT : 1];
     int simg[H ? NSLOT : 1];
     const int woff0 = ((((tid & 3) >> 1) * a.NPp + (tid >> 2)) * 16 + (tid & 1) * 8);
     if (a.mode == MODE_STREAM) {
-        const int pos0 = (int)s0 - a.PWp - 1 + (tid >> 2);
+        const int pos0 = (int)sx0 - a.PWp - 1 + (tid >> 2);
         const unsigned cin4 = (unsigned)a.Cin * 4u;
         const unsigned base = (unsigned)pos0 * cin4 + (unsigned)(tid & 3) * 16u;
 #pragma unroll
@@ -229,7 +248,7 @@
 #pragma unroll
             for (int j = 0; j < NSLOT; ++j) {
                 const int pj = pos0 + (NT / 4) * j;
-                simg[j] = (int)pp_udiv((unsigned)min(max(pj, 0), (int)a.S - 1), a.dv_per);
+                simg[j] = (int)pp_udiv((unsigned)min(max(pj, 0), (int)a.Sx - 1), a.dv_per);
             }
         }
     } else {
@@ -372,6 +391,17 @@
             oy_ = y0 + ry;
             ox_ = x0 + rx;
             ok_ = oy_ < a.H && ox_ < a.W;
+        } else if (T == 9 && !S2 && a.compact) {
+            const int pl = (wave_ * PXB + pb) * 32 + (lane_ & 31);
+            const unsigned vp = s0 + (unsigned)pl;
+            const bool in = vp < (unsigned)a.S;
+            unsigned img, yy, xx;
+            const unsigned pos = compact_pos(in ? vp : (unsigned)a.S - 1u, a, img, yy, xx);
+            aofs_ = (((lane_ >> 5) * a.NPp) + (int)(pos - sx0)) * 16;
+            on_ = (int)img;
+            oy_ = (int)yy;
+            ox_ = (int)xx;
+            ok_ = in;
         } else {
             const unsigned per = a.mode == MODE_STREAM ? (unsigned)(a.xp_h * a.PWp) : (unsigned)(a.H * a.W);
             const unsigned row = a.mode == MODE_STREAM ? (unsigned)a.PWp : (unsigned)a.W;
@@ -723,8 +753,9 @@
         int wg_first = n, wg_last = n;
         if (a.mode != MODE_TILE) {
             const unsigned last = (unsigned)min((long long)s0 + 32 * PXB * NW - 1, a.S - 1);
-            wg_first = (int)pp_udiv(min(s0, last), a.dv_per);
-            wg_last = (int)pp_udiv(last, a.dv_per);
+            const unsigned (&dvs)[2] = a.compact ? a.dv_vper : a.dv_per;
+            wg_first = (int)pp_udiv(min(s0, last), dvs);
+            wg_last = (int)pp_udiv(last, dvs);
         }
         pp_amax_commit_wg<NW, PXB>(a.y_amax, on, ymax, wg_first, wg_last, reinterpret_cast<float*>(smem));
     }
@@ -768,11 +799,16 @@
     } else {
         s0 = L * 256u;
     }
+    unsigned sx0 = s0;
+    if (a.compact) {
+        unsigned i_, y_, x_;
+        sx0 = compact_pos(s0, a, i_, y_, x_);
+    }
     unsigned goff[NSLOT];
     int simg[H ? NSLOT : 1];
     const int woff0 = ((((tid & 3) >> 1) * a.NPp + (tid >> 2)) * 16 + (tid & 1) * 8);
     if (a.mode == MODE_STREAM) {
-        const int pos0 = (int)s0 - a.PWp - 1 + (tid >> 2);
+        const int pos0 = (int)sx0 - a.PWp - 1 + (tid >> 2);
         const unsigned cin4 = (unsigned)a.Cin * 4u;
         const unsigned base = (unsigned)pos0 * cin4 + (unsigned)(tid & 3) * 16u;
 #pragma unroll
@@ -781,7 +817,7 @@
 #pragma unroll
             for (int j = 0; j < NSLOT; ++j) {
                 const int pj = pos0 + (NT / 4) * j;
-                simg[j] = (int)pp_udiv((unsigned)min(max(pj, 0), (int)a.S - 1), a.dv_per);
+                simg[j] = (int)pp_udiv((unsigned)min(max(pj, 0), (int)a.Sx - 1), a.dv_per);
             }
         }
     } else {
@@ -890,6 +926,16 @@
             oy_ = y0 + ry;
             ox_ = x0 + rx;
             ok = oy_ < a.H && ox_ < a.W;
+        } else if (a.compact) {
+            const unsigned vp = s0 + (unsigned)(b * 32 + r);
+            const bool in = vp < (unsigned)a.S;
+            unsigned img, yy, xx;
+            const unsigned pos = compact_pos(in ? vp : (unsigned)a.S - 1u, a, img, yy, xx);
+            aof = ((khalf * a.NPp) + (int)(pos - sx0)) * 16;
+            on_ = (int)img;
+            oy_ = (int)yy;
+            ox_ = (int)xx;
+            ok = in;
         } else {
             const int pl = b * 32 + r;
             aof = ((khalf * a.NPp) + pl) * 16;
@@ -1109,8 +1155,9 @@
         int wg_first = n, wg_last = n;
         if (a.mode != MODE_TILE) {
             const unsigned last = (unsigned)min((long long)s0 + 255, a.S - 1);
-            wg_first = (int)pp_udiv(min(s0, last), a.dv_per);
-            wg_last = (int)pp_udiv(last, a.dv_per);
+            const unsigned (&dvs)[2] = a.compact ? a.dv_vper : a.dv_per;
+            wg_first = (int)pp_udiv(min(s0, last), dvs);
+            wg_last = (int)pp_udiv(last, dvs);
         }
         pp_amax_commit_wg<4, SB>(a.y_amax, onn, ymax, wg_first, wg_last, reinterpret_cast<float*>(smem));
     }
@@ -1978,19 +2025,40 @@
 }
 
 
-static TileGeom tap_tiling(const ConvArgs& a, int nw, int stream_env) {
+static int compact_patch_pixels(int H, int W, int xp_h, int xp_w, int tile) {
+    const long long hw = (long long)H * W;
+    const auto pos = [&](long long v) { return (v / hw * xp_h + v % hw / W) * xp_w + v % hw % W; };
+    long long g = tile, r = hw;
+    while (r) { const long long t = g % r; g = r; r = t; }
+    long long span = 0;
+    for (long long v0 = 0; v0 < hw; v0 += g) span = std::max(span, pos(v0 + tile - 1) - pos(v0));
+    return (int)std::min<long long>(span + 2 * xp_w + 3, 1 << 30);
+}
+
+static TileGeom tap_tiling(const ConvArgs& a, int nw, int stream_env, int compact_on) {
     const int max_np = nw == 8 ? 768 : 512, xp_h = a.Hin + a.x_pad, xp_w = a.Win + a.x_pad;
     TileGeom g = pick_tile(a.Hout, a.Wout, max_np, nw / 2);
     g.mode = MODE_TILE;
+    g.compact = 0;
     const int snp = 64 * nw + 2 + 2 * xp_w;
-    const double stream_eff = (double)a.Hout * a.Wout / ((double)xp_h * xp_w);
+    const int cnp = compact_on && a.x_pad >= 1 && snp <= max_np ? compact_patch_pixels(a.Hout, a.Wout, xp_h, xp_w, 64 * nw) : 0;
+    bool compact = cnp > 0 && cnp <= max_np;
+    if (nw == 8) {
+        const int xp = a.split_f16 ? 2 : 3, wpl = a.split_f16 ? 2 : 3;
+        int npp = cnp;
+        while (npp % 8 != 4) ++npp;
+        compact = compact && (size_t)2 * xp * 2 * npp * 16 + (size_t)4 * 2 * wpl * 1024 <= (size_t)160 * 1024;
+    }
+    if (compact_on < 0) compact = compact && cnp <= (nw == 8 ? max_np : 448) && 4 * cnp <= 5 * snp;
+    const double stream_eff = compact ? 1.0 : (double)a.Hout * a.Wout / ((double)xp_h * xp_w);
     bool use_stream = a.x_pad >= 1 && snp <= max_np && (g.eff < 0 || stream_eff > g.eff + 0.02);
     if (stream_env == 0 && g.eff >= 0) use_stream = false;
     if (stream_env == 1 && a.x_pad >= 1 && snp <= max_np) use_stream = true;
     if (use_stream) {
         g.mode = MODE_STREAM;
         g.PWp = xp_w;
-        g.NP = g.NPp = snp;
+        g.compact = compact;
+        g.NP = g.NPp = compact ? cnp : snp;
         while (g.NPp % 8 != 4) ++g.NPp;
     }
     return g;
@@ -2004,6 +2072,9 @@
     static const int c48_on = env_int("POSEPIPE_SPLIT_C48", 1), c48_mult = env_int("POSEPIPE_SPLIT_C48_MULT", 0);
     static const int stream_env = env_int("POSEPIPE_SPLIT_STREAM", -1);
     const char* s2_env = getenv("POSEPIPE_SPLIT_S2_MIN_CIN");
+    static const int compact_env = env_int("POSEPIPE_SPLIT_STREAM_COMPACT", -1);
+    const int compact_knob = g_split_stream_compact.load(std::memory_order_relaxed);
+    const int compact_on = compact_knob >= 0 ? compact_knob : compact_env;
     SplitPlan p;
     p.f16 = a.split_f16 != 0;
     const size_t wpl = p.f16 ? 2 : 3;
@@ -2065,11 +2136,11 @@
         p.ncb = (a.Cout + 47) / 48 * 3;
         p.nout = p.ncb * 16;
         steps = (size_t)(p.cin / 16) * 5;
-        p.tile[0] = tap_tiling(a, 4, stream_env);
+        p.tile[0] = tap_tiling(a, 4, stream_env, compact_on);
     } else {
         p.kernel = SPLIT_TAP3;
-        p.tile[0] = tap_tiling(a, 4, stream_env);
-        p.tile[1] = tap_tiling(a, 8, stream_env);
+        p.tile[0] = tap_tiling(a, 4, stream_env, compact_on);
+        p.tile[1] = tap_tiling(a, 8, stream_env, compact_on);
     }
     p.frag_bytes = (steps + 1) * p.ncb * wpl * 64 * sizeof(uint4);
     p.bytes = p.frag_bytes + (p.f16 ? (size_t)2 * p.nout * sizeof(float) : 0);
@@ -2197,7 +2268,7 @@
     fwrite(h.data(), 8, h.size(), f);
     fclose(f);
 }
-#define PP_TL_BEGIN() s.dbg = tl_begin(a, stream)
+#define PP_TL_BEGIN() s.dbg = tiles_only ? nullptr : tl_begin(a, stream)
 #define PP_TL_END(name, nwg) tl_end(a, s, name, nwg, stream)
 #else
 #define PP_TL_BEGIN()
@@ -2211,6 +2282,8 @@
     make_magic((unsigned)std::max(s.tiles_x, 1), s.dv_tx);
     make_magic((unsigned)std::max(s.tiles_y, 1), s.dv_ty);
     make_magic((unsigned)std::max(s.PWp, 1), s.dv_pw);
+    make_magic((unsigned)std::max(s.H * s.W, 1), s.dv_vper);
+    make_magic((unsigned)std::max(s.W, 1), s.dv_vrow);
     make_magic((unsigned)std::max(s.gy, 1), s.dv_ncol);
     make_magic((unsigned)std::max(s.gx >> 3, 1), s.dv_run0);
     make_magic((unsigned)((s.gx >> 3) + 1), s.dv_run1);
@@ -2247,6 +2320,7 @@
 
 static unsigned apply_tiling(SplitArgs& s, const TileGeom& g, const ConvArgs& a, int nw) {
     s.mode = g.mode;
+    s.compact = 0;
     s.NP = g.NP;
     s.NPp = g.NPp;
     if (g.mode == MODE_GEMM) {
@@ -2255,7 +2329,9 @@
     }
     s.PWp = g.PWp;
     if (g.mode == MODE_STREAM) {
-        s.S = (long long)a.N * s.xp_h * s.xp_w;
+        s.Sx = (long long)a.N * s.xp_h * s.xp_w;
+        s.compact = g.compact;
+        s.S = g.compact ? (long long)a.N * s.H * s.W : s.Sx;
         return (unsigned)((s.S + 64 * nw - 1) / (64 * nw));
     }
     s.tiles_x = g.tiles_x; s.tiles_y = g.tiles_y; s.TH = g.TH; s.TW = g.TW; s.bw_log2 = g.bw_log2; s.gx_log2 = g.gx_log2;
@@ -2293,8 +2369,9 @@
     return PP_OK;
 }
 
-int pp_launch_conv_split(const SplitPlan& p, const ConvArgs& a, hipStream_t stream) {
-    if (a.wsplit && p.kernel == SPLIT_STEM7) return launch_stem7(a, stream);
+static int split_launch(const SplitPlan& p, const ConvArgs& a, hipStream_t stream, unsigned* tiles_only) {
+    if (tiles_only) *tiles_only = 0;
+    if (a.wsplit && p.kernel == SPLIT_STEM7) return tiles_only ? PP_OK : launch_stem7(a, stream);
     if (!a.wsplit || p.kernel == SPLIT_NONE) {
         pp_set_error("conv_split: layer not eligible");
         return PP_ERR_ARG;
@@ -2340,10 +2417,11 @@
     s.wscale = f16 ? reinterpret_cast<const float*>(static_cast<const unsigned char*>(a.wsplit) + p.frag_bytes) : nullptr;
     s.x_amax = a.x_amax;
     s.y_amax = a.y_amax;
-    if (f16 && !a.x_amax) {
+    if (f16 && !a.x_amax && !tiles_only) {
         pp_set_error("conv_split: the fp16 form needs the per-sample maximum of its input (ConvArgs::x_amax)");
         return PP_ERR_STATE;
     }
+    if (tiles_only && p.kernel == SPLIT_PRODUCT) return PP_OK;
     PP_TL_BEGIN();
     s.col_major = (size_t)a.x_bytes <= (size_t)colmaj_mb << 20;
     const char* tag;
@@ -2373,6 +2451,7 @@
             return PP_ERR_STATE;
         }
         const unsigned gx = apply_tiling(s, p.tile[0], a, 4);
+        if (tiles_only) return *tiles_only = gx, PP_OK;
         s.SP = (s.TH + 1) * s.PWp;
         int cob = 1;
         for (int c : {4, 3, 2})
@@ -2396,6 +2475,7 @@
         tag = "s2p";
     } else if (p.kernel == SPLIT_C48) {
         const unsigned gx = apply_tiling(s, p.tile[0], a, 4);
+        if (tiles_only) return *tiles_only = gx, PP_OK;
         s.gx = (int)gx;
         s.gy = s.ncb / 3;
         grid = s.xcd_remap ? dim3((unsigned)((s.gx + 7) / 8 * 8 * s.gy), 1) : dim3(gx, (unsigned)s.gy);
@@ -2421,6 +2501,7 @@
             nw = 4;
             gx = apply_tiling(s, p.tile[0], a, nw);
         }
+        if (tiles_only) return *tiles_only = gx, PP_OK;
         const int nslot = (s.NP + 16 * nw - 1) / (16 * nw);
         const auto ring_fits = [&](int c) {
             return ring4_env && nw == 4 && s.mode != MODE_GEMM && (size_t)xp * 2 * s.NPp * 16 + (size_t)4 * c * wpl * 1024 <= 80 * 1024;
@@ -2446,3 +2527,7 @@
     }
     return PP_OK;
 }
+
+int pp_launch_conv_split(const SplitPlan& p, const ConvArgs& a, hipStream_t stream) { return split_launch(p, a, stream, nullptr); }
+
+int pp_conv_split_tiles(const SplitPlan& p, const ConvArgs& a, unsigned* tiles) { return split_launch(p, a, nullptr, tiles); }
diff --git a/posepipeline_amd/csrc/net.hip b/posepipeline_amd/csrc/net.hip
--- a/posepipeline_amd/csrc/net.hip
+++ b/posepipeline_amd/csrc/net.hip
@@ -917,6 +917,18 @@
     return PP_OK;
 }
 
+int pp_net_conv_tiles(pp_net* net, int batch, int* tiles) {
+    PP_REQUIRE(net && tiles && batch >= 1 && batch <= net->max_batch, "pp_net_conv_tiles: NULL argument or batch outside 1 .. max_batch");
+    for (size_t i = 0; i < net->ops.size(); ++i) {
+        tiles[i] = 0;
+        if (net->ops[i].type != PP_OP_CONV || net->split_plan[i].kernel == SPLIT_NONE || net->folded((int)i)) continue;
+        unsigned t = 0;
+        PP_TRY(pp_conv_split_tiles(net->split_plan[i], net_conv_args(net, (int)i, batch), &t));
+        tiles[i] = (int)t;
+    }
+    return PP_OK;
+}
+
 int pp_net_folded_into(pp_net* net, int* into) {
     PP_REQUIRE(net && into, "pp_net_folded_into: NULL argument");
     for (size_t i = 0; i < net->ops.size(); ++i) into[i] = net->folded((int)i) ? net->fold_into[i] : -1;
diff --git a/posepipeline_amd/csrc/pp_internal.h b/posepipeline_amd/csrc/pp_internal.h
--- a/posepipeline_amd/csrc/pp_internal.h
+++ b/posepipeline_amd/csrc/pp_internal.h
@@ -121,6 +121,7 @@
     int TH, TW, bw_log2, gx_log2, PWp, NP, NPp, tiles_x, tiles_y;
     double eff;
     int mode;
+    int compact;
 };
 enum SplitKernel {
     SPLIT_NONE = 0,
@@ -148,6 +149,7 @@
 SplitPlan pp_conv_split_plan(const ConvArgs& a);
 int pp_conv_split_weights(const SplitPlan& p, const ConvArgs& a, void* out, hipStream_t stream);
 int pp_launch_conv_split(const SplitPlan& p, const ConvArgs& a, hipStream_t stream);
+int pp_conv_split_tiles(const SplitPlan& p, const ConvArgs& a, unsigned* tiles);
 bool pp_conv_tracks_amax(const ConvArgs& a, bool split);
 bool pp_conv_split_enabled();
 bool pp_conv_split_f16_default();
diff --git a/posepipeline_amd/program.py b/posepipeline_amd/program.py
--- a/posepipeline_amd/program.py
+++ b/posepipeline_amd/program.py
@@ -536,6 +536,11 @@
         L.check(self.ctx.lib.pp_net_conv_kinds(self.handle, L.ptr(kinds)), "pp_net_conv_kinds")
         return kinds
 
+    def conv_tiles(self, batch) -> np.ndarray:
+        tiles = np.zeros(len(self.prog.ops), dtype=np.int32)
+        L.check(self.ctx.lib.pp_net_conv_tiles(self.handle, int(batch), L.ptr(tiles)), "pp_net_conv_tiles")
+        return tiles
+
     def folded_into(self) -> np.ndarray:
         into = np.zeros(len(self.prog.ops), dtype=np.int32)
         L.check(self.ctx.lib.pp_net_folded_into(self.handle, L.ptr(into)), "pp_net_folded_into")
```
